# 2bitoperations/rtldavis

Measured on AMD Instinct MI355X. Metric: complex MSamples/s demodulated (uint8 IQ -> packed bits -> preamble matches -> packets), higher is better.
Workload: dtype f32 (FIR: f16 x f16 -> f32 on the matrix pipe, exact integer accumulation); 1 GPU; 4096 streams x 33 blocks x 8192 samples uint8 IQ per GPU (BASELINE configs[3]/[4]: 64 unique synthetic streams tiled, 2.21 GB resident in HBM), 14 samples/symbol, 19.2 kbit/s; streams_per_gpu=4096, parallelism=streams/1

## Files before the change

include/rtldavis_hip.h:

```cpp
#ifndef RTLDAVIS_HIP_H
#define RTLDAVIS_HIP_H

#include <stddef.h>
#include <stdint.h>

#ifdef __cplusplus
extern "C" {
#endif

#define RD_MAX_PREAMBLE 64
#define RD_MAX_PKT_BYTES 32

typedef enum rd_status {
    RD_OK = 0,
    RD_ERR_ARG = -1,
    RD_ERR_DEVICE = -2,
    RD_ERR_CAPACITY = -3,
    RD_ERR_STATE = -4
} rd_status;

typedef struct rd_config {
    int32_t bit_rate;
    int32_t symbol_length;
    int32_t preamble_symbols;
    int32_t packet_symbols;
    int32_t block_size;
    uint8_t preamble[RD_MAX_PREAMBLE];
} rd_config;

typedef struct rd_packet {
    int32_t stream;
    int32_t call;
    int32_t index;
    int32_t nbytes;
    uint8_t data[RD_MAX_PKT_BYTES];
    double rssi;
    double snr;
} rd_packet;

typedef struct rd_parsed {
    int32_t stream;
    int32_t call;
    int32_t index;
    int32_t freq_err;
    int32_t id;
    int32_t nbytes;
    uint8_t data[RD_MAX_PKT_BYTES];
    double rssi;
    double snr;
} rd_parsed;

typedef struct rd_timing {
    float demod_ms;
    float fixup_ms;
    float search_ms;
    float slice_ms;
    float total_ms;
    int32_t runs;
} rd_timing;

const char *rd_last_error(void);
int rd_device_count(void);
int rd_set_device(int device);
int rd_set_wait_timeout_ms(int ms);

typedef struct rd_demod rd_demod;

int rd_create(const rd_config *cfg, rd_demod **out);
void rd_destroy(rd_demod *h);
int rd_reset(rd_demod *h);
int rd_demod_block(rd_demod *h, const void *samples, size_t count, int is_complex, rd_packet *out, int cap, int *n);
int rd_create_multi(const rd_config *cfg, int n_streams, rd_demod **out);
int rd_demod_blocks(rd_demod *h, const uint8_t *iq, size_t nbytes, rd_packet *out, int cap, int *n);
int rd_demod_submit(rd_demod *h, const void *samples, size_t count, int is_complex);
int rd_set_input_push(int mode);
int rd_demod_input_mode(rd_demod *h);
int rd_demod_register_input(rd_demod *h, void *host, size_t nbytes);
int rd_demod_submit_from(rd_demod *h, size_t offset, size_t count, int is_complex);
int rd_demod_fetch(rd_demod *h, rd_packet *out, int cap, int *n);
int rd_demod_inflight(rd_demod *h);
int rd_demod_refetch(rd_demod *h, rd_packet *out, int cap, int *n);
int rd_demod_set_parse(rd_demod *h, int enabled);
int rd_demod_parsed(rd_demod *h, rd_parsed *out, int cap, int *n);
int rd_parse_packet(const uint8_t *data, int nbytes, uint8_t *msg, int *id);
int rd_copy_discriminated_stream(rd_demod *h, int stream, double *out, size_t n);
int rd_copy_discriminated(rd_demod *h, double *out, size_t n);
int rd_copy_filtered(rd_demod *h, double *out_interleaved, size_t n_complex);
int rd_copy_quantized(rd_demod *h, uint8_t *out, size_t n);

typedef struct rd_batch rd_batch;

int rd_batch_create(const rd_config *cfg, int n_streams, int n_blocks, rd_batch **out);
void rd_batch_destroy(rd_batch *b);
int rd_batch_input_ptr(rd_batch *b, void **dev_ptr, size_t *nbytes);
int rd_batch_upload(rd_batch *b, const uint8_t *iq_host, size_t nbytes);
int rd_batch_upload_async(rd_batch *b, const uint8_t *iq_host, size_t nbytes, void *hip_stream);
int rd_batch_run(rd_batch *b, void *hip_stream);
int rd_batch_results(rd_batch *b, rd_packet *out, int cap, int *n);
int rd_batch_copy_bits(rd_batch *b, int stream, uint8_t *out, size_t nbytes);
int rd_batch_copy_discriminated(rd_batch *b, int stream, size_t t0, double *out, size_t n);
int rd_batch_set_parse(rd_batch *b, int enabled);
int rd_batch_parsed(rd_batch *b, rd_parsed *out, int cap, int *n);
int rd_batch_set_timing(rd_batch *b, int enabled);
int rd_batch_get_timing(rd_batch *b, rd_timing *out);
int rd_batch_set_pipelined(rd_batch *b, int enabled);
#define RD_FORM_ORDERED_TAIL 1u
#define RD_FORM_SECOND_PASS 8u
#define RD_FORM_ONE_LAUNCH_TAIL 16u
int rd_batch_last_run_forms(rd_batch *b, uint32_t *forms);
int rd_batch_get_counters(rd_batch *b, uint64_t *fixup_runs, uint64_t *matches);
int rd_k1_schedule(rd_batch *b, uint32_t *tiles_per_chunk, uint32_t *waves);

int rd_lut_execute(const uint8_t *in_bytes, size_t n_bytes, double *out_cplx, size_t n_cplx);
int rd_rotate_fs4(const double *in_cplx, double *out_cplx, size_t n_cplx);
int rd_fir9(const double *in_cplx, size_t n_in, double *out_cplx, size_t n_out);
int rd_discriminate(const double *in_cplx, size_t n_in, double *out, size_t n_out);
int rd_quantize(const double *in, uint8_t *out, size_t n);
int rd_search(const rd_config *cfg, const uint8_t *quantized, size_t n, int32_t *indices, int cap, int *count);

typedef struct rd_chan_config {
    int32_t out_rate;
    int32_t decim;
    int32_t n_taps;
    int32_t n_channels;
    double gain;
} rd_chan_config;
typedef struct rd_chan rd_chan;

#define RD_IQ_U8 0
#define RD_IQ_S8 1
#define RD_IQ_S16 2
#define RD_IQ_CF32 4

int rd_chan_create(const rd_chan_config *cfg, const double *taps, const int64_t *shift_hz, rd_chan **out);
int rd_chan_create_fmt(const rd_chan_config *cfg, int sample_format, const double *taps, const int64_t *shift_hz,
                       rd_chan **out);
void rd_chan_destroy(rd_chan *h);
int rd_chan_upload(rd_chan *h, const void *wide_iq, size_t nbytes);
int rd_chan_input_ptr(rd_chan *h, size_t n_wide_samples, void **dev_ptr);
int rd_chan_run(rd_chan *h, size_t n_out, void *dst_dev, size_t dst_stream_stride, void *hip_stream);
int rd_chan_run_host(rd_chan *h, size_t n_out, uint8_t *out_host, size_t nbytes);
int rd_chan_spectrum(rd_chan *h, int n_bins, double *power_host, uint32_t *segments);
int rd_chan_spectrum_dev(rd_chan *h, int n_bins, void *dst_dev, void *hip_stream);
int rd_chan_set_gain(rd_chan *h, const double *gain, int n);

typedef struct rd_wideband rd_wideband;
int rd_wideband_create(const rd_config *cfg, const rd_chan_config *ccfg, const double *taps,
                       const int64_t *shift_hz, rd_wideband **out);
int rd_wb_create_fmt(const rd_config *cfg, const rd_chan_config *ccfg, int sample_format, const double *taps,
                     const int64_t *shift_hz, rd_wideband **out);
void rd_wideband_destroy(rd_wideband *w);
int rd_wideband_reset(rd_wideband *w);
int rd_wideband_submit(rd_wideband *w, const void *wide_iq, size_t nbytes);
int rd_wideband_fetch(rd_wideband *w, rd_packet *out, int cap, int *n);
int rd_wideband_refetch(rd_wideband *w, rd_packet *out, int cap, int *n);
int rd_wideband_inflight(rd_wideband *w);
int rd_wideband_copy_channelized(rd_wideband *w, uint8_t *out, size_t nbytes);
int rd_wideband_copy_discriminated(rd_wideband *w, int channel, double *out, size_t n);
int rd_wb_set_parse(rd_wideband *w, int enabled);
int rd_wb_parsed(rd_wideband *w, rd_parsed *out, int cap, int *n);
int rd_wb_retune(rd_wideband *w, const int64_t *shift_hz, int n);
int rd_wb_tuning(rd_wideband *w, int64_t *shift_hz, int64_t *phase, int n);
int rd_wb_set_gain(rd_wideband *w, const double *gain, int n);
int rd_wb_gains(rd_wideband *w, double *gain, int n);
typedef struct rd_chan_level {
    uint64_t power;
    uint32_t peak;
    uint32_t clipped;
    float gain;
    uint32_t chunk;
} rd_chan_level;
typedef struct rd_input_level {
    uint64_t power;
    uint64_t chunk;
    uint32_t peak;
    uint32_t clipped;
} rd_input_level;
int rd_wb_set_levels(rd_wideband *w, int enabled);
int rd_wb_levels(rd_wideband *w, rd_chan_level *out, int n, rd_input_level *in);
typedef struct rd_spectrum_info {
    uint64_t chunk;
    uint32_t segments;
    uint32_t n_bins;
} rd_spectrum_info;
int rd_wb_set_spectrum(rd_wideband *w, int n_bins);
int rd_wb_spectrum(rd_wideband *w, double *power, int n_bins, rd_spectrum_info *info);
typedef struct rd_burst {
    int32_t  channel;
    uint32_t first;
    uint32_t windows;
    uint32_t flags;
    uint64_t power;
    uint32_t peak;
    uint32_t pad;
    int64_t  corr_re, corr_im;
} rd_burst;
typedef struct rd_burst_floor {
    uint32_t threshold;
    uint32_t windows_off;
    uint32_t n_bursts;
    uint32_t chunk;
    uint64_t power_off;
    int64_t  corr_re_off, corr_im_off;
} rd_burst_floor;
int rd_wb_set_bursts(rd_wideband *w, int enabled);
int rd_wb_set_burst_threshold(rd_wideband *w, const uint32_t *thr, int n);
int rd_wb_burst_thresholds(rd_wideband *w, uint32_t *thr, int n);
int rd_wb_bursts(rd_wideband *w, rd_burst *out, int cap, int *n, rd_burst_floor *floor, int n_floor);
#define RD_BURST_MSG_BYTES 10
#define RD_BURST_MSG_REPAIRED 2u
#define RD_BD_REPAIR_L 8
#define RD_BURST_MSG_NARROW 4u
#define RD_BD_NB_GRID 64
#define RD_BD_NB_SHIFT 11
#define RD_BD_NB_MIN_SL 4
#define RD_BD_NB_MAX_SL 51
typedef struct rd_burst_msg {
    int32_t  channel;
    uint32_t first;
    int32_t  tau;
    uint32_t flags;
    uint64_t time;
    uint64_t margin;
    int64_t  f_re, f_im;
    uint8_t  data[RD_BURST_MSG_BYTES];
    uint8_t  ones;
    uint8_t  id;
    uint8_t  pad[4];
} rd_burst_msg;
int rd_wb_set_burst_decode(rd_wideband *w, int enabled);
int rd_wb_set_burst_repair(rd_wideband *w, int max_flips);
int rd_wb_burst_repair(rd_wideband *w, int *max_flips);
int rd_wb_set_burst_narrow(rd_wideband *w, int on);
int rd_wb_burst_narrow(rd_wideband *w, int *on);
int rd_bd_narrow_table(int sl, int16_t *taps, int16_t *centres);
int rd_wb_burst_messages(rd_wideband *w, rd_burst_msg *out, int cap, int *n, uint32_t *long_runs, int n_channels);
#define RD_BURST_MSG_EXPECTED 8u
#define RD_BX_MAX 64
#define RD_BX_MAX_SPAN 2048
#define RD_BX_ANY_ID 0xFFu
#define RD_BX_NO_ENTRY 0xFFFFFFFFu
typedef struct rd_expect {
    int32_t  channel;
    uint32_t id;
    uint64_t t_lo, t_hi;
    int32_t  corr_re, corr_im;
} rd_expect;
int rd_wb_set_burst_expect(rd_wideband *w, const rd_expect *e, int n);
int rd_wb_burst_expect(rd_wideband *w, rd_expect *out, int cap, int *n);
int rd_wb_expected_messages(rd_wideband *w, rd_burst_msg *out, int cap, int *n, uint32_t *candidates, int n_cand);
#define RD_BURST_MSG_SEARCHED 16u
#define RD_BS_MAX_CENTRES 8
#define RD_BS_PER 4
#define RD_BS_TILE 1024
typedef struct rd_bs_header {
    uint32_t n_msgs, sync_hits;
    uint32_t chunk;
    uint32_t dropped;
} rd_bs_header;
int rd_wb_set_burst_search(rd_wideband *w, const uint8_t *centres, int n);
int rd_wb_burst_search(rd_wideband *w, uint8_t *out, int cap, int *n);
int rd_wb_searched_messages(rd_wideband *w, rd_burst_msg *out, int cap, int *n, rd_bs_header *hdr, int n_hdr);
#define RD_BQ_MAX_GAP 1024
#define RD_BQ_INBAND 1u
#define RD_BQ_UNMEASURABLE 128u
typedef struct rd_burst_quality {
    uint64_t pkt, sig, noise;
    uint64_t pkt_nb, sig_nb, noise_nb;
    uint32_t n_noise, clipped;
    uint16_t peak; uint8_t g; uint8_t flags;
    uint32_t chunk;
} rd_burst_quality;
int rd_wb_set_burst_quality(rd_wideband *w, int on, int noise_gap);
int rd_wb_burst_quality(rd_wideband *w, int *on, int *noise_gap);
int rd_wb_burst_message_quality(rd_wideband *w, rd_burst_quality *out, int cap, int *n);
int rd_wb_expected_message_quality(rd_wideband *w, rd_burst_quality *out, int cap, int *n);
int rd_bq_window(int sl, int n_sym, int block_size, int have_prev, int64_t tau, int gap, int32_t *out);
#define RD_BC_RUNS 1u
#define RD_BC_MESSAGES 2u
#define RD_BC_MAX_ROLL 1024
#define RD_BC_MAX_QUOTA 65536
#define RD_BC_MAX_POOL (1u << 26)
#define RD_BC_PER 16
#define RD_BC_CUT_START 1
#define RD_BC_CUT_END 2
#define RD_BC_FROM_PREV 4
typedef struct rd_burst_clip {
    int32_t  channel;
    uint32_t source;
    uint32_t flags;
    int32_t  t0;
    uint32_t n;
    uint32_t offset;
    uint64_t time;
    uint64_t ref;
    uint32_t chunk;
    uint32_t pad;
} rd_burst_clip;
int rd_wb_set_burst_clips(rd_wideband *w, int sources, int pre, int post, int quota);
int rd_wb_burst_clips_config(rd_wideband *w, int *sources, int *pre, int *post, int *quota);
int rd_wb_burst_clips(rd_wideband *w, rd_burst_clip *out, int cap, int *n, uint8_t *bytes, size_t bytes_cap, size_t *n_bytes,
                      uint32_t *dropped, int n_channels);
int rd_bc_window(int block_size, int have_prev, int64_t a, int64_t e, int32_t *out);
#define RD_BURST_MSG_REPLAYED 32u
#define RD_CD_MAX_SPAN 2048
#define RD_CD_MAX_JOBS (1 << 20)
#define RD_CD_MAX_TAU (1 << 30)
typedef struct rd_clip_job {
    uint64_t offset;
    uint64_t clock;
    uint32_t n;
    uint32_t id;
    int32_t  tau_lo, tau_hi;
    int32_t  corr_re, corr_im;
    int32_t  channel;
    uint32_t pad;
} rd_clip_job;
typedef struct rd_cd_header { uint32_t n_msgs, candidates; int32_t ca, cb; } rd_cd_header;
typedef struct rd_clips rd_clips;
int rd_clips_create(const rd_config *cfg, rd_clips **out);
void rd_clips_destroy(rd_clips *h);
int rd_clips_upload(rd_clips *h, const uint8_t *pool, size_t nbytes);
int rd_clips_decode(rd_clips *h, const rd_clip_job *jobs, int n_jobs, int max_flips, int narrow, rd_burst_msg *msgs,
                    rd_cd_header *hdr, int64_t *soft);
int rd_clips_kernel_ms(rd_clips *h, float *ms);
int rd_cd_check_jobs(const rd_config *cfg, const rd_clip_job *jobs, int n_jobs, size_t pool_outputs, int *bad, const char **why);
#define RD_CS_MAX_SYM 192
#define RD_CS_MAX_PRE 4096
#define RD_CS_MAX_N (1 << 24)
#define RD_CS_MAX_SPECS (1 << 20)
#define RD_CS_MAX_AMP (1u << 16)
#define RD_CS_MAX_NOISE (1u << 20)
#define RD_CS_MAX_AT (1 << 30)
#define RD_CS_MAX_POOL (1ull << 40)
#define RD_CS_TABLE 4096
typedef struct rd_clip_spec {
    uint64_t offset;
    uint64_t seed;
    uint32_t n;
    int32_t  at;
    uint32_t phase0;
    int32_t  f_c;
    uint32_t f_d;
    uint32_t amp_q;
    uint32_t noise_q;
    uint32_t n_sym;
    uint16_t pre, post;
    uint32_t pad;
    uint8_t  bits[24];
} rd_clip_spec;
int rd_clips_synth(rd_clips *h, const rd_clip_spec *specs, int n_specs, uint64_t pool_outputs);
int rd_clips_download(rd_clips *h, uint8_t *out, size_t nbytes);
int rd_clips_synth_ms(rd_clips *h, float *ms);
int rd_cs_check_specs(const rd_clip_spec *specs, int n_specs, uint64_t pool_outputs, int *bad, const char **why);
void rd_cs_table(int16_t out[RD_CS_TABLE]);
int rd_wb_fetched_chunk(rd_wideband *w, uint64_t *chunk);
int rd_wideband_debug_advance_clock(rd_wideband *w, uint64_t n_out);

void rd_debug_mfma_taps(uint16_t *out);
void rd_debug_mfma_taps8(uint16_t *out);
void rd_debug_mfma_taps8s(uint16_t *vals, uint32_t *idx);
int rd_debug_demod_mfma(const uint8_t *iq_host, int n_streams, uint32_t n_samples, int hist_mode,
                        uint32_t hist_bytes, float *g_out, uint32_t *bits_out, uint32_t *fix_out,
                        uint32_t fix_cap, uint32_t *n_fix);
int rd_debug_bursts(const uint8_t *chan, size_t stride, int n_ch, size_t n_out, const uint32_t *thr, uint64_t seq,
                    rd_burst *recs_out, rd_burst_floor *floor_out);
int rd_debug_burst_decode(const rd_config *cfg, const uint8_t *cur, const uint8_t *prev, size_t stride, int n_ch,
                          uint64_t clock, uint64_t seq, const rd_burst *runs, const uint32_t *n_runs,
                          rd_burst_msg *msgs_out, uint32_t *n_msgs, uint32_t *long_runs, uint32_t *chunk);
int rd_debug_burst_decode_repair(const rd_config *cfg, const uint8_t *cur, const uint8_t *prev, size_t stride, int n_ch,
                                 uint64_t clock, uint64_t seq, const rd_burst *runs, const uint32_t *n_runs, int max_flips,
                                 rd_burst_msg *msgs_out, uint32_t *n_msgs, uint32_t *long_runs, uint32_t *chunk);
int rd_debug_burst_decode_narrow(const rd_config *cfg, const uint8_t *cur, const uint8_t *prev, size_t stride, int n_ch,
                                 uint64_t clock, uint64_t seq, const rd_burst *runs, const uint32_t *n_runs, int max_flips,
                                 int narrow, rd_burst_msg *msgs_out, uint32_t *n_msgs, uint32_t *long_runs, uint32_t *chunk);
int rd_debug_burst_expect(const rd_config *cfg, const uint8_t *cur, const uint8_t *prev, size_t stride, int n_ch,
                          uint64_t clock, uint64_t seq, const rd_expect *e, int n_e, int max_flips, int narrow,
                          rd_burst_msg *msgs_out, uint32_t *hdr_out);
int rd_debug_burst_search(const rd_config *cfg, const uint8_t *cur, const uint8_t *prev, size_t stride, int n_ch,
                          uint64_t clock, uint64_t seq, const uint8_t *centres, int n, rd_burst_msg *msgs_out,
                          rd_bs_header *hdr_out);
#define RD_BQ_DEBUG_CHUNK 0x51A7u
int rd_debug_burst_quality(const rd_config *cfg, const uint8_t *cur, const uint8_t *prev, size_t stride, int n_ch,
                           int noise_gap, const rd_burst_msg *msgs, const uint32_t *n_msgs_per_channel, rd_burst_quality *out);
size_t rd_bc_slot_size(int n_ch, int quota);
int rd_debug_burst_clips(const rd_config *cfg, const uint8_t *cur, const uint8_t *prev, size_t stride, int n_ch, uint64_t clock,
                         uint64_t seq, const rd_burst *runs, const uint32_t *n_runs, const rd_burst_msg *msgs,
                         const uint32_t *n_msgs, const rd_burst_msg *x_msgs, const uint32_t *x_hdr, int n_expect,
                         const rd_burst_msg *s_msgs, const rd_bs_header *s_hdr, int n_search, const uint32_t *owed_prev,
                         int sources, int pre, int post, int quota, uint8_t *out);

#ifdef __cplusplus
}
#endif
#endif
```

rtldavis_amd/batch.py:

```python
from __future__ import annotations

import ctypes as C
from typing import List, Optional

import numpy as np

from . import _lib
from .dsp import Packet, PacketConfig, _cfg_struct


RD_PACKET_DTYPE = np.dtype([("stream", "<i4"), ("call", "<i4"), ("index", "<i4"), ("nbytes", "<i4"),
                            ("data", "u1", (_lib.RD_MAX_PKT_BYTES,)), ("rssi", "<f8"), ("snr", "<f8")])
assert RD_PACKET_DTYPE.itemsize == C.sizeof(_lib.RdPacket)


RD_PARSED_DTYPE = np.dtype([("stream", "<i4"), ("call", "<i4"), ("index", "<i4"), ("freq_err", "<i4"),
                            ("id", "<i4"), ("nbytes", "<i4"), ("data", "u1", (_lib.RD_MAX_PKT_BYTES,)),
                            ("rssi", "<f8"), ("snr", "<f8")])
assert RD_PARSED_DTYPE.itemsize == C.sizeof(_lib.RdParsed)


class BatchDemodulator:
    def __init__(self, cfg: PacketConfig, n_streams: int, n_blocks: int, device: Optional[int] = None) -> None:
        self.cfg = cfg
        self.n_streams = int(n_streams)
        self.n_blocks = int(n_blocks)
        self.n_samples = self.n_blocks * cfg.block_size
        self._b = C.c_void_p()
        if device is not None:
            _lib.check(_lib.lib().rd_set_device(int(device)))
        _lib.check(_lib.lib().rd_batch_create(C.byref(_cfg_struct(cfg)), self.n_streams, self.n_blocks, C.byref(self._b)))
        self._cap = 0
        self._recs = None

    def close(self) -> None:
        if self._b:
            b, self._b = self._b, None
            _lib.lib().rd_batch_destroy(b)

    def __del__(self):
        try:
            self.close()
        except Exception:
            pass

    def input_ptr(self):
        p, n = C.c_void_p(), C.c_size_t()
        _lib.check(_lib.lib().rd_batch_input_ptr(self._b, C.byref(p), C.byref(n)))
        return p.value, n.value

    def upload(self, iq: np.ndarray) -> None:
        a = np.ascontiguousarray(iq, dtype=np.uint8)
        if a.size != self.n_streams * 2 * self.n_samples:
            raise ValueError("Incompatible array sizes")
        _lib.check(_lib.lib().rd_batch_upload(self._b, a.ctypes.data, a.size))

    def upload_async(self, iq: np.ndarray, hip_stream: int) -> None:
        if iq.dtype != np.uint8 or not iq.flags["C_CONTIGUOUS"] or iq.size != self.n_streams * 2 * self.n_samples:
            raise ValueError("Incompatible array sizes")
        _lib.check(_lib.lib().rd_batch_upload_async(self._b, iq.ctypes.data, iq.size, C.c_void_p(hip_stream or None)))

    def run(self, hip_stream: int = 0) -> None:
        _lib.check(_lib.lib().rd_batch_run(self._b, C.c_void_p(hip_stream or None)))

    def set_parse(self, enabled: bool) -> None:
        _lib.check(_lib.lib().rd_batch_set_parse(self._b, int(bool(enabled))))

    def parsed(self) -> np.ndarray:
        cap = max(1024, 4 * self.n_streams)
        while True:
            buf = (_lib.RdParsed * cap)()
            n = C.c_int(0)
            rc = _lib.lib().rd_batch_parsed(self._b, buf, cap, C.byref(n))
            if rc == _lib.RD_ERR_CAPACITY:
                cap = n.value + 1024
                continue
            _lib.check(rc)
            return np.frombuffer(buf, dtype=RD_PARSED_DTYPE, count=n.value).copy()

    def set_timing(self, level) -> None:
        _lib.check(_lib.lib().rd_batch_set_timing(self._b, int(level)))

    def set_pipelined(self, enabled=True) -> None:
        _lib.check(_lib.lib().rd_batch_set_pipelined(self._b, 1 if enabled else 0))

    def timing(self) -> dict:
        t = _lib.RdTiming()
        _lib.check(_lib.lib().rd_batch_get_timing(self._b, C.byref(t)))
        return {k: float(getattr(t, k)) for k, _ in t._fields_}

    def last_run_forms(self) -> dict:
        f = C.c_uint32()
        _lib.check(_lib.lib().rd_batch_last_run_forms(self._b, C.byref(f)))
        return {"ordered_tail": bool(f.value & 1), "second_pass": bool(f.value & 8), "one_launch_tail": bool(f.value & 16)}

    def counters(self) -> dict:
        f, m = C.c_uint64(), C.c_uint64()
        _lib.check(_lib.lib().rd_batch_get_counters(self._b, C.byref(f), C.byref(m)))
        ch, wv = C.c_uint32(), C.c_uint32()
        _lib.check(_lib.lib().rd_k1_schedule(self._b, C.byref(ch), C.byref(wv)))
        return {"fixup_runs": f.value, "matches": m.value, "k1_chunk": ch.value, "k1_waves": wv.value}

    def results(self) -> np.ndarray:
        L = _lib.lib()
        n = C.c_int(0)
        if self._recs is None:
            self._cap = max(1024, 16 * self.n_streams)
            self._recs = (_lib.RdPacket * self._cap)()
        rc = L.rd_batch_results(self._b, self._recs, self._cap, C.byref(n))
        if rc == _lib.RD_ERR_CAPACITY:
            self._cap = n.value + 1024
            self._recs = (_lib.RdPacket * self._cap)()
            rc = L.rd_batch_results(self._b, self._recs, self._cap, C.byref(n))
        _lib.check(rc)
        return np.frombuffer(self._recs, dtype=RD_PACKET_DTYPE, count=n.value)

    def records(self):
        out = []
        for r in self.results():
            data = np.frombuffer(r["data"][: int(r["nbytes"])].tobytes(), dtype=np.uint8)
            out.append((int(r["stream"]), int(r["call"]),
                        Packet(int(r["index"]), data, float(r["rssi"]), float(r["snr"]))))
        return out

    def packets(self) -> List[List[List[Packet]]]:
        res = [[[] for _ in range(self.n_blocks)] for _ in range(self.n_streams)]
        for s, c, p in self.records():
            res[s][c].append(p)
        return res

    def bits(self, stream: int) -> np.ndarray:
        out = np.empty((self.n_samples + 7) // 8, dtype=np.uint8)
        _lib.check(_lib.lib().rd_batch_copy_bits(self._b, int(stream), out.ctypes.data, out.size))
        return out

    def discriminated(self, stream: int, t0: int, n: int) -> np.ndarray:
        out = np.empty(int(n), dtype=np.float64)
        _lib.check(_lib.lib().rd_batch_copy_discriminated(self._b, int(stream), int(t0), out.ctypes.data, out.size))
        return out

    def demodulate(self, iq: np.ndarray) -> List[List[List[Packet]]]:
        self.upload(iq)
        self.run()
        return self.packets()
```

rtldavis_amd/csrc/rd_batch.hip:

```cpp
#include <algorithm>
#include <chrono>
#include <cstdio>
#include <cstdlib>
#include <cstring>
#include <map>
#include <mutex>
#include <vector>

#include "rd_internal.h"
#include "rd_math.h"

static_assert(RD_BATCH_RUN == RD_RUN, "rd_batch_plan.h sizes the bit arrays by the kernels' run length");

static bool dbg_host() {
    static int v = -1;
    if (v < 0) v = getenv("RD_DEBUG_HOST") ? 1 : 0;
    return v == 1;
}
static double now_ms() {
    return std::chrono::duration<double, std::milli>(std::chrono::steady_clock::now().time_since_epoch()).count();
}

struct rd_batch_bufs {
    int device = -1;
    uint8_t *d_iq = nullptr;
    uint32_t *d_bits = nullptr, *d_fix = nullptr;
    uint32_t *d_cnt = nullptr;
    uint32_t *fixb = nullptr, *gstate = nullptr;
    uint32_t match_cap = 0, rec_cap = 0;
    rd_match *d_matches = nullptr;
    rd_packet *d_recs = nullptr;
    void *d_tasks = nullptr;
    rd_parsed *d_parsed = nullptr;
    uint32_t *h_cnt_pin = nullptr;
    rd_packet *h_recs_pin = nullptr;
    hipStream_t copy_stream = nullptr;
    hipEvent_t done = nullptr;
    hipEvent_t kdone = nullptr;
    hipEvent_t kfirst = nullptr;
    hipEvent_t uploaded = nullptr;
};
struct rd_batch_run_state {
    bool ran = false;
    bool fetched = false;
    bool upload_pending = false;
    hipStream_t stream = nullptr;
    int cnt_set = 0;
    bool timing = false, detail = false;
    hipEvent_t *ev = nullptr;
    rd_run_plan plan;
    bool ft_run = false;
    bool dev_order = false;
    int dense = 0;
    bool second_pass = false;
    bool deferred = false;
    uint32_t ft_seq = 0;
    uint32_t last_launch[2] = {0, 0};
    uint32_t have = 0;
    uint32_t h_cnt[RD_CNT_SLOTS] = {};
};
struct rd_batch_timer {
    std::vector<hipEvent_t> evs;
    size_t ev_runs = 0;
    std::vector<uint8_t> ev_end;
};
struct rd_batch {
    rd_devcfg dc;
    int n_streams, n_blocks;
    rd_batch_sizes sz;
    bool dev_ready = false;
    bool timing = false, timing_detail = false, parse = false, pipelined = false;
    rd_batch_bufs m;
    rd_batch_run_state run;
    rd_batch_learned learned;
    rd_batch_timer timer;
    rd_order_scratch order;
};

static rd_layout batch_layout(const rd_batch *b) {
    rd_layout l;
    l.iq = b->m.d_iq;
    l.stream_stride = (size_t)b->sz.n_samples * 2;
    l.n_streams = b->n_streams;
    l.n_samples = (uint32_t)b->sz.n_samples;
    l.hist_mode = 0;
    l.valid_from = 0;
    l.bits = b->m.d_bits;
    l.bits_stride = b->sz.bits_stride;
    return l;
}

extern "C" int rd_batch_create(const rd_config *cfg, int n_streams, int n_blocks, rd_batch **out) {
    if (!out) return rd_fail_msg(RD_ERR_ARG, "null out");
    rd_devcfg dc;
    int rc = rd_devcfg_checked(cfg, &dc);
    if (rc) return rc;
    const char *why = "";
    if ((rc = rd_batch_check_size(n_streams, n_blocks, cfg->block_size, &why))) return rd_fail_msg(rc, "%s", why);
    rd_batch *b = new rd_batch();
    b->dc = dc;
    b->n_streams = n_streams;
    b->n_blocks = n_blocks;
    b->sz = rd_batch_sizes_of(n_streams, n_blocks, dc, rd_batch_hooks());
    *out = b;
    return RD_OK;
}

static uint32_t *batch_cnt(const rd_batch *b) { return b->m.d_cnt + (size_t)b->run.cnt_set * b->sz.cnt_stride; }

static int batch_alloc_lists(rd_batch *b, uint32_t match_cap) {
    rd_batch_bufs &m = b->m;
    const bool ran = b->run.ran;
    if (m.match_cap) {
        hipFree(m.d_matches); m.d_matches = nullptr;
        hipFree(m.d_recs); m.d_recs = nullptr;
        hipHostFree(m.h_recs_pin); m.h_recs_pin = nullptr;
        hipFree(m.d_tasks); m.d_tasks = nullptr;
        hipFree(m.d_parsed); m.d_parsed = nullptr;
    }
    m.match_cap = m.rec_cap = 0;
    b->run.ran = false;
    const uint32_t rec_cap = 2 * match_cap;
    HIPCHK(hipMalloc(&m.d_matches, (size_t)match_cap * sizeof(rd_match)));
    HIPCHK(hipMalloc(&m.d_recs, (size_t)rec_cap * sizeof(rd_packet)));
    HIPCHK(hipMalloc(&m.d_tasks, (size_t)rec_cap * RD_TASK_BYTES));
    HIPCHK(hipHostMalloc((void **)&m.h_recs_pin, (size_t)rec_cap * sizeof(rd_packet), hipHostMallocDefault));
    m.match_cap = match_cap;
    m.rec_cap = rec_cap;
    b->run.ran = ran;
    return RD_OK;
}

static int batch_alloc(rd_batch *b) {
    rd_batch_bufs &m = b->m;
    if (b->dev_ready) return rd_use_device(m.device);
    int rc = rd_ensure_device();
    if (rc) return rc;
    HIPCHK(hipGetDevice(&m.device));
    const rd_batch_sizes z = b->sz = rd_batch_sizes_of(b->n_streams, b->n_blocks, b->dc, rd_batch_hooks_env());
    b->learned.bcap = z.bcap;
    HIPCHK(hipMalloc(&m.d_iq, z.iq_bytes + RD_INPUT_PAD));
    HIPCHK(hipMemset(m.d_iq + z.iq_bytes, 127, RD_INPUT_PAD));
    HIPCHK(hipMalloc(&m.d_bits, (uint64_t)b->n_streams * z.bits_stride * sizeof(uint32_t)));
    HIPCHK(hipMalloc(&m.d_fix, (size_t)z.fix_cap * sizeof(uint32_t)));
    if (z.ft_ok) {
        HIPCHK(hipMalloc(&m.fixb, z.groups * z.fix_bcap * sizeof(uint32_t)));
        HIPCHK(hipMalloc(&m.gstate, 3 * z.groups * sizeof(uint32_t)));
        HIPCHK(hipMemset(m.gstate, 0, 3 * z.groups * sizeof(uint32_t)));
    }
    HIPCHK(hipMalloc(&m.d_cnt, 2 * z.cnt_stride * sizeof(uint32_t)));
    HIPCHK(hipMemset(m.d_cnt, 0, 2 * z.cnt_stride * sizeof(uint32_t)));
    if ((rc = batch_alloc_lists(b, z.match_cap))) return rc;
    HIPCHK(hipHostMalloc((void **)&m.h_cnt_pin, RD_CNT_SLOTS * sizeof(uint32_t), hipHostMallocDefault));
    HIPCHK(hipEventCreateWithFlags(&m.done, hipEventDisableTiming));
    HIPCHK(hipEventCreateWithFlags(&m.kdone, hipEventDisableTiming));
    HIPCHK(hipEventCreateWithFlags(&m.kfirst, hipEventDisableTiming));
    HIPCHK(hipEventCreateWithFlags(&m.uploaded, hipEventDisableTiming));
    HIPCHK(hipStreamCreateWithFlags(&m.copy_stream, hipStreamNonBlocking));
    b->dev_ready = true;
    return RD_OK;
}

static void batch_free(rd_batch_bufs &m) {
    hipFree(m.d_iq); hipFree(m.d_bits); hipFree(m.d_fix); hipFree(m.d_cnt);
    hipFree(m.d_matches); hipFree(m.d_recs); hipFree(m.d_tasks);
    hipFree(m.d_parsed);
    hipFree(m.fixb); hipFree(m.gstate);
    hipHostFree(m.h_cnt_pin); hipHostFree(m.h_recs_pin);
    if (m.done) hipEventDestroy(m.done);
    if (m.kdone) hipEventDestroy(m.kdone);
    if (m.kfirst) hipEventDestroy(m.kfirst);
    if (m.uploaded) hipEventDestroy(m.uploaded);
    if (m.copy_stream) hipStreamDestroy(m.copy_stream);
}

static int timer_reserve(rd_batch_timer &t, size_t n) {
    const size_t old = t.evs.size();
    if (old >= n) return RD_OK;
    t.evs.resize(n, nullptr);
    for (size_t i = old; i < n; i++) HIPCHK(hipEventCreate(&t.evs[i]));
    return RD_OK;
}

static int batch_readback(rd_batch *b, hipEvent_t after) {
    rd_batch_bufs &m = b->m;
    HIPCHK(hipStreamWaitEvent(m.copy_stream, after, 0));
    HIPCHK(hipMemcpyAsync(m.h_cnt_pin, batch_cnt(b), RD_CNT_SLOTS * sizeof(uint32_t), hipMemcpyDeviceToHost, m.copy_stream));
    b->run.have = rd_batch_spec_count(b->run.dev_order, m.match_cap, m.rec_cap, b->learned.spec_recs);
    if (b->run.have)
        HIPCHK(hipMemcpyAsync(m.h_recs_pin, m.d_recs, (size_t)b->run.have * sizeof(rd_packet), hipMemcpyDeviceToHost, m.copy_stream));
    HIPCHK(hipEventRecord(m.done, m.copy_stream));
    return RD_OK;
}

static std::mutex g_tail_mx;
typedef std::pair<int, hipStream_t> rd_tail_key;
static std::map<rd_tail_key, rd_batch *> g_tail;

static void tail_park(rd_batch *b) {
    g_tail[rd_tail_key(b->m.device, b->run.stream)] = b;
    b->run.deferred = true;
}
static rd_batch *tail_take(int device, hipStream_t st) {
    auto it = g_tail.find(rd_tail_key(device, st));
    if (it == g_tail.end()) return nullptr;
    rd_batch *p = it->second;
    g_tail.erase(it);
    p->run.deferred = false;
    return p;
}
static void tail_drop(rd_batch *p) {
    auto it = g_tail.find(rd_tail_key(p->m.device, p->run.stream));
    if (it != g_tail.end() && it->second == p) g_tail.erase(it);
    p->run.deferred = false;
}

static int batch_flush_locked(rd_batch *p) {
    if (!p->run.deferred) return RD_OK;
    tail_drop(p);
    int rc = rd_use_device(p->m.device);
    if (rc) return rc;
    HIPCHK(hipEventRecord(p->m.kdone, p->run.stream));
    return batch_readback(p, p->m.kdone);
}
static int batch_flush(rd_batch *b) {
    std::lock_guard<std::mutex> g(g_tail_mx);
    return batch_flush_locked(b);
}
static bool batch_stream_has_tail(int device, hipStream_t st) {
    std::lock_guard<std::mutex> g(g_tail_mx);
    return g_tail.find(rd_tail_key(device, st)) != g_tail.end();
}
static int batch_adopt(int device, hipStream_t st, hipEvent_t carrier) {
    std::lock_guard<std::mutex> g(g_tail_mx);
    rd_batch *p = tail_take(device, st);
    return p ? batch_readback(p, carrier) : RD_OK;
}

static int batch_settle(rd_batch *b, const hipStream_t *st, const char *what = nullptr) {
    if (!b->run.ran || b->run.fetched) return RD_OK;
    int rc = batch_flush(b);
    if (rc) return rc;
    if (!st) return rd_wait_event(b->m.done, what);
    HIPCHK(hipStreamWaitEvent(*st, b->m.done, 0));
    return RD_OK;
}

extern "C" void rd_batch_destroy(rd_batch *b) {
    if (!b) return;
    {
        std::lock_guard<std::mutex> g(g_tail_mx);
        tail_drop(b);
    }
    if (b->dev_ready && rd_owns_device_state()) {
        if (b->m.device >= 0) hipSetDevice(b->m.device);
        if (b->run.ran && !b->run.fetched) hipDeviceSynchronize();
        batch_free(b->m);
        for (auto &e : b->timer.evs) if (e) hipEventDestroy(e);
    }
    delete b;
}

extern "C" int rd_batch_input_ptr(rd_batch *b, void **dev_ptr, size_t *nbytes) {
    if (!b || !dev_ptr) return rd_fail_msg(RD_ERR_ARG, "null argument");
    int rc = batch_alloc(b);
    if (rc) return rc;
    *dev_ptr = b->m.d_iq;
    if (nbytes) *nbytes = b->sz.iq_bytes;
    return RD_OK;
}

extern "C" int rd_batch_upload(rd_batch *b, const uint8_t *iq_host, size_t nbytes) {
    if (!b || !iq_host) return rd_fail_msg(RD_ERR_ARG, "null argument");
    int rc = batch_alloc(b);
    if (rc) return rc;
    if (nbytes != b->sz.iq_bytes) {
        return rd_fail_msg(RD_ERR_ARG, "Incompatible array sizes: got %zu bytes, expected %zu", nbytes, b->sz.iq_bytes);
    }
    if ((rc = batch_settle(b, nullptr, "the previous run before an upload"))) return rc;
    HIPCHK(hipMemcpy(b->m.d_iq, iq_host, nbytes, hipMemcpyHostToDevice));
    if (!b->learned.ft_sticky) b->learned.tail_off = false;
    return RD_OK;
}

extern "C" int rd_batch_upload_async(rd_batch *b, const uint8_t *iq_host, size_t nbytes, void *hip_stream) {
    if (!b || !iq_host) return rd_fail_msg(RD_ERR_ARG, "null argument");
    int rc = batch_alloc(b);
    if (rc) return rc;
    if (nbytes != b->sz.iq_bytes) return rd_fail_msg(RD_ERR_ARG, "Incompatible array sizes: got %zu bytes, expected %zu", nbytes, b->sz.iq_bytes);
    hipStream_t cs = (hipStream_t)hip_stream;
    if ((rc = batch_settle(b, &cs))) return rc;
    HIPCHK(hipMemcpyAsync(b->m.d_iq, iq_host, nbytes, hipMemcpyHostToDevice, cs));
    HIPCHK(hipEventRecord(b->m.uploaded, cs));
    b->run.upload_pending = true;
    if (!b->learned.ft_sticky) b->learned.tail_off = false;
    return RD_OK;
}

static hipEvent_t batch_event(const rd_batch *b, rd_run_event which) {
    switch (which) {
    case RD_RUN_EV0: return b->run.ev[0];
    case RD_RUN_EV1: return b->run.ev[1];
    case RD_RUN_EV4: return b->run.ev[4];
    case RD_RUN_KFIRST: return b->m.kfirst;
    case RD_RUN_KDONE: return b->m.kdone;
    default: return nullptr;
    }
}

static int batch_tail(rd_batch *b, bool first, uint32_t *zero_next = nullptr) {
    rd_batch_bufs &m = b->m;
    rd_batch_run_state &r = b->run;
    hipStream_t st = r.stream;
    const rd_layout lay = batch_layout(b);
    const long B = b->dc.B, L = b->dc.L, p_lo = B - L, p_hi = (long)(b->n_blocks + 1) * B - L;
    const bool last_on_slice = !b->parse, defer = first && r.plan.defer;
    hipEvent_t last = batch_event(b, first ? r.plan.end : r.plan.end_again);
    if (r.timing && first) b->timer.ev_end.push_back(defer ? 0 : 1);
    r.dev_order = false;
    if (r.ft_run && first) {
        rd_ft_bufs fb;
        fb.fixb = m.fixb; fb.gstate = m.gstate; fb.fix_bcap = b->sz.fix_bcap; fb.bcap = b->learned.bcap;
        fb.fixcnt = batch_cnt(b) + b->sz.ft_cnt_off;
        r.ft_seq = r.ft_seq % 4095u + 1u;
        const int ok = rd_launch_tail_fused(lay, b->dc, b->n_blocks, p_lo, p_hi, fb, b->sz.ft_limit ? b->sz.ft_limit : fb.bcap, r.ft_seq, 0,
                                            m.d_recs, m.rec_cap, batch_cnt(b), st, last_on_slice ? last : nullptr, zero_next,
                                            (uint32_t)b->sz.cnt_stride);
        if (!ok) return rd_fail_msg(RD_ERR_STATE, "the one-launch tail refused a shape its buffers were allocated for");
        r.dev_order = true;
        r.dense = 1;
    } else {
        rd_launch_search(m.d_bits, b->sz.bits_stride, b->n_streams, b->sz.n_samples, p_lo, p_hi, b->dc, m.d_matches, m.match_cap,
                         batch_cnt(b), st);
        if (r.timing && r.detail) HIPCHK(hipEventRecord(r.ev[3], st));
        r.dense = rd_launch_slice(lay, m.d_bits, b->sz.bits_stride, b->sz.n_samples, b->dc, m.d_matches, m.match_cap, 1, b->n_blocks, 0,
                                  m.d_recs, nullptr, batch_cnt(b), st, last_on_slice ? last : nullptr, m.d_tasks);
    }
    if (b->parse) {
        if (!m.d_parsed) HIPCHK(hipMalloc(&m.d_parsed, (size_t)m.rec_cap * sizeof(rd_parsed)));
        rd_launch_parse(lay, b->dc, m.d_recs, m.match_cap, m.d_parsed, batch_cnt(b), st, r.dense);
    }
    if (defer) {
        std::lock_guard<std::mutex> g(g_tail_mx);
        auto it = g_tail.find(rd_tail_key(m.device, st));
        if (it != g_tail.end() && it->second != b) {
            int rc = batch_flush_locked(it->second);
            if (rc) return rc;
        }
        tail_park(b);
        HIPCHK(hipGetLastError());
        return RD_OK;
    }
    if (!last_on_slice) HIPCHK(hipEventRecord(last, st));
    int rc = batch_readback(b, last);
    if (rc) return rc;
    HIPCHK(hipGetLastError());
    return RD_OK;
}

static int batch_refused(rd_batch *b, bool had_upload) {
    b->run.cnt_set ^= 1;
    b->run.upload_pending = had_upload;
    if (b->timing) b->timer.ev_runs--;
    b->run.ran = false;
    b->run.fetched = true;
    return rd_fail_msg(RD_ERR_STATE, "the demod kernel's grid has fewer waves than work queues and more chunks than waves: not launched");
}

static int batch_begin_run(rd_batch *b, hipStream_t st, bool *had_upload) {
    rd_batch_run_state &r = b->run;
    int rc = batch_settle(b, &st);
    if (rc) return rc;
    r.stream = st;
    *had_upload = r.upload_pending;
    if (r.upload_pending) {
        HIPCHK(hipStreamWaitEvent(st, b->m.uploaded, 0));
        r.upload_pending = false;
    }
    r.fetched = false;
    r.cnt_set ^= 1;
    r.timing = b->timing;
    r.detail = b->timing_detail;
    if (r.timing) {
        if ((rc = timer_reserve(b->timer, 5 * (b->timer.ev_runs + 1)))) return rc;
        r.ev = &b->timer.evs[5 * b->timer.ev_runs++];
    }
    return RD_OK;
}

extern "C" int rd_batch_run(rd_batch *b, void *hip_stream) {
    if (!b) return rd_fail_msg(RD_ERR_ARG, "null batch");
    int rc = batch_alloc(b);
    if (rc) return rc;
    rd_batch_run_state &r = b->run;
    hipStream_t st = (hipStream_t)hip_stream;
    bool had_upload = false;
    if ((rc = batch_begin_run(b, st, &had_upload))) return rc;
    uint32_t *cnt = batch_cnt(b), *cnt_next = b->m.d_cnt + (size_t)(r.cnt_set ^ 1) * b->sz.cnt_stride;
    const rd_run_plan p = r.plan = rd_batch_plan_run({b->sz.fast_ok, b->sz.ft_ok, b->learned.tail_off, r.timing, r.detail, b->pipelined,
                                                      b->parse, batch_stream_has_tail(b->m.device, st)});
    uint32_t *fixl = p.buckets ? b->m.fixb : b->m.d_fix, *bcnt = p.buckets ? cnt + b->sz.ft_cnt_off : nullptr;
    const uint32_t fixc = p.buckets ? b->sz.fix_bcap : b->sz.fix_cap;
    const rd_layout lay = batch_layout(b);
    uint32_t honoured = 0;
    if (p.record_around) HIPCHK(hipEventRecord(r.ev[0], st));
    if (p.demod) {
        honoured = rd_launch_demod(lay, fixl, fixc, cnt, st, batch_event(b, p.ride_start), batch_event(b, p.ride_stop),
                                   p.buckets ? RD_DEMOD_FIX_BUCKETS : 0u, r.last_launch, bcnt);
        if (honoured & RD_DEMOD_REFUSED) return batch_refused(b, had_upload);
    }
    if (p.record_around) HIPCHK(hipEventRecord(r.ev[1], st));
    if (p.record_carrier) HIPCHK(hipEventRecord(batch_event(b, p.carrier), st));
    if (p.carrier && (rc = batch_adopt(b->m.device, st, batch_event(b, p.carrier)))) return rc;
    r.second_pass = false;
    r.ft_run = p.demod && (honoured & RD_DEMOD_FIX_BUCKETS);
    if (!r.ft_run)
        rd_launch_fixup(lay, fixl, fixc, cnt, p.demod ? 0 : 1, cnt_next, st, (uint32_t)b->sz.cnt_stride, b->learned.last_fix);
    if (r.timing && r.detail) HIPCHK(hipEventRecord(r.ev[2], st));
    if ((rc = batch_tail(b, true, r.ft_run ? cnt_next : nullptr))) return rc;
    r.ran = true;
    return RD_OK;
}

static int batch_second_pass(rd_batch *b) {
    const uint32_t zero[5] = {0, 0, 0, 0, 0};
    HIPCHK(hipMemcpyAsync(batch_cnt(b) + RD_CNT_MATCH, zero, sizeof zero, hipMemcpyHostToDevice, b->run.stream));
    b->run.second_pass = true;
    return batch_tail(b, false);
}

struct batch_ladder {
    rd_batch *b;
    int read(rd_ladder_in &in) {
        rd_batch_run_state &r = b->run;
        const double ta = now_ms();
        int rc = rd_wait_event(b->m.done, "the batch run's results");
        if (rc) return rc;
        memcpy(r.h_cnt, b->m.h_cnt_pin, sizeof r.h_cnt);
        if (dbg_host()) fprintf(stderr, "[rd] finish: wait %.3f ms\n", now_ms() - ta);
        in = {r.h_cnt[RD_CNT_FIX], r.h_cnt[RD_CNT_MATCH], r.h_cnt[RD_CNT_OVF], r.ft_run, r.second_pass, r.dev_order, b->sz.fast_ok, 0,
              b->sz.fix_cap, b->m.match_cap, b->sz.ft_limit, (uint64_t)b->n_streams * b->sz.bits_stride};
        return RD_OK;
    }
    int carry_out(const rd_ladder_action &a) {
        rd_batch_run_state &r = b->run;
        int rc = RD_OK;
        r.dev_order = a.dev_order;
        if (a.exact_fixup) rd_launch_fixup(batch_layout(b), b->m.d_fix, b->sz.fix_cap, batch_cnt(b), 1, nullptr, r.stream);
        const uint32_t cap = b->sz.fix_cap;
        if (a.stamp_fix) HIPCHK(hipMemcpyAsync(batch_cnt(b) + RD_CNT_FIX, &cap, sizeof cap, hipMemcpyHostToDevice, r.stream));
        if (a.tail_overflow && dbg_host())
            fprintf(stderr, "[rd] one-launch tail overflow: flags %u (1 a stream's match list, 2 records), matches %u\n",
                    r.h_cnt[RD_CNT_OVF], r.h_cnt[RD_CNT_MATCH]);
        if (a.grow_to && (rc = batch_alloc_lists(b, a.grow_to))) return rc;
        if (a.second_pass && (rc = batch_second_pass(b))) return rc;
        if (a.done) r.fetched = true;
        return RD_OK;
    }
    int gave_up() { return rd_fail_msg(RD_ERR_DEVICE, "result lists kept overflowing"); }
};

static int batch_finish(rd_batch *b) {
    if (!b->run.ran) return rd_fail_msg(RD_ERR_STATE, "rd_batch_run has not been called");
    int rc = batch_flush(b);
    if (rc) return rc;
    batch_ladder hands = {b};
    return rd_batch_ladder_run(hands, b->learned);
}

extern "C" int rd_batch_results(rd_batch *b, rd_packet *out, int cap, int *n) {
    if (!b || !n) return rd_fail_msg(RD_ERR_ARG, "null argument");
    const double t0 = now_ms();
    int rc = batch_finish(b);
    if (rc) return rc;
    const double t1 = now_ms();
    rd_batch_bufs &m = b->m;
    rd_batch_run_state &r = b->run;
    const rd_result_counts c = rd_batch_result_counts(r.h_cnt, r.dense != 0, m.match_cap, m.rec_cap);
    if (c.nprim > r.have) {
        rc = rd_copy_d2h(m.h_recs_pin + r.have, m.d_recs + r.have, (size_t)(c.nprim - r.have) * sizeof(rd_packet), m.copy_stream);
        if (rc) return rc;
    }
    if (c.nextra) {
        rc = rd_copy_d2h(m.h_recs_pin + c.nprim, m.d_recs + m.match_cap, (size_t)c.nextra * sizeof(rd_packet), m.copy_stream);
        if (rc) return rc;
    }
    const uint32_t nrec = c.nprim + c.nextra;
    b->learned.spec_recs = std::max<uint32_t>(1024, c.nprim + c.nprim / 4);
    r.have = rd_batch_spec_count(r.dev_order, m.match_cap, m.rec_cap, b->learned.spec_recs);
    const double t2 = now_ms();
    if (!r.dev_order) rd_order_and_dedupe(m.h_recs_pin, nrec, b->dc.S, b->order);
    const size_t count = r.dev_order ? nrec : b->order.kept.size();
    *n = (int)count;
    if ((int)count > cap) return rd_fail_msg(RD_ERR_CAPACITY, "need room for %zu packets", count);
    if (count && !out) return rd_fail_msg(RD_ERR_ARG, "null out");
    if (r.dev_order && count) memcpy(out, m.h_recs_pin, count * sizeof(rd_packet));
    if (!r.dev_order)
        for (size_t i = 0; i < count; i++) out[i] = m.h_recs_pin[b->order.kept[i]];
    if (dbg_host())
        fprintf(stderr, "[rd] results%s: finish %.3f ms, D2H %u recs %.3f ms, %s %.3f ms\n", r.dev_order ? " (k_tail)" : "", t1 - t0,
                nrec, t2 - t1, r.dev_order ? "copy" : "order+dedupe+copy", now_ms() - t2);
    return RD_OK;
}

extern "C" int rd_batch_copy_bits(rd_batch *b, int stream, uint8_t *out, size_t nbytes) {
    if (!b || !out) return rd_fail_msg(RD_ERR_ARG, "null argument");
    if (stream < 0 || stream >= b->n_streams) return rd_fail_msg(RD_ERR_ARG, "stream out of range");
    const size_t need = (size_t)((b->sz.n_samples + 7) / 8);
    if (nbytes < need) return rd_fail_msg(RD_ERR_ARG, "bit buffer too small: %zu < %zu", nbytes, need);
    int rc = batch_finish(b);
    if (rc) return rc;
    return rd_copy_d2h(out, (const uint8_t *)(b->m.d_bits + (size_t)stream * b->sz.bits_stride), need, b->run.stream);
}

extern "C" int rd_batch_copy_discriminated(rd_batch *b, int stream, size_t t0, double *out, size_t n) {
    if (!b || !out) return rd_fail_msg(RD_ERR_ARG, "null argument");
    if (stream < 0 || stream >= b->n_streams || t0 + n > (size_t)b->sz.n_samples)
        return rd_fail_msg(RD_ERR_ARG, "range out of bounds");
    int rc = batch_alloc(b);
    if (rc) return rc;
    if (n == 0) return RD_OK;
    double *d = nullptr;
    HIPCHK(hipMalloc(&d, n * sizeof(double)));
    rd_launch_disc(batch_layout(b), stream, (long)t0, (long)n, d, b->run.stream);
    rc = rd_copy_d2h(out, d, n * sizeof(double), b->run.stream);
    hipFree(d);
    return rc;
}

extern "C" int rd_batch_set_parse(rd_batch *b, int enabled) {
    if (!b) return rd_fail_msg(RD_ERR_ARG, "null batch");
    b->parse = enabled != 0;
    return RD_OK;
}

extern "C" int rd_batch_parsed(rd_batch *b, rd_parsed *out, int cap, int *n) {
    if (!b || !n) return rd_fail_msg(RD_ERR_ARG, "null argument");
    if (!b->parse) return rd_fail_msg(RD_ERR_STATE, "rd_batch_set_parse(b, 1) must precede rd_batch_run");
    int rc = batch_finish(b);
    if (rc) return rc;
    const uint32_t np = std::min(b->run.h_cnt[RD_CNT_PARSED], b->m.rec_cap);
    std::vector<rd_parsed> recs(np);
    if (np) {
        rc = rd_copy_d2h(recs.data(), b->m.d_parsed, (size_t)np * sizeof(rd_parsed), b->run.stream);
        if (rc) return rc;
    }
    const size_t kept = rd_order_parsed(recs.data(), recs.size(), b->dc.S);
    *n = (int)kept;
    if ((int)kept > cap) return rd_fail_msg(RD_ERR_CAPACITY, "need room for %zu messages", kept);
    if (kept) {
        if (!out) return rd_fail_msg(RD_ERR_ARG, "null out");
        memcpy(out, recs.data(), kept * sizeof(rd_parsed));
    }
    return RD_OK;
}

extern "C" int rd_batch_set_pipelined(rd_batch *b, int enabled) {
    if (!b) return rd_fail_msg(RD_ERR_ARG, "null batch");
    b->pipelined = enabled != 0;
    return RD_OK;
}

extern "C" int rd_batch_set_timing(rd_batch *b, int enabled) {
    if (!b) return rd_fail_msg(RD_ERR_ARG, "null batch");
    b->timing = enabled != 0;
    b->timing_detail = enabled >= 2;
    b->timer.ev_runs = 0;
    b->timer.ev_end.clear();
    if (b->timing && b->dev_ready && rd_use_device(b->m.device) == RD_OK) return timer_reserve(b->timer, 5 * 64);
    return RD_OK;
}

extern "C" int rd_batch_get_timing(rd_batch *b, rd_timing *out) {
    if (!b || !out) return rd_fail_msg(RD_ERR_ARG, "null argument");
    if (!b->timing) return rd_fail_msg(RD_ERR_STATE, "timing not enabled");
    int rc = batch_finish(b);
    if (rc) return rc;
    rd_timing t = {};
    size_t n_end = 0;
    for (size_t r = 0; r < b->timer.ev_runs; r++) {
        hipEvent_t *e = &b->timer.evs[5 * r];
        float v[5] = {0, 0, 0, 0, 0};
        HIPCHK(hipEventElapsedTime(&v[0], e[0], e[1]));
        if (b->timing_detail) {
            HIPCHK(hipEventElapsedTime(&v[1], e[1], e[2]));
            HIPCHK(hipEventElapsedTime(&v[2], e[2], e[3]));
            HIPCHK(hipEventElapsedTime(&v[3], e[3], e[4]));
        }
        const bool has_end = r >= b->timer.ev_end.size() || b->timer.ev_end[r];
        if (has_end) { HIPCHK(hipEventElapsedTime(&v[4], e[0], e[4])); n_end++; }
        t.demod_ms += v[0]; t.fixup_ms += v[1]; t.search_ms += v[2]; t.slice_ms += v[3]; t.total_ms += v[4];
    }
    if (b->timer.ev_runs) {
        const float k = 1.0f / (float)b->timer.ev_runs;
        t.demod_ms *= k; t.fixup_ms *= k; t.search_ms *= k; t.slice_ms *= k;
        t.total_ms = n_end ? t.total_ms / (float)n_end : 0.0f;
    }
    t.runs = (int32_t)b->timer.ev_runs;
    b->timer.ev_runs = 0;
    b->timer.ev_end.clear();
    *out = t;
    return RD_OK;
}

extern "C" int rd_batch_last_run_forms(rd_batch *b, uint32_t *forms) {
    if (!b || !forms) return rd_fail_msg(RD_ERR_ARG, "null argument");
    int rc = batch_finish(b);
    if (rc) return rc;
    *forms = (b->run.dev_order ? RD_FORM_ORDERED_TAIL | RD_FORM_ONE_LAUNCH_TAIL : 0u) | (b->run.second_pass ? RD_FORM_SECOND_PASS : 0u);
    return RD_OK;
}

extern "C" int rd_k1_schedule(rd_batch *b, uint32_t *tiles_per_chunk, uint32_t *waves) {
    uint32_t v[2] = {0, 0};
    if (b) {
        if (!b->run.ran) return rd_fail_msg(RD_ERR_STATE, "rd_batch_run has not been called");
        v[0] = b->run.last_launch[0]; v[1] = b->run.last_launch[1];
    } else {
        rd_debug_last_launch(v);
    }
    if (tiles_per_chunk) *tiles_per_chunk = v[0];
    if (waves) *waves = v[1];
    return RD_OK;
}

extern "C" int rd_batch_get_counters(rd_batch *b, uint64_t *fixup_runs, uint64_t *matches) {
    if (!b) return rd_fail_msg(RD_ERR_ARG, "null batch");
    int rc = batch_finish(b);
    if (rc) return rc;
    if (fixup_runs) *fixup_runs = b->learned.last_fix;
    if (matches) *matches = b->learned.last_match;
    return RD_OK;
}
```

rtldavis_amd/csrc/rd_batch_plan.cpp:

```cpp
#include "rd_batch_plan.h"

#include <stdlib.h>

#include <algorithm>

int rd_batch_check_size(int n_streams, int n_blocks, int block_size, const char **why) {
    if (n_streams < 1 || n_blocks < 1) { *why = "n_streams and n_blocks must be >= 1"; return RD_ERR_ARG; }
    const long n = (long)n_blocks * block_size;
    const uint64_t runs = (uint64_t)n_streams * ((n + RD_BATCH_RUN - 1) / RD_BATCH_RUN);
    if (n > 0x7FFFFFF0L || runs > 0x0FFFFFFFull) {
        *why = "batch too large: at most 2^28 32-sample runs (8.6e9 samples) per batch";
        return RD_ERR_ARG;
    }
    *why = "";
    return RD_OK;
}

rd_batch_hooks rd_batch_hooks_env(void) {
    rd_batch_hooks h;
    const char *ti = getenv("RD_TAIL_IMPL");
    h.legacy_tail = ti && ti[0] == 'l';
    if (const char *e = getenv("RD_TEST_MATCH_CAP")) h.match_cap = atol(e);
    if (const char *e = getenv("RD_TEST_BUCKET_CAP")) h.bucket_cap = atol(e);
    if (const char *e = getenv("RD_TEST_FIX_BCAP")) h.fix_bcap = atol(e);
    return h;
}

rd_batch_sizes rd_batch_sizes_of(int n_streams, int n_blocks, const rd_devcfg &dc, const rd_batch_hooks &hooks) {
    rd_batch_sizes z;
    const long n = (long)n_blocks * dc.B;
    z.n_samples = n;
    z.bits_stride = (size_t)((n + 31) / 32);
    z.fast_ok = ((size_t)n * 2) % 16 == 0;
    const uint64_t runs = (uint64_t)n_streams * z.bits_stride;
    z.iq_bytes = (size_t)n_streams * n * 2;
    z.fix_cap = (uint32_t)std::min<uint64_t>(runs, std::max<uint64_t>(4096, runs / 8));
    z.match_cap = (uint32_t)std::min<uint64_t>((uint64_t)n_streams * (8 + 1ull * n_blocks) + 1024, 1u << 26);
    if (hooks.match_cap >= 1 && hooks.match_cap < (long)z.match_cap) z.match_cap = (uint32_t)hooks.match_cap;
    z.ft_ok = !hooks.legacy_tail && z.fast_ok && rd_davis_shape(dc) &&
              n < (1l << 30) && dc.B < (1 << 24) && z.bits_stride % 4 == 0 && dc.L >= dc.B &&
              (long)(n_blocks + 1) * dc.B - dc.L >= 0 &&
              ((long)(n_blocks + 1) * dc.B - dc.L) / 32 + 16 <= (long)z.bits_stride;
    if (hooks.bucket_cap >= 1 && hooks.bucket_cap < RD_BUCKET_MIN) z.ft_limit = (uint32_t)hooks.bucket_cap;
    if (!z.ft_ok) return z;
    z.groups = ((size_t)n_streams + RD_FT_STREAMS - 1) / RD_FT_STREAMS;
    z.ft_cnt_off = z.cnt_stride;
    z.cnt_stride += (z.groups + 3) & ~(size_t)3;
    const uint64_t tps = ((uint64_t)n + RD_TILE_SAMPLES - 1) / RD_TILE_SAMPLES;
    z.fix_bcap = (uint32_t)std::min<uint64_t>((2 * RD_FT_STREAMS * (tps / 4 + 8) + 63) & ~63ull, 1u << 20);
    if (hooks.fix_bcap >= 1 && hooks.fix_bcap < (long)z.fix_bcap) z.fix_bcap = (uint32_t)hooks.fix_bcap;
    z.bcap = rd_ord_bucket_cap(n);
    return z;
}

rd_run_plan rd_batch_plan_run(const rd_run_mode &m) {
    rd_run_plan p;
    p.demod = m.fast_ok;
    p.buckets = m.ft_ok && m.fast_ok && !m.tail_off && !(m.timing && m.timing_detail);
    if (m.timing && m.fast_ok) {
        p.ride_start = RD_RUN_EV0;
        p.ride_stop = RD_RUN_EV1;
    } else if (m.fast_ok && m.parked) {
        p.ride_stop = RD_RUN_KFIRST;
    }
    p.record_around = m.timing && !m.fast_ok;
    if (m.parked) {
        p.carrier = m.timing ? RD_RUN_EV1 : RD_RUN_KFIRST;
        p.record_carrier = !m.timing && !m.fast_ok;
    }
    p.defer = m.pipelined && !m.parse && !(m.timing && m.timing_detail);
    p.end_again = m.timing ? RD_RUN_EV4 : RD_RUN_KDONE;
    p.end = p.defer ? RD_RUN_EV_NONE : p.end_again;
    return p;
}

rd_ladder_action rd_batch_ladder_step(const rd_ladder_in &in, rd_batch_learned &lr) {
    rd_ladder_action a;
    a.dev_order = in.dev_order;
    const bool first_ft = in.ft_run && !in.second_pass;
    bool redo = false;
    if (first_ft && (in.ovf & (8u | 16u))) {
        a.exact_fixup = redo = true;
        lr.last_fix = in.all_runs;
        lr.tail_off = true;
        a.dev_order = false;
    } else {
        if (first_ft && (in.ovf & 1u)) {
            if (!in.ft_limit && lr.bcap < RD_BUCKET_MAX) lr.bcap = std::min<uint32_t>(2 * lr.bcap, RD_BUCKET_MAX);
            else if (!in.ft_limit) lr.ft_sticky = true;
        }
        if (in.fast_ok && !in.ft_run && in.fix > in.fix_cap) {
            a.exact_fixup = a.stamp_fix = redo = true;
            lr.last_fix = in.all_runs;
            if (lr.tail_off) a.dev_order = false;
        } else if (in.attempt == 0) {
            lr.last_fix = in.fix;
        }
        if (a.dev_order && in.ovf) {
            lr.tail_off = true;
            a.tail_overflow = a.second_pass = true;
            return a;
        }
    }
    if (!a.dev_order && in.match > in.match_cap) {
        a.grow_to = in.match + in.match / 4 + 1024;
        redo = true;
    }
    a.second_pass = redo;
    a.done = !redo;
    if (a.done) lr.last_match = in.match;
    return a;
}

uint32_t rd_batch_spec_count(bool dev_order, uint32_t match_cap, uint32_t rec_cap, uint32_t spec_recs) {
    return std::min(dev_order ? rec_cap : match_cap, spec_recs);
}

rd_result_counts rd_batch_result_counts(const uint32_t *h_cnt, bool dense, uint32_t match_cap, uint32_t rec_cap) {
    rd_result_counts c;
    c.nprim = dense ? std::min(h_cnt[RD_CNT_TASKS], rec_cap) : std::min(h_cnt[RD_CNT_MATCH], match_cap);
    c.nextra = dense ? 0u : std::min(h_cnt[RD_CNT_REC], match_cap);
    return c;
}
```

rtldavis_amd/csrc/rd_batch_plan.h:

```cpp
#pragma once
#include <stddef.h>
#include <stdint.h>

#include "rd_host.h"

enum { RD_CNT_FIX = 0, RD_CNT_MATCH = 1, RD_CNT_REC = 2, RD_CNT_TASKS = 3, RD_CNT_PARSED = 4, RD_CNT_OVF = 5, RD_CNT_SLOTS = 8 };
#define RD_FT_GSH 2
#define RD_FT_STREAMS (1 << RD_FT_GSH)
#define RD_NQUEUE 32
#define RD_QUEUE_STRIDE 64
#define RD_CNT_QUEUE0 RD_QUEUE_STRIDE
#define RD_CNT_TOTAL (RD_CNT_QUEUE0 + RD_NQUEUE * RD_QUEUE_STRIDE)
#define RD_TILE_SAMPLES 2048
#define RD_BATCH_RUN 32
#define RD_BATCH_ATTEMPTS 8

int rd_batch_check_size(int n_streams, int n_blocks, int block_size, const char **why);

struct rd_batch_hooks {
    bool legacy_tail = false;
    long match_cap = 0;
    long bucket_cap = 0;
    long fix_bcap = 0;
};
rd_batch_hooks rd_batch_hooks_env(void);

struct rd_batch_sizes {
    long n_samples = 0;
    size_t bits_stride = 0;
    bool fast_ok = false;
    size_t iq_bytes = 0;
    uint32_t fix_cap = 0;
    uint32_t match_cap = 0;
    bool ft_ok = false;
    size_t groups = 0;
    size_t cnt_stride = RD_CNT_TOTAL;
    size_t ft_cnt_off = 0;
    uint32_t fix_bcap = 0;
    uint32_t bcap = 0;
    uint32_t ft_limit = 0;
};
rd_batch_sizes rd_batch_sizes_of(int n_streams, int n_blocks, const rd_devcfg &dc, const rd_batch_hooks &hooks);

enum rd_run_event : uint8_t { RD_RUN_EV_NONE = 0, RD_RUN_EV0, RD_RUN_EV1, RD_RUN_EV4, RD_RUN_KFIRST, RD_RUN_KDONE };
struct rd_run_plan {
    bool demod = false;
    bool buckets = false;
    rd_run_event ride_start = RD_RUN_EV_NONE, ride_stop = RD_RUN_EV_NONE;
    bool record_around = false;
    rd_run_event carrier = RD_RUN_EV_NONE;
    bool record_carrier = false;
    bool defer = false;
    rd_run_event end = RD_RUN_EV_NONE;
    rd_run_event end_again = RD_RUN_EV_NONE;
};
struct rd_run_mode {
    bool fast_ok, ft_ok, tail_off, timing, timing_detail, pipelined, parse;
    bool parked;
};
rd_run_plan rd_batch_plan_run(const rd_run_mode &m);

struct rd_batch_learned {
    bool tail_off = false;
    bool ft_sticky = false;
    uint32_t bcap = 0;
    uint32_t spec_recs = 1024;
    uint64_t last_fix = 0, last_match = 0;
};
struct rd_ladder_in {
    uint32_t fix, match, ovf;
    bool ft_run, second_pass, dev_order, fast_ok;
    int attempt;
    uint32_t fix_cap, match_cap, ft_limit;
    uint64_t all_runs;
};
struct rd_ladder_action {
    bool exact_fixup = false;
    bool stamp_fix = false;
    uint32_t grow_to = 0;
    bool second_pass = false;
    bool done = false;
    bool dev_order = false;
    bool tail_overflow = false;
};
rd_ladder_action rd_batch_ladder_step(const rd_ladder_in &in, rd_batch_learned &lr);
template <class Dev>
int rd_batch_ladder_run(Dev &dev, rd_batch_learned &lr) {
    for (int attempt = 0; attempt < RD_BATCH_ATTEMPTS; attempt++) {
        rd_ladder_in in = {};
        int rc = dev.read(in);
        if (rc) return rc;
        in.attempt = attempt;
        const rd_ladder_action a = rd_batch_ladder_step(in, lr);
        if ((rc = dev.carry_out(a))) return rc;
        if (a.done) return RD_OK;
    }
    return dev.gave_up();
}

uint32_t rd_batch_spec_count(bool dev_order, uint32_t match_cap, uint32_t rec_cap, uint32_t spec_recs);
struct rd_result_counts { uint32_t nprim, nextra; };
rd_result_counts rd_batch_result_counts(const uint32_t *h_cnt, bool dense, uint32_t match_cap, uint32_t rec_cap);
```

rtldavis_amd/csrc/rd_demod_mfma.hip:

```cpp
#include <cstdio>
#include <cstdlib>
#include <cstring>

#include <hip/hip_ext.h>

#include "rd_internal.h"
#include "rd_math.h"
#include "rd_mfma.h"

#define RD_MF_WG 256
#define RD_MF_WAVES (RD_MF_WG / 64)
#ifndef RD_MF_MINWAVES
#define RD_MF_MINWAVES 4
#endif
#define RD_MF_GROUP_BYTES 1152
#define RD_MF_IMG_BYTES (16 + 4 * RD_MF_GROUP_BYTES)
#define RD_MF_IMG_PAD 4624
#define RD_MF_XB_BYTES (3 * 1024 + 32 + 32)
#define RD_MF_PEND 64
#ifndef RD_MF_STAGE_TILES
#define RD_MF_STAGE_TILES 4
#endif

typedef _Float16 rd_h8 __attribute__((ext_vector_type(8)));
typedef _Float16 rd_h16 __attribute__((ext_vector_type(16)));
typedef _Float16 rd_h2 __attribute__((ext_vector_type(2)));
typedef float rd_f16v __attribute__((ext_vector_type(16)));
typedef uint32_t rd_u4v __attribute__((ext_vector_type(4)));
typedef float rd_f4v __attribute__((ext_vector_type(4)));
typedef uint32_t rd_u2v __attribute__((ext_vector_type(2)));

static const rd_mf_taps h_mf_taps = rd_mf_make_taps();
__device__ const rd_mf_taps8 g_mf_taps8 = rd_mf_make_taps8();
static const rd_mf_taps8 h_mf_taps8 = rd_mf_make_taps8();
extern "C" void rd_debug_mfma_taps8(uint16_t *out) { memcpy(out, &h_mf_taps8, sizeof h_mf_taps8); }
#ifndef RD_MF_SPARSE
#define RD_MF_SPARSE 1
#endif
constexpr bool rd_mf_taps8s_ok() { bool ok = true; (void)rd_mf_make_taps8s(&ok); return ok; }
static_assert(rd_mf_taps8s_ok(), "a row of the tap matrix has more than two non-zero elements in a group of four");
constexpr rd_mf_taps8s rd_mf_taps8s_value() { bool ok = true; return rd_mf_make_taps8s(&ok); }
__device__ const rd_mf_taps8s g_mf_taps8s = rd_mf_taps8s_value();
static const rd_mf_taps8s h_mf_taps8s = rd_mf_taps8s_value();
extern "C" void rd_debug_mfma_taps8s(uint16_t *vals, uint32_t *idx) {
    memcpy(vals, h_mf_taps8s.v, sizeof h_mf_taps8s.v);
    memcpy(idx, h_mf_taps8s.idx, sizeof h_mf_taps8s.idx);
}

extern "C" void rd_debug_mfma_taps(uint16_t *out) { memcpy(out, &h_mf_taps, sizeof h_mf_taps); }

__device__ __forceinline__ rd_h8 rd_mf_frag(rd_u2v d) {
    rd_u4v v;
    v.x = d.x & 0x00FF00FFu;
    v.y = __builtin_amdgcn_perm(0u, d.x, 0x0c030c01u);
    v.z = d.y & 0x00FF00FFu;
    v.w = __builtin_amdgcn_perm(0u, d.y, 0x0c030c01u);
    return __builtin_bit_cast(rd_h8, v);
}

__device__ __forceinline__ float rd_mf_num(float ar, float ai, float cr, float ci, float &t1) {
    t1 = ai * ci;
    return __builtin_fmaf(-ar, cr, -t1);
}
__device__ __forceinline__ float rd_mf_guard(float nmin, float tmax) { return __builtin_fmaf(-4.76837158e-7f, tmax, nmin); }


template <int OFF>
__device__ __forceinline__ void rd_lds_write16(uint32_t addr, rd_f4v v) {
    asm volatile("ds_write_b128 %0, %1 offset:%2" : : "v"(addr), "v"(v), "i"(OFF) : "memory");
}
template <int OFF>
__device__ __forceinline__ rd_f4v rd_lds_read16(uint32_t addr) {
    rd_f4v r;
    asm volatile("ds_read_b128 %0, %1 offset:%2" : "=v"(r) : "v"(addr), "i"(OFF) : "memory");
    return r;
}
__device__ __forceinline__ void rd_lds_wait(rd_f4v &r) { asm volatile("s_waitcnt lgkmcnt(0)" : "+v"(r) : : "memory"); }
__device__ __forceinline__ void rd_lds_write4(uint32_t addr, uint32_t v) {
    asm volatile("ds_write_b32 %0, %1" : : "v"(addr), "v"(v) : "memory");
}
__device__ __forceinline__ rd_u4v rd_lds_read16u(uint32_t addr) {
    rd_u4v r;
    asm volatile("ds_read_b128 %0, %1\n\ts_waitcnt lgkmcnt(0)" : "=&v"(r) : "v"(addr) : "memory");
    return r;
}
__device__ __forceinline__ uint32_t rd_lds_read4(uint32_t addr) {
    uint32_t r;
    asm volatile("ds_read_b32 %0, %1\n\ts_waitcnt lgkmcnt(0)" : "=&v"(r) : "v"(addr) : "memory");
    return r;
}
__device__ __forceinline__ uint32_t rd_lds_addr(const void *p) {
    return (uint32_t)(uintptr_t)(const __attribute__((address_space(3))) void *)p;
}

__device__ __forceinline__ bool rd_mf_any(bool c) { return __ballot(c) != 0; }


struct rd_mf8_addr {
    uint32_t xw;
    uint32_t xw7;
    uint32_t rd1, rdE, rdO;
    uint32_t rd0;
};
struct rd_mf8_kept {
    float n2, n3;
    float g0r, g0i;
    float g1r, g1i, g2r, g2i;
    float nmin, tmax;
};

template <int B>
__device__ __forceinline__ constexpr int rd_mf8_woff() { return B == 0 ? 0 : (B & 1) ? 1024 : 2048; }

template <int B, int DBG>
__device__ __forceinline__ void rd_mf8_finish(const rd_mf8_kept &k, rd_f4v &p, uint32_t &W, uint32_t &fb, bool &slow) {
    rd_lds_wait(p);
    float t0, t1;
    const float n0 = rd_mf_num(p.x, p.y, p.z, p.w, t0);
    const float n1 = rd_mf_num(p.z, p.w, k.g0r, k.g0i, t1);
    if (DBG == 0 || DBG == 3) {
        const float nm = rd_mf_guard(rd_min3abs(k.nmin, n0, n1), rd_max3abs(k.tmax, t0, t1));
        if (rd_mf_any(!(nm > RD_MF_C0_MAX))) {
            slow = true;
            float F = rd_max3abs(0.0f, p.x, p.y);
            F = rd_max3abs(F, p.z, p.w);
            F = rd_max3abs(F, k.g0r, k.g0i);
            F = rd_max3abs(F, k.g1r, k.g1i);
            F = rd_max3abs(F, k.g2r, k.g2i);
            if (!(nm > rd_mf_c0(F))) fb |= 1u << (8 * (B & 3));
        }
    }
    uint32_t w = rd_shift_in_sign(W, n0);
    w = rd_shift_in_sign(w, n1);
    w = rd_shift_in_sign(w, k.n2);
    W = __builtin_amdgcn_alignbit(w, __builtin_bit_cast(uint32_t, k.n3), 27);
}

template <int B, int DBG>
__device__ __forceinline__ void rd_mf8_block(const rd_h8 (&A)[2], const rd_f16v &dcC, const int sidx, const int sidx2, const rd_u2v (&D)[9],
                                             rd_h8 &bfA, rd_h16 &bb, const rd_mf8_addr &ad, rd_mf8_kept &k0, rd_mf8_kept &kp, rd_f4v &p, uint32_t &Wlo,
                                             uint32_t &Whi, uint32_t &fblo, uint32_t &fbhi, bool &slow, float *dg, int dleft) {
    const rd_h8 bfB = rd_mf_frag(D[B + 1]);
    if (RD_MF_SPARSE && DBG != 8 && DBG != 9) {
        const rd_h16 wB = __builtin_shufflevector(bfB, bfB, 0, 1, 2, 3, 4, 5, 6, 7, 0, 1, 2, 3, 4, 5, 6, 7);
        if (B & 1) bb = __builtin_shufflevector(wB, bb, 0, 1, 2, 3, 4, 5, 6, 7, 24, 25, 26, 27, 28, 29, 30, 31);
        else bb = __builtin_shufflevector(bb, wB, 0, 1, 2, 3, 4, 5, 6, 7, 16, 17, 18, 19, 20, 21, 22, 23);
    }
    __builtin_amdgcn_sched_barrier(0);
    rd_f16v acc;
    if (DBG == 8 || DBG == 9) {
        rd_f16v c0 = dcC;
        if (DBG == 9) asm volatile("" : "+v"(c0));
        acc = __builtin_amdgcn_mfma_f32_32x32x16_f16(A[0], bfA, c0, 0, 0, 0);
        asm volatile("" : : "v"(bfB));
    } else if (RD_MF_SPARSE) {
        const uint32_t dbits = __builtin_bit_cast(uint32_t, -(float)RD_MF_DHI / 16777216.0f);
        uint64_t dh2 = ((uint64_t)dbits << 32) | dbits;
        asm volatile("" : "+s"(dh2));
        struct { uint64_t q[8]; } ci;
#pragma unroll
        for (int i = 0; i < 4; i++) asm volatile("v_mov_b64 %0, %1" : "=v"(ci.q[i]) : "s"(dh2));
#pragma unroll
        for (int i = 4; i < 8; i++) asm volatile("v_mov_b64 %0, 0" : "=v"(ci.q[i]));
        asm volatile("s_nop 1" ::: "memory");
        const rd_f16v c0 = __builtin_bit_cast(rd_f16v, ci);
        acc = (B & 1) ? __builtin_amdgcn_smfmac_f32_32x32x32_f16(A[1], bb, c0, sidx2, 0, 0)
                      : __builtin_amdgcn_smfmac_f32_32x32x32_f16(A[0], bb, c0, sidx, 0, 0);
    } else {
        acc = __builtin_amdgcn_mfma_f32_32x32x16_f16(A[0], bfA, dcC, 0, 0, 0);
        acc = __builtin_amdgcn_mfma_f32_32x32x16_f16(A[1], bfB, acc, 0, 0, 0);
    }
    if (B >= 2) rd_mf8_finish<B - 1, DBG>(kp, p, B - 1 <= 3 ? Wlo : Whi, B - 1 <= 3 ? fblo : fbhi, slow);
    __builtin_amdgcn_sched_barrier(0);
    float g[8];
#pragma unroll
    for (int i = 0; i < 8; i++) g[i] = __builtin_fmaf(acc[i], 2048.0f, acc[8 + i]);
    if (DBG == 3) {
#pragma unroll
        for (int r = 0; r < 4; r++)
            if (8 * B + r < dleft) { dg[2 * (8 * B + r)] = g[2 * r]; dg[2 * (8 * B + r) + 1] = g[2 * r + 1]; }
    }
    if (DBG != 10 && DBG != 11) {
        const rd_f4v x = {g[4], g[5], g[6], g[7]};
        if (B == 7) rd_lds_write16<0>(ad.xw7, x);
        else rd_lds_write16<rd_mf8_woff<B>()>(ad.xw, x);
    } else {
        asm volatile("" : : "v"(g[4]), "v"(g[5]), "v"(g[6]), "v"(g[7]));
    }
    if (B >= 1 && DBG != 10 && DBG != 11) p = rd_lds_read16<0>(B == 1 ? ad.rd1 : (B & 1) ? ad.rdO : ad.rdE);
    if (DBG == 11) asm volatile("" : "+v"(p));
    rd_mf8_kept &k = B == 0 ? k0 : kp;
    float t2, t3;
    k.n2 = rd_mf_num(g[0], g[1], g[2], g[3], t2);
    k.n3 = rd_mf_num(g[2], g[3], g[4], g[5], t3);
    k.nmin = rd_min3abs(3.0e38f, k.n2, k.n3);
    k.tmax = rd_max3abs(0.0f, t2, t3);
    k.g0r = g[0]; k.g0i = g[1];
    k.g1r = g[2]; k.g1i = g[3]; k.g2r = g[4]; k.g2i = g[5];
    bfA = bfB;
}

template <int DBG>
__device__ __forceinline__ void rd_mf8_tile(const rd_h8 (&A)[2], const rd_f16v &dcC, const int sidx, const int sidx2, const rd_u2v (&D)[9],
                                            const rd_mf8_addr &ad,
                                            uint32_t &word, uint32_t &fbw, bool &slow, float *dg, int dleft) {
    rd_h8 bfA = rd_mf_frag(D[0]);
    rd_h16 bb = __builtin_shufflevector(bfA, bfA, 0, 1, 2, 3, 4, 5, 6, 7, 8, 9, 10, 11, 12, 13, 14, 15);
    rd_mf8_kept k0, kp;
    rd_f4v p = {0.0f, 0.0f, 0.0f, 0.0f};
    uint32_t Wlo = 0, Whi = 0, fblo = 0, fbhi = 0;
    slow = false;
    rd_mf8_block<0, DBG>(A, dcC, sidx, sidx2, D, bfA, bb, ad, k0, kp, p, Wlo, Whi, fblo, fbhi, slow, dg, dleft);
    rd_mf8_block<1, DBG>(A, dcC, sidx, sidx2, D, bfA, bb, ad, k0, kp, p, Wlo, Whi, fblo, fbhi, slow, dg, dleft);
    rd_mf8_block<2, DBG>(A, dcC, sidx, sidx2, D, bfA, bb, ad, k0, kp, p, Wlo, Whi, fblo, fbhi, slow, dg, dleft);
    rd_mf8_block<3, DBG>(A, dcC, sidx, sidx2, D, bfA, bb, ad, k0, kp, p, Wlo, Whi, fblo, fbhi, slow, dg, dleft);
    rd_mf8_block<4, DBG>(A, dcC, sidx, sidx2, D, bfA, bb, ad, k0, kp, p, Wlo, Whi, fblo, fbhi, slow, dg, dleft);
    rd_mf8_block<5, DBG>(A, dcC, sidx, sidx2, D, bfA, bb, ad, k0, kp, p, Wlo, Whi, fblo, fbhi, slow, dg, dleft);
    rd_mf8_block<6, DBG>(A, dcC, sidx, sidx2, D, bfA, bb, ad, k0, kp, p, Wlo, Whi, fblo, fbhi, slow, dg, dleft);
    rd_mf8_block<7, DBG>(A, dcC, sidx, sidx2, D, bfA, bb, ad, k0, kp, p, Wlo, Whi, fblo, fbhi, slow, dg, dleft);
    rd_f4v p0 = rd_lds_read16<0>(ad.rd0);
    rd_mf8_finish<7, DBG>(kp, p, Whi, fbhi, slow);
    {
        rd_lds_wait(p0);
        float t0, t1;
        const float n0 = rd_mf_num(p0.x, p0.y, p0.z, p0.w, t0);
        const float n1 = rd_mf_num(p0.z, p0.w, k0.g0r, k0.g0i, t1);
        if (DBG == 0 || DBG == 3) {
            const float nm = rd_mf_guard(rd_min3abs(k0.nmin, n0, n1), rd_max3abs(k0.tmax, t0, t1));
            if (rd_mf_any(!(nm > RD_MF_C0_MAX))) {
                slow = true;
                float F = rd_max3abs(0.0f, p0.x, p0.y);
                F = rd_max3abs(F, p0.z, p0.w);
                F = rd_max3abs(F, k0.g0r, k0.g0i);
                F = rd_max3abs(F, k0.g1r, k0.g1i);
                F = rd_max3abs(F, k0.g2r, k0.g2i);
                if (!(nm > rd_mf_c0(F))) fblo |= 1u;
            }
        }
        uint32_t b0 = rd_shift_in_sign(0u, n0);
        b0 = rd_shift_in_sign(b0, n1);
        b0 = rd_shift_in_sign(b0, k0.n2);
        b0 = __builtin_amdgcn_alignbit(b0, __builtin_bit_cast(uint32_t, k0.n3), 27);
        Wlo = (b0 << 24) | Wlo;
    }
    const uint32_t Vlo = __builtin_bitreverse32(Wlo & 0xF0F0F0F0u), Vhi = __builtin_bitreverse32(Whi & 0xF0F0F0F0u);
    const auto r = __builtin_amdgcn_permlane32_swap(Vlo, Vhi, false, false);
    word = (r[1] << 4) | r[0];
    fbw = 0;
    if (slow && rd_mf_any((fblo | fbhi) != 0)) {
        const auto f = __builtin_amdgcn_permlane32_swap(fblo, fbhi, false, false);
        fbw = f[0] | f[1];
    }
}

#ifndef RD_MF_LOAD_AUX
#define RD_MF_LOAD_AUX 2
#endif

__device__ __forceinline__ void rd_mf_issue(const rd_layout &lay, uint32_t s, uint32_t ti, uint8_t *img, int lane,
                                            bool halo_dma = true) {
    const uint8_t *src = lay.iq + (size_t)s * lay.stream_stride + (size_t)ti * RD_TILE_BYTES;
    const int perm = 8 * (lane & 7) + (lane >> 3);
    const __attribute__((address_space(1))) void *g0 = (const __attribute__((address_space(1))) void *)(src + perm * 16);
    __builtin_amdgcn_global_load_lds(g0, (__attribute__((address_space(3))) void *)(img + 16), 16, 0, RD_MF_LOAD_AUX);
    __builtin_amdgcn_global_load_lds(g0, (__attribute__((address_space(3))) void *)(img + 16 + 128), 16, 1024, RD_MF_LOAD_AUX);
    __builtin_amdgcn_global_load_lds(g0, (__attribute__((address_space(3))) void *)(img + 16 + 256), 16, 2048, RD_MF_LOAD_AUX);
    __builtin_amdgcn_global_load_lds(g0, (__attribute__((address_space(3))) void *)(img + 16 + 384), 16, 3072, RD_MF_LOAD_AUX);
    const bool has_halo = (ti > 0) || lay.hist_mode;
    if (lane == 0 && halo_dma)
        __builtin_amdgcn_global_load_lds((const __attribute__((address_space(1))) void *)(src + (has_halo ? -16 : 0)),
                                         (__attribute__((address_space(3))) void *)(img), 16, 0, 0);
}

__device__ __forceinline__ int rd_lane_now() {
    return (int)__builtin_amdgcn_mbcnt_hi(~0u, __builtin_amdgcn_mbcnt_lo(~0u, 0u));
}

__device__ __forceinline__ void rd_mf_flush(const uint32_t *pend, uint32_t count, uint32_t *fix_list, uint32_t fix_cap,
                                            uint32_t *counters, uint32_t bits_stride, uint32_t *bucket_cnt) {
    const int lane = rd_lane_now();
    asm volatile("s_waitcnt lgkmcnt(0)" ::: "memory");
    if (bucket_cnt) {
        for (uint32_t i = lane; i < count; i += 64) {
            const uint32_t e = pend[i];
            const uint32_t grp = ((e >> 4) / bits_stride) >> RD_FT_GSH;
            const uint32_t slot = atomicAdd(&bucket_cnt[grp], 1u);
            if (slot < fix_cap) fix_list[(size_t)grp * fix_cap + slot] = e;
        }
        return;
    }
    uint32_t base = 0;
    if (lane == 0) base = atomicAdd(&counters[RD_CNT_FIX], count);
    base = __builtin_amdgcn_readfirstlane(base);
    for (uint32_t i = lane; i < count; i += 64)
        if (base + i < fix_cap) fix_list[base + i] = pend[i];
}


__device__ __forceinline__ void rd_mf_store_staged(uint32_t stage_addr, uint32_t nst, uint32_t *base, uint32_t stflags) {
    const int lane = rd_lane_now();
    if (nst == RD_MF_STAGE_TILES) {
#pragma unroll
        for (int j = 0; j < RD_MF_STAGE_TILES / 4; j++) {
            const rd_u4v v = rd_lds_read16u(stage_addr + 16 * (lane + 64 * j));
            if (!(stflags & 1)) __builtin_nontemporal_store(v, (rd_u4v *)(base + 4 * (lane + 64 * j)));
            else *(rd_u4v *)(base + 4 * (lane + 64 * j)) = v;
        }
    } else {
        for (uint32_t q = 0; q < nst; q++) base[64 * q + lane] = rd_lds_read4(stage_addr + 256 * q + 4 * lane);
    }
}

struct rd_mf_pos {
    uint32_t tile, s, ti, inchunk;
};
struct rd_mf_nextchunk {
    uint32_t tile, s, ti;
};
__device__ __forceinline__ rd_mf_nextchunk rd_mf_chunk_at(uint64_t chunk_id, uint32_t chunk, uint32_t tps, uint32_t total) {
    rd_mf_nextchunk c;
    const uint32_t n_chunks = (total + chunk - 1) / chunk;
    const bool have = chunk_id < n_chunks;
    const uint32_t nt = have ? (uint32_t)chunk_id * chunk : 0u;
    c.tile = have ? nt : 0xFFFFFFFFu;
    c.s = 0; c.ti = 0;
    if (have) {
        c.s = __builtin_amdgcn_readfirstlane(c.tile / tps);
        c.ti = c.tile - c.s * tps;
    }
    return c;
}
__device__ __forceinline__ rd_mf_pos rd_mf_next(rd_mf_pos p, uint32_t chunk, uint32_t tps, const rd_mf_nextchunk &nc) {
    rd_mf_pos q;
    if (p.inchunk + 1 < chunk) {
        q.tile = p.tile + 1; q.inchunk = p.inchunk + 1;
        q.s = p.s; q.ti = p.ti + 1;
        if (q.ti >= tps) { q.ti = 0; q.s++; }
    } else {
        q.tile = nc.tile; q.inchunk = 0;
        q.s = nc.s; q.ti = nc.ti;
    }
    return q;
}

__device__ __forceinline__ void rd_mf_read_window(uint32_t a_prv, uint32_t a_own, rd_u2v (&D)[9]) {
    asm volatile("ds_read_b64 %0, %9\n\t"
                 "ds_read_b64 %1, %10\n\t"
                 "ds_read_b64 %2, %10 offset:128\n\t"
                 "ds_read_b64 %3, %10 offset:256\n\t"
                 "ds_read_b64 %4, %10 offset:384\n\t"
                 "ds_read_b64 %5, %10 offset:512\n\t"
                 "ds_read_b64 %6, %10 offset:640\n\t"
                 "ds_read_b64 %7, %10 offset:768\n\t"
                 "ds_read_b64 %8, %10 offset:896\n\t"
                 "s_waitcnt lgkmcnt(0)"
                 : "=&v"(D[0]), "=&v"(D[1]), "=&v"(D[2]), "=&v"(D[3]), "=&v"(D[4]), "=&v"(D[5]), "=&v"(D[6]),
                   "=&v"(D[7]), "=&v"(D[8])
                 : "v"(a_prv), "v"(a_own)
                 : "memory");
}

__device__ __forceinline__ uint64_t rd_stamp() {
    uint64_t t;
    __builtin_amdgcn_sched_barrier(0);
    asm volatile("s_memtime %0\n\ts_waitcnt lgkmcnt(0)" : "=s"(t) : : "memory");
    __builtin_amdgcn_sched_barrier(0);
    return t;
}
__device__ __forceinline__ uint64_t rd_stamp_real() {
    uint64_t t;
    __builtin_amdgcn_sched_barrier(0);
    asm volatile("s_memrealtime %0\n\ts_waitcnt lgkmcnt(0)" : "=s"(t) : : "memory");
    __builtin_amdgcn_sched_barrier(0);
    return t;
}


#define RD_STAMP_WORDS 12
#define RD_STF_BUCKETS 8192u
template <int DBG, bool STAMP>
__global__ __launch_bounds__(RD_MF_WG, RD_MF_MINWAVES) void k_demod_mfma(rd_layout lay, uint32_t tiles_per_stream, uint32_t total_tiles,
                                                         uint32_t chunk, uint32_t *fix_list, uint32_t fix_cap,
                                                         uint32_t *counters, float *dbg_g, uint32_t stflags) {
    __shared__ __attribute__((aligned(16))) uint8_t s_img[RD_MF_WAVES][RD_MF_IMG_PAD];
    __shared__ __attribute__((aligned(32))) uint8_t s_xb[RD_MF_WAVES][RD_MF_XB_BYTES];
    __shared__ uint32_t s_pend[RD_MF_WAVES][RD_MF_PEND];
    __shared__ __attribute__((aligned(16))) uint32_t s_stage[RD_MF_WAVES][RD_MF_STAGE_TILES][64];
    constexpr bool LOADS = DBG != 1;
    const int lane = threadIdx.x & 63;
    const int wave = __builtin_amdgcn_readfirstlane(threadIdx.x >> 6);
    uint8_t *img0 = s_img[wave];
    uint8_t *xb = s_xb[wave];
    uint32_t *mypend = s_pend[wave];
    uint32_t npend = 0;
    constexpr bool CAN_BUCKET = DBG == 0 && !STAMP;
    uint32_t *bucket_cnt = (CAN_BUCKET && (stflags & RD_STF_BUCKETS)) ? (uint32_t *)dbg_g : nullptr;

    const int n = lane & 31, h = lane >> 5;
    rd_h8 A8[2];
    rd_f16v dcC;
    int sidx = 0, sidx2 = 0;
    if (RD_MF_SPARSE && DBG != 8 && DBG != 9) {
        A8[0] = *(const rd_h8 *)g_mf_taps8s.v[lane];
        A8[1] = *(const rd_h8 *)g_mf_taps8s.v[lane ^ 32];
        sidx = (int)g_mf_taps8s.idx[lane];
        sidx2 = (int)g_mf_taps8s.idx[lane ^ 32];
    } else {
        A8[0] = *(const rd_h8 *)g_mf_taps8.v[0][lane];
        A8[1] = *(const rd_h8 *)g_mf_taps8.v[1][lane];
    }
    const float dchi = -(float)RD_MF_DHI / 16777216.0f;
#pragma unroll
    for (int i = 0; i < 16; i++) dcC[i] = i < 8 ? dchi : 0.0f;
    if (RD_MF_SPARSE && DBG != 8 && DBG != 9) asm volatile("" : "+v"(A8[0]), "+v"(A8[1]), "+v"(sidx), "+v"(sidx2));
    else asm volatile("" : "+v"(A8[0]), "+v"(A8[1]), "+v"(dcC));
    const uint32_t img_addr = rd_lds_addr(img0);
    const uint32_t own = 16 + RD_MF_GROUP_BYTES * (n >> 3) + 16 * (n & 7) + 8 * h;
    const uint32_t prv = n == 0 ? 8 * h
                       : (n & 7) ? own + 16 * 55
                                 : 16 + RD_MF_GROUP_BYTES * ((n >> 3) - 1) + 16 * 63 + 8 * h;
    const uint32_t xb_addr = rd_lds_addr(xb), pend_addr = rd_lds_addr(mypend);
    const uint32_t stage_addr = rd_lds_addr(s_stage[wave]);
    const uint32_t rtoggle = lane == 0 ? 16u : 0u, wtoggle = lane == 63 ? 16u : 0u;
    rd_mf8_addr ad8;
    ad8.xw = xb_addr + 16 * lane;
    ad8.xw7 = xb_addr + (lane == 63 ? 3072 : 1024 + 16 * lane);
    ad8.rd1 = xb_addr + (h ? 1024 + 16 * (lane - 32) : 16 * (lane + 32));
    ad8.rdE = xb_addr + (h ? 2048 + 16 * (lane - 32) : 1024 + 16 * (lane + 32));
    ad8.rdO = xb_addr + (h ? 1024 + 16 * (lane - 32) : 2048 + 16 * (lane + 32));
    ad8.rd0 = xb_addr + (h ? 16 * (lane - 32) : lane ? 1024 + 16 * (lane + 31) : 3072 + 16);
    if (lane < 8) ((uint32_t *)(xb + 3072))[lane] = 0;

    const uint32_t nwaves = gridDim.x * RD_MF_WAVES;
    const uint32_t wave_id = blockIdx.x * RD_MF_WAVES + wave;
    const bool dynamic = !(stflags & 4096) && chunk >= 4;
    uint32_t cur_chunk = wave_id;
    rd_mf_nextchunk nextc = {0xFFFFFFFFu, 0, 0};
    if (!dynamic) nextc = rd_mf_chunk_at((uint64_t)cur_chunk + nwaves, chunk, tiles_per_stream, total_tiles);
    uint32_t grab = 0;
    bool grab_pending = false;
    const uint32_t my_queue = wave_id % RD_NQUEUE;
    uint32_t *queue = &counters[RD_CNT_QUEUE0 + RD_QUEUE_STRIDE * my_queue];
    rd_mf_pos cur;
    cur.tile = wave_id * chunk;
    cur.s = cur.tile / tiles_per_stream;
    cur.ti = cur.tile % tiles_per_stream;
    cur.inchunk = 0;
    rd_mf_pos nx1 = rd_mf_next(cur, chunk, tiles_per_stream, nextc);

    uint32_t nst = 0;
    uint32_t *st_base = nullptr;
    bool st_flush = false;
    uint64_t sm_wait = 0, sm_gap = 0, sm_comp = 0, sm_wait_st = 0, sm_t0 = 0, sm_r0 = 0, sm_mark = 0, sm_wmax = 0;
    uint32_t sm_iters = 0, sm_iters_st = 0;
    bool sm_stored = false;
    if (STAMP) { sm_t0 = rd_stamp(); sm_r0 = rd_stamp_real(); }
    if (LOADS && cur.tile < total_tiles) rd_mf_issue(lay, cur.s, cur.ti, img0, lane);
    if (STAMP) sm_mark = rd_stamp();
    while (cur.tile < total_tiles) {
        const uint32_t tile = cur.tile, s = cur.s, ti = cur.ti, inchunk = cur.inchunk;
        uint64_t sm_a = 0;
        if (STAMP) { sm_a = rd_stamp(); sm_comp += sm_a - sm_mark; }
        asm volatile("s_waitcnt vmcnt(0)" : "+v"(grab) : : "memory");
        uint64_t sm_b = 0;
        if (STAMP) {
            sm_b = rd_stamp();
            const uint64_t w = sm_b - sm_a;
            sm_wait += w;
            if (w > sm_wmax) sm_wmax = w;
            if (sm_stored) { sm_wait_st += w; sm_iters_st++; }
            sm_iters++;
            sm_stored = false;
        }
        if (dynamic) {
            if (grab_pending) {
                nextc = rd_mf_chunk_at((uint64_t)nwaves + my_queue + (uint64_t)RD_NQUEUE * __builtin_amdgcn_readfirstlane(grab),
                                       chunk, tiles_per_stream, total_tiles);
                grab_pending = false;
            }
            if (inchunk == 0) {
                const uint32_t one = 1, zoff = 0;
                uint64_t saved_exec;
                asm volatile("s_mov_b64 %1, exec\n\ts_mov_b64 exec, 1\n\tglobal_atomic_add %0, %2, %3, %4 sc0\n\ts_mov_b64 exec, %1"
                             : "+v"(grab), "=&s"(saved_exec) : "v"(zoff), "v"(one), "s"(queue) : "memory");
                grab_pending = true;
            }
        } else if (inchunk == 0 && tile != wave_id * chunk) {
            cur_chunk += nwaves;
            nextc = rd_mf_chunk_at((uint64_t)cur_chunk + nwaves, chunk, tiles_per_stream, total_tiles);
        }
        if (!(stflags & 4)) __builtin_amdgcn_s_setprio(3);
        rd_u2v D[9];
        rd_mf_read_window(img_addr + prv, img_addr + own, D);
        if (nst == RD_MF_STAGE_TILES || (nst && st_flush)) {
            rd_mf_store_staged(stage_addr, nst, st_base, stflags);
            nst = 0;
            if (STAMP) sm_stored = true;
        }
        const rd_mf_pos nx2 = rd_mf_next(nx1, chunk, tiles_per_stream, nextc);
        bool halo_dma = true;
        {
            const bool follows = nx1.tile < total_tiles && nx1.s == s && nx1.ti == ti + 1;
            if (follows) {
                halo_dma = false;
                if (n == 31) asm volatile("ds_write_b64 %0, %1" : : "v"(img_addr + 8 * h), "v"(D[8]) : "memory");
            }
        }
        if (LOADS && nx1.tile < total_tiles) rd_mf_issue(lay, nx1.s, nx1.ti, img0, lane, halo_dma);
        if (!(stflags & 4)) __builtin_amdgcn_s_setprio(0);
        if (STAMP) { sm_mark = rd_stamp(); sm_gap += sm_mark - sm_b; }

        uint32_t word = 0;
        bool slow_taken = false;
        uint32_t fbw8 = 0;
        if (DBG == 2 || DBG == 6) {
#pragma unroll
            for (int j = 0; j < 9; j++) word ^= D[j].x ^ D[j].y;
        } else {
            float *dg = DBG == 3 ? dbg_g + ((size_t)tile * RD_TILE_SAMPLES + 64 * n + 4 * h + 1) * 2 : nullptr;
            const int dleft = RD_TILE_SAMPLES - (64 * n + 4 * h + 1);
            rd_mf8_tile<DBG>(A8, dcC, sidx, sidx2, D, ad8, word, fbw8, slow_taken, dg, dleft);
            ad8.rd0 ^= rtoggle;
            ad8.xw7 ^= wtoggle;
        }
        uint32_t gmask = 0;
        const bool carry = inchunk > 0 && ti > 0;
        const uint32_t run = ti * 64 + 2 * n + h;
        const uint32_t t0 = run * RD_RUN;
        const bool any_flag = slow_taken && rd_mf_any(fbw8 != 0);
        if (any_flag) gmask = ((fbw8 * 0x00204081u) >> 21) & 0xFu;
        if (!carry && lane == 0) {
            if (ti == 0 && !lay.hist_mode) gmask = 0xFu;
            else gmask |= 1u;
        }
        const bool ragged = (ti + 1 == tiles_per_stream) && (lay.n_samples % RD_TILE_SAMPLES) != 0;
        if (DBG == 6) {
            if (word == 0x12345678u) lay.bits[0] = word;
        } else if (!ragged) {
            if (nst == 0) {
                st_base = &lay.bits[(size_t)s * lay.bits_stride + ti * 64];
                if (stflags & 2) st_base = &lay.bits[(((size_t)s * lay.bits_stride + ti * 64) & 0x3FFFFu) & ~255u];
            }
            rd_lds_write4(stage_addr + 256 * nst + 4 * (2 * n + h), word);
            nst++;
            const bool next_ragged = (nx1.ti + 1 == tiles_per_stream) && (lay.n_samples % RD_TILE_SAMPLES) != 0;
            st_flush = !(nx1.tile < total_tiles && nx1.s == s && nx1.ti == ti + 1 && !next_ragged);
        } else if (t0 < lay.n_samples) {
            const uint32_t left = lay.n_samples - t0;
            if (left < RD_RUN) {
                word &= (1u << left) - 1u;
                gmask &= (1u << ((left + RD_GROUP - 1) / RD_GROUP)) - 1u;
            }
            lay.bits[(size_t)s * lay.bits_stride + run] = word;
        } else {
            gmask = 0;
        }
        if (DBG == 1 || DBG == 2 || DBG == 6) gmask = 0;
        const uint64_t fm = (any_flag || !carry) ? __ballot(gmask != 0) : 0;
        if (fm) {
            static_assert(RD_MF_PEND >= 64, "a tile can list one word per lane");
            const uint32_t nf = (uint32_t)__popcll(fm);
            if (npend + nf > RD_MF_PEND) {
                rd_mf_flush(mypend, npend, fix_list, fix_cap, counters, (uint32_t)lay.bits_stride, bucket_cnt);
                npend = 0;
            }
            if (gmask)
                rd_lds_write4(pend_addr + 4 * (npend + __builtin_amdgcn_mbcnt_hi((uint32_t)(fm >> 32),
                                                                                  __builtin_amdgcn_mbcnt_lo((uint32_t)fm, 0))),
                              ((uint32_t)((size_t)s * lay.bits_stride + run) << 4) | gmask);
            npend += nf;
        }
        cur = nx1;
        nx1 = nx2;
    }
    if (nst) rd_mf_store_staged(stage_addr, nst, st_base, stflags);
    if (npend) rd_mf_flush(mypend, npend, fix_list, fix_cap, counters, (uint32_t)lay.bits_stride, bucket_cnt);
    if (STAMP && dbg_g) {
        const uint64_t t1 = rd_stamp(), r1 = rd_stamp_real();
        sm_comp += t1 - sm_mark;
        if (lane == 0) {
            uint64_t *o = (uint64_t *)dbg_g + (size_t)wave_id * RD_STAMP_WORDS;
            o[0] = sm_wait; o[1] = sm_gap; o[2] = sm_comp; o[3] = sm_wait_st;
            o[4] = sm_iters; o[5] = sm_iters_st; o[6] = t1 - sm_t0; o[7] = r1 - sm_r0;
            o[8] = sm_wmax; o[9] = sm_r0; o[10] = r1;
            uint32_t xcc;
            asm volatile("s_getreg_b32 %0, hwreg(HW_REG_XCC_ID)" : "=s"(xcc));
            o[11] = xcc;
        }
    }
}

static int rd_mf_env(const char *name, int dflt) {
    const char *e = getenv(name);
    return e ? atoi(e) : dflt;
}

struct rd_mf_params {
    int dbg = 0, stamp = 0, chunk_env = 0, per_cu_env = 0, n_cu = 256, test_wgs = 0;
    uint32_t stflags = 0;
    rd_mf_params() {
        chunk_env = rd_mf_env("RD_K1_CHUNK", 0);
        per_cu_env = rd_mf_env("RD_K1_WGS_PER_CU", 0);
        test_wgs = rd_mf_env("RD_TEST_K1_WGS", 0);
        if (test_wgs > 0 && test_wgs < RD_NQUEUE / RD_MF_WAVES) test_wgs = RD_NQUEUE / RD_MF_WAVES;
#ifdef RD_DIAG
        dbg = rd_mf_env("RD_K1_DEBUG", 0);
        stamp = rd_mf_env("RD_K1_STAMPS", 0) ? 1 : 0;
        stflags = (uint32_t)rd_mf_env("RD_K1_STFLAGS", 0) & (1u | 2u | 4u | 4096u);
#endif
        int dev = 0;
        hipDeviceProp_t prop;
        if (hipGetDevice(&dev) == hipSuccess && hipGetDeviceProperties(&prop, dev) == hipSuccess && prop.multiProcessorCount > 0)
            n_cu = prop.multiProcessorCount;
    }
};
static const rd_mf_params &rd_mf_get_params() {
    static const rd_mf_params p;
    return p;
}

#ifdef RD_DIAG
static uint64_t *g_stamp_buf = nullptr;
static uint32_t g_stamp_waves = 0;
extern "C" int rd_diag_read_stamps(uint64_t *out, uint32_t cap_waves, uint32_t *n_waves) {
    if (!g_stamp_buf || !n_waves) return RD_ERR_STATE;
    if (hipDeviceSynchronize() != hipSuccess) return RD_ERR_DEVICE;
    *n_waves = g_stamp_waves;
    const uint32_t n = g_stamp_waves < cap_waves ? g_stamp_waves : cap_waves;
    if (n && hipMemcpy(out, g_stamp_buf, (size_t)n * RD_STAMP_WORDS * 8, hipMemcpyDeviceToHost) != hipSuccess) return RD_ERR_DEVICE;
    return RD_OK;
}
extern "C" int rd_diag_variant(int *dbg, int *stamp, uint32_t *stflags) {
    const rd_mf_params &P = rd_mf_get_params();
    if (dbg) *dbg = P.dbg;
    if (stamp) *stamp = P.stamp;
    if (stflags) *stflags = P.stflags;
    return RD_OK;
}
#endif

struct rd_mf_launch_args {
    rd_layout lay;
    uint32_t tps, total;
    uint64_t total64;
    uint32_t *fix_list, fix_cap, *counters;
    hipStream_t st;
    hipEvent_t ev_start, ev_stop;
    uint32_t *bucket_cnt = nullptr;
    uint32_t *chunk_out = nullptr;
    float *dbg_g;
};

template <int D, bool STAMP>
static bool rd_mf_launch_variant(const rd_mf_launch_args &a) {
    const rd_mf_params &P = rd_mf_get_params();
    static const int per_cu_occ = [] {
        int occ = 0;
        const hipError_t e = hipOccupancyMaxActiveBlocksPerMultiprocessor(&occ, k_demod_mfma<D, STAMP>, RD_MF_WG, 0);
        return (e == hipSuccess && occ >= 1) ? (occ > 8 ? 8 : occ) : 2;
    }();
    const int per_cu = (P.per_cu_env >= 1 && P.per_cu_env <= 8) ? P.per_cu_env : per_cu_occ;
    uint32_t chunk = P.chunk_env > 0 ? (uint32_t)(P.chunk_env < 2 ? 2 : P.chunk_env) : ((P.stflags & 4096) ? 28 : 8);
    if (P.chunk_env <= 0) {
        const uint64_t waves = (uint64_t)P.n_cu * per_cu * RD_MF_WAVES;
        while (chunk > RD_MF_STAGE_TILES && a.total64 / chunk < waves) chunk -= RD_MF_STAGE_TILES;
    }
    if (chunk > a.total) chunk = a.total;
    const uint64_t chunks = (a.total64 + chunk - 1) / chunk;
    uint64_t wgs = (chunks + RD_MF_WAVES - 1) / RD_MF_WAVES;
    uint64_t max_wgs = (uint64_t)P.n_cu * per_cu;
    if (P.test_wgs > 0 && (uint64_t)P.test_wgs < max_wgs) max_wgs = (uint64_t)P.test_wgs;
    if (wgs > max_wgs) wgs = max_wgs;
    {
        const uint64_t nwaves = wgs * RD_MF_WAVES;
        const bool queues = !(P.stflags & 4096) && chunk >= 4;
        if (queues && !(nwaves >= RD_NQUEUE || chunks <= nwaves)) return false;
    }
    float *dbg = a.dbg_g;
    uint32_t stf = P.stflags;
    if (a.bucket_cnt && D == 0 && !STAMP) { dbg = (float *)a.bucket_cnt; stf |= RD_STF_BUCKETS; }
    if (a.chunk_out) { a.chunk_out[0] = chunk; a.chunk_out[1] = (uint32_t)wgs * RD_MF_WAVES; }
#ifdef RD_DIAG
    if (STAMP) {
        const uint32_t nw = (uint32_t)wgs * RD_MF_WAVES;
        if (nw > g_stamp_waves || !g_stamp_buf) {
            if (g_stamp_buf) hipFree(g_stamp_buf);
            g_stamp_buf = nullptr;
            if (hipMalloc(&g_stamp_buf, (size_t)nw * RD_STAMP_WORDS * 8) != hipSuccess) g_stamp_buf = nullptr;
        }
        g_stamp_waves = g_stamp_buf ? nw : 0;
        dbg = (float *)g_stamp_buf;
    }
#endif
    if (a.ev_start || a.ev_stop)
        hipExtLaunchKernelGGL((k_demod_mfma<D, STAMP>), dim3((unsigned)wgs), dim3(RD_MF_WG), 0, a.st, a.ev_start,
                              a.ev_stop, 0, a.lay, a.tps, a.total, chunk, a.fix_list, a.fix_cap, a.counters, dbg, stf);
    else
        hipLaunchKernelGGL((k_demod_mfma<D, STAMP>), dim3((unsigned)wgs), dim3(RD_MF_WG), 0, a.st, a.lay, a.tps, a.total,
                           chunk, a.fix_list, a.fix_cap, a.counters, dbg, stf);
    return true;
}

int rd_launch_demod_mfma(const rd_layout &lay, uint32_t *fix_list, uint32_t fix_cap, uint32_t *counters, hipStream_t st,
                          hipEvent_t ev_start, hipEvent_t ev_stop, float *dbg_g, uint32_t flags, uint32_t *chunk_out,
                          uint32_t *bucket_cnt) {
    rd_mf_launch_args a;
    a.chunk_out = chunk_out;
    a.bucket_cnt = (flags & RD_DEMOD_FIX_BUCKETS) && !dbg_g ? bucket_cnt : nullptr;
    a.lay = lay;
    a.tps = (lay.n_samples + RD_TILE_SAMPLES - 1) / RD_TILE_SAMPLES;
    a.total64 = (uint64_t)lay.n_streams * a.tps;
    if (a.total64 == 0) return a.bucket_cnt != nullptr ? 1 : 0;
    a.total = (uint32_t)a.total64;
    a.fix_list = fix_list; a.fix_cap = fix_cap; a.counters = counters;
    a.st = st; a.ev_start = ev_start; a.ev_stop = ev_stop; a.dbg_g = dbg_g;
    if (dbg_g) {
        return rd_mf_launch_variant<3, false>(a) ? 0 : -1;
    }
#ifdef RD_DIAG
    const rd_mf_params &P = rd_mf_get_params();
    if (P.stamp || P.dbg) {
        a.bucket_cnt = nullptr;
        if (P.stamp && P.dbg == 0) return rd_mf_launch_variant<0, true>(a) ? 0 : -1;
        switch (P.dbg) {
            case 1: return rd_mf_launch_variant<1, false>(a) ? 0 : -1;
            case 2: return rd_mf_launch_variant<2, false>(a) ? 0 : -1;
            case 6: return rd_mf_launch_variant<6, false>(a) ? 0 : -1;
            case 7: return rd_mf_launch_variant<7, false>(a) ? 0 : -1;
            case 8: return rd_mf_launch_variant<8, false>(a) ? 0 : -1;
            case 9: return rd_mf_launch_variant<9, false>(a) ? 0 : -1;
            case 10: return rd_mf_launch_variant<10, false>(a) ? 0 : -1;
            case 11: return rd_mf_launch_variant<11, false>(a) ? 0 : -1;
            default:
                fprintf(stderr, "[rd diag] no kernel variant RD_K1_DEBUG=%d RD_K1_STAMPS=%d is compiled in\n", P.dbg, P.stamp);
                abort();
        }
    }
#endif
    if (!rd_mf_launch_variant<0, false>(a)) return -1;
    return a.bucket_cnt != nullptr ? 1 : 0;
}

static uint32_t g_dbg_launch[2] = {0, 0};
void rd_debug_last_launch(uint32_t out[2]) { out[0] = g_dbg_launch[0]; out[1] = g_dbg_launch[1]; }

extern "C" int rd_debug_demod_mfma(const uint8_t *iq_host, int n_streams, uint32_t n_samples, int hist_mode,
                                   uint32_t hist_bytes, float *g_out, uint32_t *bits_out, uint32_t *fix_out,
                                   uint32_t fix_cap, uint32_t *n_fix) {
    int rc = rd_ensure_device();
    if (rc) return rc;
    const size_t stride = (size_t)n_samples * 2 + (hist_mode ? hist_bytes : 0);
    if (stride % 16 || (hist_mode && hist_bytes % 16)) return RD_ERR_ARG;
    const uint32_t tps = (n_samples + RD_TILE_SAMPLES - 1) / RD_TILE_SAMPLES;
    const size_t words = (n_samples + 31) / 32;
    const size_t iq_bytes = stride * n_streams;
    uint8_t *d_iq = nullptr;
    uint32_t *d_bits = nullptr, *d_fix = nullptr, *d_cnt = nullptr;
    float *d_g = nullptr;
    const size_t g_floats = (size_t)n_streams * tps * RD_TILE_SAMPLES * 2;
#define RD_DBG_CHK(x) do { if ((x) != hipSuccess) { rc = RD_ERR_DEVICE; goto out; } } while (0)
    RD_DBG_CHK(hipMalloc(&d_iq, iq_bytes + RD_INPUT_PAD));
    RD_DBG_CHK(hipMemset(d_iq + iq_bytes, 127, RD_INPUT_PAD));
    RD_DBG_CHK(hipMemcpy(d_iq, iq_host, iq_bytes, hipMemcpyHostToDevice));
    RD_DBG_CHK(hipMalloc(&d_bits, words * n_streams * 4));
    RD_DBG_CHK(hipMemset(d_bits, 0, words * n_streams * 4));
    RD_DBG_CHK(hipMalloc(&d_fix, (size_t)fix_cap * 4 + 4));
    RD_DBG_CHK(hipMalloc(&d_cnt, RD_CNT_TOTAL * 4));
    RD_DBG_CHK(hipMemset(d_cnt, 0, RD_CNT_TOTAL * 4));
    if (g_out) {
        RD_DBG_CHK(hipMalloc(&d_g, g_floats * 4));
        RD_DBG_CHK(hipMemset(d_g, 0, g_floats * 4));
    }
    {
        rd_layout lay;
        lay.iq = d_iq + (hist_mode ? hist_bytes : 0);
        lay.stream_stride = stride;
        lay.n_streams = n_streams;
        lay.n_samples = n_samples;
        lay.hist_mode = hist_mode;
        lay.valid_from = hist_mode ? -(long)(hist_bytes / 2) : 0;
        lay.bits = d_bits;
        lay.bits_stride = words;
        g_dbg_launch[0] = g_dbg_launch[1] = 0;
        if (rd_launch_demod_mfma(lay, d_fix, fix_cap, d_cnt, nullptr, nullptr, nullptr, d_g, 0, g_dbg_launch) < 0) {
            rc = RD_ERR_STATE;
            goto out;
        }
    }
    RD_DBG_CHK(hipDeviceSynchronize());
    if (g_out) RD_DBG_CHK(hipMemcpy(g_out, d_g, g_floats * 4, hipMemcpyDeviceToHost));
    RD_DBG_CHK(hipMemcpy(bits_out, d_bits, words * n_streams * 4, hipMemcpyDeviceToHost));
    {
        uint32_t cnt[RD_CNT_SLOTS];
        RD_DBG_CHK(hipMemcpy(cnt, d_cnt, sizeof cnt, hipMemcpyDeviceToHost));
        *n_fix = cnt[RD_CNT_FIX];
        const uint32_t have = cnt[RD_CNT_FIX] < fix_cap ? cnt[RD_CNT_FIX] : fix_cap;
        if (have) RD_DBG_CHK(hipMemcpy(fix_out, d_fix, (size_t)have * 4, hipMemcpyDeviceToHost));
    }
out:
#undef RD_DBG_CHK
    hipFree(d_iq); hipFree(d_bits); hipFree(d_fix); hipFree(d_cnt); hipFree(d_g);
    return rc;
}
```

rtldavis_amd/csrc/rd_internal.h:

```cpp
#pragma once
#include <hip/hip_runtime.h>
#include <stdint.h>

#include "../../include/rtldavis_hip.h"
#include "rd_hiphost.h"
#include "rd_host.h"
#include "rd_batch_plan.h"

#define RD_DEMOD_FIX_BUCKETS 4u
struct rd_ft_bufs {
    uint32_t *fixb = nullptr;
    uint32_t *fixcnt = nullptr;
    uint32_t fix_bcap = 0;
    uint32_t bcap = 0;
    uint32_t *gstate = nullptr;
};
#define RD_TILE_BYTES 4096
#define RD_INPUT_PAD 8192

struct rd_layout {
    const uint8_t *iq;
    size_t stream_stride;
    int n_streams;
    uint32_t n_samples;
    int hist_mode;
    long valid_from;
    uint32_t *bits;
    size_t bits_stride;
};


struct rd_match {
    int32_t stream;
    int32_t pos;
};

static inline int rd_devcfg_checked(const rd_config *c, rd_devcfg *d) {
    const char *why = "";
    const int rc = rd_make_devcfg(c, d, &why);
    return rc ? rd_fail_msg(rc, "%s", why) : RD_OK;
}

#define RD_DEMOD_REFUSED 0x80000000u
uint32_t rd_launch_demod(const rd_layout &lay, uint32_t *fix_list, uint32_t fix_cap, uint32_t *counters, hipStream_t st,
                         hipEvent_t ev_start = nullptr, hipEvent_t ev_stop = nullptr, uint32_t flags = 0,
                         uint32_t *chunk_out = nullptr, uint32_t *bucket_cnt = nullptr);
int rd_launch_demod_mfma(const rd_layout &lay, uint32_t *fix_list, uint32_t fix_cap, uint32_t *counters, hipStream_t st,
                          hipEvent_t ev_start = nullptr, hipEvent_t ev_stop = nullptr, float *dbg_g = nullptr,
                          uint32_t flags = 0, uint32_t *chunk_out = nullptr, uint32_t *bucket_cnt = nullptr);
void rd_debug_last_launch(uint32_t out[2]);
void rd_launch_fixup(const rd_layout &lay, const uint32_t *fix_list, uint32_t fix_cap, uint32_t *counters, int all,
                     uint32_t *zero_next, hipStream_t st, uint32_t zero_words = RD_CNT_TOTAL, uint64_t expect = 0);
void rd_launch_search(const uint32_t *bits, size_t bits_stride, int n_streams, long n_bits, long p_lo, long p_hi,
                      const rd_devcfg &cfg, rd_match *matches, uint32_t match_cap, uint32_t *counters,
                      hipStream_t st);
int rd_launch_tail_fused(const rd_layout &lay, const rd_devcfg &cfg, int n_calls, long p_lo, long p_hi, const rd_ft_bufs &fb,
                         uint32_t bucket_limit, uint32_t seq, int skip_fix, rd_packet *recs, uint32_t rec_cap, uint32_t *counters,
                         hipStream_t st, hipEvent_t ev_stop = nullptr, uint32_t *zero_next = nullptr, uint32_t zero_words = 0);
int rd_launch_slice(const rd_layout &lay, const uint32_t *bits, size_t bits_stride, long n_bits, const rd_devcfg &cfg,
                     const rd_match *matches, uint32_t match_cap, int batch_mode, int n_calls, int call,
                     rd_packet *recs, rd_packet *recs_host, uint32_t *counters, hipStream_t st,
                     hipEvent_t ev_stop = nullptr, void *tasks = nullptr);
#define RD_TASK_BYTES 16
void rd_launch_parse(const rd_layout &lay, const rd_devcfg &cfg, const rd_packet *recs, uint32_t match_cap,
                     rd_parsed *parsed, uint32_t *counters, hipStream_t st, int dense = 0);
void rd_launch_stream_parse(const rd_layout &lay, const rd_devcfg &cfg, const rd_packet *recs, uint32_t match_cap,
                            int32_t *fe, const uint32_t *counters, hipStream_t st);
struct rd_cplx_layout;
void rd_launch_cplx_stream_parse(const rd_cplx_layout &lay, const rd_devcfg &cfg, const rd_packet *recs, uint32_t match_cap,
                                 int32_t *fe, const uint32_t *counters, hipStream_t st);
void rd_launch_disc(const rd_layout &lay, int stream, long t0, long n, double *out, hipStream_t st);
void rd_launch_filtered(const rd_layout &lay, int stream, long t0, long n, double *out, hipStream_t st);
void rd_launch_window_update(uint32_t *win_out, const uint32_t *win_in, long n_win_bits, const uint32_t *block,
                             long n_block_bits, int n_streams, size_t win_stride, size_t block_stride,
                             hipStream_t st);

#define RD_SB_THREADS 1024
#ifndef RD_SBC_THREADS
#define RD_SBC_THREADS 256
#endif
struct rd_sb_args {
    rd_devcfg cfg;
    uint8_t *ring;
    size_t ring_stride;
    const uint8_t *in;
    const uint32_t *win_in;
    uint32_t *win_out;
    rd_packet *recs_host;
    uint32_t *cnt_host;
    uint32_t *flag_host;
    uint32_t seq;
    long seen_before;
    uint64_t *stamps;
    int parse;
    int32_t *fe_host;
};
int rd_launch_stream_block(const rd_sb_args &a, int n_streams, hipStream_t st);

struct rd_sbc_args {
    rd_devcfg cfg;
    double *ring;
    const void *in;
    int in_is_u8;
    const uint32_t *win_in;
    uint32_t *win_out;
    rd_packet *recs_host;
    uint32_t *cnt_host, *flag_host;
    uint32_t seq;
    long seen_before;
    uint32_t *sync;
    uint64_t *stamps;
    int parse;
    int32_t *fe_host;
};
int rd_launch_stream_block_cplx(const rd_sbc_args &a, hipStream_t st);

struct rd_cplx_layout {
    const double *x;
    long valid_from;
    long n;
};
void rd_launch_cplx_bits(const rd_cplx_layout &lay, uint32_t *bits, hipStream_t st);
void rd_launch_cplx_disc(const rd_cplx_layout &lay, long t0, long n, double *out, hipStream_t st);
void rd_launch_cplx_filtered(const rd_cplx_layout &lay, long t0, long n, double *out, hipStream_t st);
void rd_launch_cplx_slice(const rd_cplx_layout &lay, const uint32_t *bits, long n_bits, const rd_devcfg &cfg,
                          const rd_match *matches, uint32_t match_cap, int call, rd_packet *recs, rd_packet *recs_host,
                          uint32_t *counters, hipStream_t st);
void rd_launch_lut(const uint8_t *in, double *out, size_t n_cplx, hipStream_t st);

void rd_launch_rotate(const double *in, double *out, size_t n, hipStream_t st);
void rd_launch_fir9(const double *in, double *out, size_t n_out, hipStream_t st);
void rd_launch_discriminate(const double *in, double *out, size_t n_out, hipStream_t st);
void rd_launch_quantize(const double *in, uint8_t *out, size_t n, hipStream_t st);
void rd_launch_pack_bytes(const uint8_t *in01, uint32_t *words, size_t n, hipStream_t st);

int rd_chan_stream_prepare(rd_chan *h);
int rd_chan_stream_launch(rd_chan *h, const uint8_t *wide, const uint8_t *prev, size_t n_out, uint64_t t_base, void *dst,
                          size_t dst_stride, hipStream_t st);
int rd_chan_retune(rd_chan *h, const int64_t *rec, int n, int slot, hipStream_t st);
void rd_chan_tuning(const rd_chan *h, const int64_t **shift_hz, const int64_t **phase);
int rd_chan_check_gains(const rd_chan *h, const double *gain, int n);
const float *rd_chan_gains(const rd_chan *h);
int rd_chan_stream_gains(rd_chan *h, const float *gain, int slot, hipStream_t st);
#define RD_LV_ACC_WORDS 8
int rd_chan_stream_levels(rd_chan *h, const uint8_t *wide, size_t n_out, const uint8_t *chan_out, size_t out_stride,
                          uint64_t seq, rd_chan_level *out, rd_input_level *in, uint32_t *acc, hipStream_t st);
#define RD_CF32_CLAMP 8.0f
__device__ __forceinline__ float rd_chan_adm(uint32_t bits) {
    const float v = __builtin_bit_cast(float, bits);
    return v != v ? 0.0f : fminf(fmaxf(v, -RD_CF32_CLAMP), RD_CF32_CLAMP);
}
#define RD_SP_MAX_GROUPS 64
struct rd_spec;
int rd_spec_check(int n_bins, size_t n_samples);
int rd_spec_prepare(rd_spec **sp, int n_bins, size_t n_samples, hipStream_t st);
int rd_spec_launch(rd_spec *sp, const uint8_t *wide, int fmt, size_t n_samples, uint64_t seq, void *out, hipStream_t st);
void rd_spec_destroy(rd_spec *sp);
int rd_bursts_check(size_t n_out);
int rd_bursts_launch(const uint8_t *chan_out, size_t out_stride, int n_ch, size_t n_out, uint64_t seq, void *slot, hipStream_t st);
#define RD_BD_MAX_W 32
#define RD_BD_MAX_LOOK_W 16
#define RD_BD_DATA_BYTES RD_BURST_MSG_BYTES
#define RD_BD_MAX_FLIPS 2
int rd_bd_look_windows(const rd_config *cfg);
int rd_burst_decode_check(const rd_config *cfg);
int rd_burst_decode_launch(const rd_config *cfg, const uint8_t *chan_out, const uint8_t *chan_prev, size_t out_stride, int n_ch,
                           size_t n_out, uint64_t clock, uint64_t seq, int max_flips, const uint32_t *narrow_tab,
                           const void *burst_slot, void *slot, hipStream_t st);
int rd_bd_narrow_upload(int sl, uint32_t **d_tab);
int rd_burst_expect_stage(const rd_config *cfg, int have_prev, uint64_t clock, const rd_expect *e, int n, void *slot_host,
                          uint32_t *cand);
int rd_burst_expect_launch(const rd_config *cfg, const uint8_t *chan_out, const uint8_t *chan_prev, size_t out_stride, int n_ch,
                           size_t n_out, uint64_t clock, uint64_t seq, int n, int max_flips, const uint32_t *narrow_tab,
                           void *slot_dev, hipStream_t st);
int rd_burst_search_launch(const rd_config *cfg, const uint8_t *chan_out, const uint8_t *chan_prev, size_t out_stride, int n_ch,
                           size_t n_out, uint64_t clock, uint64_t seq, const uint8_t *centres, int n, const uint32_t *narrow_tab,
                           void *slot_dev, hipStream_t st);
int rd_burst_quality_launch(const rd_config *cfg, const uint8_t *chan_out, const uint8_t *chan_prev, size_t out_stride, int n_ch,
                            size_t n_out, int noise_gap, const uint32_t *narrow_tab, const rd_burst_msg *recs, size_t cap,
                            const rd_bq_header *hdr, int n_groups, rd_burst_quality *qual, hipStream_t st);
int rd_burst_clips_check(int n_ch, int sources, int pre, int post, int quota);
int rd_burst_clips_launch(const rd_config *cfg, const uint8_t *chan_out, const uint8_t *chan_prev, size_t out_stride, int n_ch,
                          size_t n_out, uint64_t clock, uint64_t seq, int sources, int pre, int post, int quota,
                          const void *burst_slot, const void *decode_slot, const void *expect_slot, int n_expect,
                          const void *search_slot, int n_search, const rd_bc_header *prev_hdr, void *slot, hipStream_t st);
int rd_chan_format(const rd_chan *h);
int rd_chan_n_channels(const rd_chan *h);
int rd_chan_decim(const rd_chan *h);
const float *rd_chan_device_gains(const rd_chan *h);
int64_t rd_chan_out_rate(const rd_chan *h);
int64_t rd_chan_wide_rate(const rd_chan *h);
int rd_chan_bytes_per_sample(const rd_chan *h);
int rd_demod_prepare(rd_demod *h, hipStream_t *st, hipStream_t *st_copy);
int rd_demod_check_room(rd_demod *h);
int rd_demod_submit_device(rd_demod *h, const uint8_t *dev_block);
int rd_demod_pending(const rd_demod *h);
```

rtldavis_amd/csrc/rd_tail.hip:

```cpp
#include "rd_device.h"

#define RD_FT_WG 256
#ifndef RD_FT_DEPTH
#define RD_FT_DEPTH 5
#endif
struct rd_ft_args {
    rd_layout lay;
    rd_devcfg cfg;
    int n_calls;
    int p_hi;
    int skip_fix;
    const uint32_t *fixb;
    const uint32_t *fixcnt;
    uint32_t fix_bcap;
    uint32_t bcap;
    uint32_t bucket_limit;
    uint32_t *gstate;
    uint32_t seq;
    rd_packet *recs;
    uint32_t rec_cap;
    uint32_t *counters;
    uint32_t *zero_next;
    uint32_t zero_words;
    uint64_t *stamps;
    int abl;
};
#define RD_FT_STAMP(k) RD_STAMP(a.stamps && (tid & 63) == 0, a.stamps[(size_t)grp * 8 + (k)])

template <int S_, int T>
__device__ __forceinline__ uint32_t rd_tap(const uint32_t *r, int o) {
    constexpr int wj = (T * S_) >> 5, sh = (T * S_) & 31;
    return sh ? __builtin_amdgcn_alignbit(r[o + wj + 1], r[o + wj], sh) : r[o + wj];
}
constexpr int rd_tt3(bool pa, bool pb, bool pc) { return (pa ? 0xF0 : 0x0F) & (pb ? 0xCC : 0x33) & (pc ? 0xAA : 0x55); }
template <int S_, int P_, uint64_t PRE_, int T>
__device__ __forceinline__ uint32_t rd_match_from(uint32_t m, const uint32_t *r, int o) {
    if constexpr (T >= P_) {
        return m;
    } else if constexpr (T + 1 == P_) {
        const uint32_t v = rd_tap<S_, T>(r, o);
        return __builtin_amdgcn_bitop3_b32(m, v, v, rd_tt3(true, (PRE_ >> T) & 1, (PRE_ >> T) & 1));
    } else {
        const uint32_t n = __builtin_amdgcn_bitop3_b32(m, rd_tap<S_, T>(r, o), rd_tap<S_, T + 1>(r, o),
                                                       rd_tt3(true, (PRE_ >> T) & 1, (PRE_ >> (T + 1)) & 1));
        return rd_match_from<S_, P_, PRE_, T + 2>(n, r, o);
    }
}
template <int S_, int P_, uint64_t PRE_>
__device__ __forceinline__ uint32_t rd_match_word(const uint32_t *r, int o) {
    static_assert(P_ >= 3, "three taps in the first instruction");
    const uint32_t m = __builtin_amdgcn_bitop3_b32(rd_tap<S_, 0>(r, o), rd_tap<S_, 1>(r, o), rd_tap<S_, 2>(r, o),
                                                   rd_tt3(PRE_ & 1, (PRE_ >> 1) & 1, (PRE_ >> 2) & 1));
    return rd_match_from<S_, P_, PRE_, 3>(m, r, o);
}

template <int S_, int P_, uint64_t PRE_, int K_>
__global__ __launch_bounds__(RD_FT_WG, 4) void k_tail(rd_ft_args a) {
    constexpr int G = RD_FT_STREAMS;
    static_assert(PRE_ & 1, "positions below 0 are skipped because the preamble starts with a one");
    static_assert(RD_FT_WG == 64 * G, "one wave per stream in the classify strips");
    extern __shared__ __attribute__((aligned(16))) uint32_t s_dyn[];
    uint32_t *s_t = s_dyn;
    int32_t *s_pos = (int32_t *)(s_dyn + (size_t)G * a.bcap * 8);
    uint32_t *s_ord = s_dyn + (size_t)G * a.bcap * 9;
    __shared__ uint32_t s_cnt[G], s_kept[G];
    __shared__ uint32_t s_ready;
    const int tid = threadIdx.x, lane = tid & 63, wave = __builtin_amdgcn_readfirstlane(tid >> 6);
    const int grp = blockIdx.x, n_groups = gridDim.x;
    const int stream0 = grp * G;
    const int n_here = a.lay.n_streams - stream0 < G ? a.lay.n_streams - stream0 : G;
    const int nwords = (int)((a.lay.n_samples + 31) / 32);
    if (grp == 0 && a.zero_next)
        for (uint32_t i = tid; i < a.zero_words; i += RD_FT_WG) a.zero_next[i] = 0;
    if (tid < G) { s_cnt[tid] = 0; s_kept[tid] = 0; }
    if (tid == 0) s_ready = 0;
    const int prio_q = (int)(((unsigned)grp * 4u) / (unsigned)n_groups);
    if (wave == 0) RD_FT_STAMP(0);

    uint32_t n_fix_raw = 0;
    if (!a.skip_fix) {
        const uint32_t *bk = a.fixb + (size_t)grp * a.fix_bcap;
        const uint32_t e_first = (uint32_t)tid < a.fix_bcap ? bk[tid] : 0u;
        n_fix_raw = a.fixcnt[grp];
        const uint32_t n_fix = n_fix_raw < a.fix_bcap ? n_fix_raw : a.fix_bcap;
        uint32_t *s_items = s_t;
        __shared__ uint32_t s_nitems;
        static_assert(RD_GROUPS == 4, "an entry lists up to four groups");
        for (uint32_t i0 = 0; i0 < n_fix; i0 += RD_FT_WG) {
            if (tid == 0) s_nitems = 0;
            __syncthreads();
            const uint32_t i = i0 + (uint32_t)tid;
            const uint32_t e = i < n_fix ? (i0 == 0 ? e_first : bk[i]) : 0u;
            const uint32_t k = (uint32_t)__popc(e & 0xFu);
            if (k) {
                uint32_t at = atomicAdd(&s_nitems, k);
                for (int g = 0; g < RD_GROUPS; g++)
                    if ((e >> g) & 1) s_items[at++] = ((uint32_t)tid << 2) | (uint32_t)g;
                s_items[4 * RD_FT_WG + tid] = e;
            }
            __syncthreads();
            const uint32_t n_items = s_nitems;
            for (uint32_t it = (uint32_t)tid; it < n_items; it += RD_FT_WG) {
                const uint32_t item = s_items[it];
                const uint32_t ee = s_items[4 * RD_FT_WG + (item >> 2)];
                const int g = (int)(item & 3u);
                const uint32_t widx = ee >> 4;
                const uint32_t s = widx / (uint32_t)a.lay.bits_stride;
                const uint32_t run = widx - s * (uint32_t)a.lay.bits_stride;
                const uint8_t *base = rd_view_of(a.lay, s).base;
                const long t0 = (long)run * RD_RUN + g * RD_GROUP;
                const long left = (long)a.lay.n_samples - t0;
                if (left <= 0) continue;
                const int count = left < RD_GROUP ? (int)left : RD_GROUP;
                const uint8_t *p = base + 2 * (t0 - 10);
                uint32_t dw[10];
                const long x = a.lay.valid_from - (t0 - 10), z = (long)a.lay.n_samples + 8 - (t0 - 10);
                const int d_lo = x <= 0 ? 0 : x >= 20 ? 10 : (int)(x / 2);
                const int d_hi = z <= 0 ? 0 : z >= 20 ? 10 : (int)((z + 1) / 2);
#pragma unroll
                for (int d = 0; d < 10; d++) dw[d] = (d >= d_lo && d < d_hi) ? *(const uint32_t *)(p + 4 * d) : 0u;
                ((uint8_t *)a.lay.bits)[(size_t)widx * 4 + g] = (uint8_t)rd_exact_group_dw(dw, t0, count, a.lay.valid_from);
            }
            if (i0 + RD_FT_WG < n_fix) __syncthreads();
        }
    }
    __syncthreads();
    if (wave == 0) RD_FT_STAMP(1);

    {
        constexpr int NW = ((RD_SEARCH_OUT + ((P_ - 1) * S_ + 31) / 32 + 1 + 3) / 4) * 4;
        const int gps = a.p_hi / (32 * RD_SEARCH_OUT) + 1;
        const int wgps = (gps + 63) / 64;
        const int units = n_here * wgps;
        auto fetch = [&](int g, int rem, uint32_t (&r)[NW]) {
            const int gi = rem * 64 + lane;
            const uint32_t *w = a.lay.bits + (size_t)(stream0 + g) * a.lay.bits_stride;
            int w0 = RD_SEARCH_OUT * gi;
            w0 = w0 + NW <= nwords ? w0 : nwords - NW;
#pragma unroll
            for (int j = 0; j < NW / 4; j++) {
                const uint4 v4 = *(const uint4 *)(w + w0 + 4 * j);
                r[4 * j] = v4.x; r[4 * j + 1] = v4.y; r[4 * j + 2] = v4.z; r[4 * j + 3] = v4.w;
            }
        };
        auto test = [&](int g, int rem, const uint32_t (&r)[NW]) {
            const int gi = rem * 64 + lane;
            uint32_t m[RD_SEARCH_OUT] = {};
            const int p0 = 32 * RD_SEARCH_OUT * gi;
            if (gi < gps) {
#pragma unroll
                for (int o = 0; o < RD_SEARCH_OUT; o++) m[o] = rd_match_word<S_, P_, PRE_>(r, o);
                if (p0 + 32 * RD_SEARCH_OUT - 1 > a.p_hi) {
#pragma unroll
                    for (int o = 0; o < RD_SEARCH_OUT; o++) {
                        const int q0 = p0 + 32 * o;
                        if (q0 + 31 > a.p_hi) m[o] &= (a.p_hi < q0) ? 0u : (0xFFFFFFFFu >> (31 - (a.p_hi - q0)));
                    }
                }
            }
            uint32_t anym = 0;
#pragma unroll
            for (int o = 0; o < RD_SEARCH_OUT; o++) anym |= m[o];
            if (__ballot(anym != 0)) {
                uint32_t mine = 0;
#pragma unroll
                for (int o = 0; o < RD_SEARCH_OUT; o++) mine += (uint32_t)__popc(m[o]);
                uint32_t incl = mine;
#pragma unroll
                for (int sh = 1; sh < 64; sh <<= 1) {
                    const uint32_t up = (uint32_t)__shfl_up((int)incl, sh, 64);
                    if (lane >= sh) incl += up;
                }
                const uint32_t tot = (uint32_t)__shfl((int)incl, 63, 64);
                uint32_t slot0 = 0;
                if (lane == 0) slot0 = atomicAdd(&s_cnt[g], tot);
                uint32_t slot = (uint32_t)__builtin_amdgcn_readfirstlane((int)slot0) + incl - mine;
#pragma unroll
                for (int o = 0; o < RD_SEARCH_OUT; o++) {
                    uint32_t mm = m[o];
                    while (mm) {
                        const int bpos = __builtin_ctz(mm);
                        mm &= mm - 1;
                        if (slot < a.bcap) s_pos[(size_t)g * a.bcap + slot] = p0 + 32 * o + bpos;
                        slot++;
                    }
                }
            }
        };
        constexpr int DEPTH = RD_FT_DEPTH;
        uint32_t rb[DEPTH][NW];
        const int dq = G / wgps, dr = G % wgps;
        int fg = wave / wgps, fr = wave % wgps, fu = wave;
        int tg = fg, tr = fr, prio_k = 0;
        auto step = [&](int &gg, int &rr) { gg += dq; rr += dr; if (rr >= wgps) { rr -= wgps; gg++; } };
        auto fetch_next = [&](uint32_t (&r)[NW]) {
#ifdef RD_DIAG
            if (a.abl & 2) return;
#endif
            fetch(fg, fr, r);
            if (fu + G < units) { fu += G; step(fg, fr); }
        };
        auto test_next = [&](const uint32_t (&r)[NW]) {
#ifdef RD_DIAG
            if (a.abl & 1) { if (r[0] == 0x12345678u) s_cnt[0] = 1; step(tg, tr); return; }
#endif
            switch ((prio_q + prio_k++) & 3) {
                case 0: __builtin_amdgcn_s_setprio(0); break;
                case 1: __builtin_amdgcn_s_setprio(1); break;
                case 2: __builtin_amdgcn_s_setprio(2); break;
                default: __builtin_amdgcn_s_setprio(3); break;
            }
            test(tg, tr, r);
            step(tg, tr);
        };
        if (wave < units) {
#pragma unroll
            for (int j = 0; j < DEPTH - 1; j++) fetch_next(rb[j]);
            for (int u = wave; u < units; u += DEPTH * G) {
#pragma unroll
                for (int j = 0; j < DEPTH; j++) {
                    if (u + j * G < units) {
                        fetch_next(rb[(j + DEPTH - 1) % DEPTH]);
                        test_next(rb[j]);
                    }
                }
            }
        }
    }
    __builtin_amdgcn_s_setprio(0);
    if (wave == 0) RD_FT_STAMP(6);
    rd_barrier_lds();
    if (wave == 0) RD_FT_STAMP(2);

    constexpr int NBITS = (K_ - 1) * S_ + 1;
    constexpr int NU = (NBITS + 31) / 32;
    constexpr int NWS = NU + 1;
    static_assert(K_ % 8 == 0 && (K_ + 7) / 8 <= 12 && NWS <= 36, "packet bytes fit a task entry");
    const int g = wave;
    const int stream = stream0 + g;
    const uint32_t nmatch = g < n_here ? s_cnt[g] : 0u;
    const bool ovf = nmatch > a.bucket_limit;
    const uint32_t count = ovf ? 0u : nmatch;
    uint32_t *tg = s_t + (size_t)g * a.bcap * 8;
    const int B = a.cfg.B, L = a.cfg.L;
    for (uint32_t j = lane; j < count; j += 64) {
        const int pos = s_pos[(size_t)g * a.bcap + j];
        const uint32_t *w = a.lay.bits + (size_t)stream * a.lay.bits_stride;
        const int wi0 = pos >> 5;
        const uint32_t sh = (uint32_t)(pos & 31);
        uint32_t W[NWS];
#pragma unroll
        for (int i = 0; i < NWS; i++) W[i] = (wi0 + i < nwords) ? w[wi0 + i] : 0u;
        const uint32_t pl = (uint32_t)(pos + L), bq = pl / (uint32_t)B, br = pl - bq * (uint32_t)B;
        const int b0 = (int)bq - 1;
        const int q0 = pos - ((b0 + 1) * B - L);
        const bool ok0 = b0 >= 0 && b0 < a.n_calls;
        const int b1 = b0 - 1, q1 = q0 + B;
        const bool ok1 = br == 0 && b1 >= 0 && b1 < a.n_calls;
        uint32_t uu[NU];
#pragma unroll
        for (int i = 0; i < NU; i++) uu[i] = __builtin_amdgcn_alignbit(W[i + 1], W[i], sh);
        uint32_t dw[3] = {0, 0, 0};
#pragma unroll
        for (int k = 0; k < K_; k++) {
            const int bit = k * S_, bi = k >> 3;
            const uint32_t b = (uu[bit >> 5] >> (bit & 31)) & 1u;
            dw[bi >> 2] |= b << (8 * (bi & 3) + 7 - (k & 7));
        }
        const uint32_t ph0 = (uint32_t)q0 % (uint32_t)S_, ph1 = (uint32_t)q1 % (uint32_t)S_;
        uint4 *e = (uint4 *)(tg + 8 * j);
        e[0] = uint4{(ok0 ? 1u : 0u) | (ok1 ? 2u : 0u), (uint32_t)b0, (ph0 << 24) | (uint32_t)q0, (ph1 << 24) | (uint32_t)q1};
        e[1] = uint4{dw[0], dw[1], dw[2], 0u};
    }
    if (wave == 0) RD_FT_STAMP(7);
    for (uint32_t j = lane; j < ((count + 63) & ~63u); j += 64) {
        const bool live = j < count;
        const uint4 me = live ? *(const uint4 *)(tg + 8 * j) : uint4{0, 0, 0, 0};
        const uint4 md = live ? *(const uint4 *)(tg + 8 * j + 4) : uint4{0, 0, 0, 0};
        const int b0 = (int)me.y, b1 = b0 - 1;
        const uint32_t k0 = me.z, k1 = me.w;
        bool dup0 = false, dup1 = false;
        for (uint32_t i0 = 0; i0 < count; i0 += 4) {
            uint4 xa[4], da[4];
#pragma unroll
            for (int u = 0; u < 4; u++) {
                const uint32_t i = (i0 + u) < a.bcap ? i0 + u : i0;
                xa[u] = *(const uint4 *)(tg + 8 * i);
                da[u] = *(const uint4 *)(tg + 8 * i + 4);
            }
#pragma unroll
            for (int u = 0; u < 4; u++) {
                const uint32_t i = i0 + u;
                const uint4 x = xa[u], d = da[u];
                const int ob0 = (int)x.y;
                const bool lower = i < j;
                if (i < count && d.x == md.x && d.y == md.y && d.z == md.z) {
                    if ((x.x & 1u) && ob0 == b0 && (x.z < k0 || (x.z == k0 && lower))) dup0 = true;
                    if ((x.x & 2u) && ob0 - 1 == b0 && (x.w < k0 || (x.w == k0 && lower))) dup0 = true;
                    if ((x.x & 1u) && ob0 == b1 && (x.z < k1 || (x.z == k1 && lower))) dup1 = true;
                    if ((x.x & 2u) && ob0 - 1 == b1 && (x.w < k1 || (x.w == k1 && lower))) dup1 = true;
                }
            }
        }
        if (live) tg[8 * j + 7] = (((me.x & 1u) && !dup0) ? 1u : 0u) | (((me.x & 2u) && !dup1) ? 2u : 0u);
    }
    uint32_t kept_here = 0;
    for (uint32_t j = lane; j < ((count + 63) & ~63u); j += 64) {
        const bool live = j < count;
        const uint4 me = live ? *(const uint4 *)(tg + 8 * j) : uint4{0, 0, 0, 0};
        const uint32_t mk = live ? tg[8 * j + 7] : 0u;
        const int b0 = (int)me.y, b1 = b0 - 1;
        const uint32_t k0 = me.z, k1 = me.w;
        uint32_t r0 = 0, r1 = 0;
        for (uint32_t i0 = 0; i0 < count; i0 += 4) {
            uint4 xa[4];
            uint32_t ka[4];
#pragma unroll
            for (int u = 0; u < 4; u++) {
                const uint32_t i = (i0 + u) < a.bcap ? i0 + u : i0;
                xa[u] = *(const uint4 *)(tg + 8 * i);
                ka[u] = tg[8 * i + 7];
            }
#pragma unroll
            for (int u = 0; u < 4; u++) {
                const uint4 x = xa[u];
                const uint32_t xk = (i0 + u) < count ? ka[u] & 3u : 0u;
                const int ob0 = (int)x.y;
                auto before = [](int ca, uint32_t ka_, int cb, uint32_t kb) { return ca < cb || (ca == cb && ka_ < kb); };
                if (xk & 1u) { r0 += before(ob0, x.z, b0, k0) ? 1u : 0u; r1 += before(ob0, x.z, b1, k1) ? 1u : 0u; }
                if (xk & 2u) { r0 += before(ob0 - 1, x.w, b0, k0) ? 1u : 0u; r1 += before(ob0 - 1, x.w, b1, k1) ? 1u : 0u; }
            }
        }
        kept_here += (uint32_t)__popcll(__ballot((mk & 1u) != 0)) + (uint32_t)__popcll(__ballot((mk & 2u) != 0));
        if (live) tg[8 * j + 7] = mk | (r0 << 2) | (r1 << 17);
    }
    if (lane == 0) s_kept[g] = kept_here;
    if (ovf && lane == 0) atomicOr(&a.counters[RD_CNT_OVF], 1u);
    rd_barrier_lds();
    uint32_t off = 0, total = 0, mtotal = 0;
#pragma unroll
    for (int i = 0; i < G; i++) {
        off += i < g ? s_kept[i] : 0u;
        total += s_kept[i];
        mtotal += i < n_here ? s_cnt[i] : 0u;
    }
    for (uint32_t j = lane; j < count; j += 64) {
        const uint32_t res = tg[8 * j + 7];
        if (res & 1u) s_ord[off + ((res >> 2) & 0x7FFFu)] = ((uint32_t)g << 16) | (j << 1);
        if (res & 2u) s_ord[off + (res >> 17)] = ((uint32_t)g << 16) | (j << 1) | 1u;
    }
    const uint32_t tag = (a.seq & 0xFFFu) << 20;
    if (tid == 0) {
        __hip_atomic_store(&a.gstate[n_groups + grp], tag | (mtotal < 0xFFFFFu ? mtotal : 0xFFFFFu), __ATOMIC_RELAXED, __HIP_MEMORY_SCOPE_AGENT);
        __hip_atomic_store(&a.gstate[2 * n_groups + grp], tag | (n_fix_raw < 0xFFFFFu ? n_fix_raw : 0xFFFFFu), __ATOMIC_RELAXED,
                           __HIP_MEMORY_SCOPE_AGENT);
        __hip_atomic_store(&a.gstate[grp], tag | total, __ATOMIC_RELAXED, __HIP_MEMORY_SCOPE_AGENT);
        if (n_fix_raw > a.fix_bcap) atomicOr(&a.counters[RD_CNT_OVF], 8u);
    }
    rd_barrier_lds();
    if (wave == 0) RD_FT_STAMP(3);

    if (wave == G - 1) {
        uint32_t polls = 0;
        bool gave_up = false;
        auto tagged = [&](const uint32_t *p) -> uint32_t {
            for (;;) {
                const uint32_t v = __hip_atomic_load(p, __ATOMIC_RELAXED, __HIP_MEMORY_SCOPE_AGENT);
                if ((v & 0xFFF00000u) == tag) return v & 0xFFFFFu;
                if (++polls > (1u << 22)) { gave_up = true; return 0u; }
                __builtin_amdgcn_s_sleep(8);
            }
        };
        uint32_t sum = 0;
        for (int j0 = 0; j0 < grp; j0 += 1024) {
            uint32_t v[16];
#pragma unroll
            for (int k = 0; k < 16; k++) {
                const int j = j0 + lane + 64 * k;
                v[k] = j < grp ? __hip_atomic_load(&a.gstate[j], __ATOMIC_RELAXED, __HIP_MEMORY_SCOPE_AGENT) : tag;
            }
#pragma unroll
            for (int k = 0; k < 16; k++) {
                if ((v[k] & 0xFFF00000u) != tag) v[k] = tag | tagged(&a.gstate[j0 + lane + 64 * k]);
                sum += v[k] & 0xFFFFFu;
            }
        }
#pragma unroll
        for (int o = 32; o > 0; o >>= 1) sum += (uint32_t)__shfl_xor((int)sum, o, 64);
        if (lane == 0) __hip_atomic_store(&s_ready, sum + 1u, __ATOMIC_RELAXED, __HIP_MEMORY_SCOPE_WORKGROUP);
        if (grp == n_groups - 1) {
            uint32_t mt = 0, ft = 0;
            for (int i0 = 0; i0 < n_groups; i0 += 512) {
                uint32_t vm[8], vf[8];
#pragma unroll
                for (int k = 0; k < 8; k++) {
                    const int i = i0 + lane + 64 * k;
                    vm[k] = i < n_groups ? __hip_atomic_load(&a.gstate[n_groups + i], __ATOMIC_RELAXED, __HIP_MEMORY_SCOPE_AGENT) : tag;
                    vf[k] = i < n_groups ? __hip_atomic_load(&a.gstate[2 * n_groups + i], __ATOMIC_RELAXED, __HIP_MEMORY_SCOPE_AGENT) : tag;
                }
#pragma unroll
                for (int k = 0; k < 8; k++) {
                    const int i = i0 + lane + 64 * k;
                    if ((vm[k] & 0xFFF00000u) != tag) vm[k] = tagged(&a.gstate[n_groups + i]);
                    if ((vf[k] & 0xFFF00000u) != tag) vf[k] = tagged(&a.gstate[2 * n_groups + i]);
                    mt += vm[k] & 0xFFFFFu;
                    ft += vf[k] & 0xFFFFFu;
                }
            }
#pragma unroll
            for (int o = 32; o > 0; o >>= 1) {
                mt += (uint32_t)__shfl_xor((int)mt, o, 64);
                ft += (uint32_t)__shfl_xor((int)ft, o, 64);
            }
            if (lane == 0) {
                a.counters[RD_CNT_TASKS] = sum + total;
                a.counters[RD_CNT_MATCH] = mt;
                a.counters[RD_CNT_FIX] = ft;
                if (sum + total > a.rec_cap) atomicOr(&a.counters[RD_CNT_OVF], 2u);
            }
        }
        if (__ballot(gave_up) && lane == 0) atomicOr(&a.counters[RD_CNT_OVF], 16u);
        RD_FT_STAMP(4);
    }
    float *s_res = (float *)(s_dyn + (size_t)G * a.bcap * 11);
    if ((uint32_t)wave < total) {
        rd_k_h8 Ahi[3], Alo[3];
#pragma unroll
        for (int d = 0; d < 3; d++) {
            Ahi[d] = *(const rd_k_h8 *)g_rssi_taps.v[0][d][lane];
            Alo[d] = *(const rd_k_h8 *)g_rssi_taps.v[1][d][lane];
        }
        struct task { int stream, call, q; };
        auto task_at = [&](uint32_t r) {
            const uint32_t o = s_ord[r];
            const uint32_t *e = s_t + ((size_t)(o >> 16) * a.bcap + ((o >> 1) & 0x7FFFu)) * 8;
            task t;
            t.stream = stream0 + (int)(o >> 16);
            t.call = (int)e[1] - (int)(o & 1u);
            t.q = (int)(e[2] & 0xFFFFFFu) + ((o & 1u) ? B : 0);
            return t;
        };
        auto view = [&](int s) { return rd_view_of(a.lay, s); };
        auto job_of = [&](const task &t) {
            return rd_rssi_prepare(view(__builtin_amdgcn_readfirstlane(t.stream)), __builtin_amdgcn_readfirstlane(t.call) * B, a.cfg,
                                   __builtin_amdgcn_readfirstlane(t.q), lane);
        };
        task t_cur = task_at((uint32_t)wave);
        rd_rssi_job j_cur = job_of(t_cur);
        rd_rssi_data d_cur = {};
        if (j_cur.ok) d_cur = rd_rssi_fetch(j_cur);
        for (uint32_t r = (uint32_t)wave; r < total; r += G) {
            const task t_now = t_cur;
            const rd_rssi_job j_now = j_cur;
            const rd_rssi_data d_now = d_cur;
            if (r + G < total) {
                t_cur = task_at(r + G);
                j_cur = job_of(t_cur);
                if (j_cur.ok) d_cur = rd_rssi_fetch(j_cur);
            }
            double rssi = 0.0, snr = 0.0;
            if (j_now.ok) {
                float noise, sig;
                rd_rssi_block(j_now, d_now, Ahi, Alo, lane, noise, sig);
                rd_rssi_finish(noise, sig, j_now.ns, j_now.pe, j_now.q, lane, rssi, snr);
            } else {
                rd_rssi_u8(view(__builtin_amdgcn_readfirstlane(t_now.stream)), (long)__builtin_amdgcn_readfirstlane(t_now.call) * B, a.cfg,
                           (long)__builtin_amdgcn_readfirstlane(t_now.q), lane, rssi, snr);
            }
            if (lane == 0) { s_res[2 * r] = (float)rssi; s_res[2 * r + 1] = (float)snr; }
        }
    }
    rd_barrier_lds();
    if ((uint32_t)tid < total) {
        uint32_t spins = 0, v = 0;
        while (!(v = __hip_atomic_load(&s_ready, __ATOMIC_RELAXED, __HIP_MEMORY_SCOPE_WORKGROUP)) && ++spins < (1u << 24))
            __builtin_amdgcn_s_sleep(2);
        const uint32_t first = v - 1u;
        for (uint32_t r = (uint32_t)tid; r < total; r += RD_FT_WG) {
            const uint32_t o = s_ord[r];
            const uint32_t *e = s_t + ((size_t)(o >> 16) * a.bcap + ((o >> 1) & 0x7FFFu)) * 8;
            const uint4 x = *(const uint4 *)e, d = *(const uint4 *)(e + 4);
            const uint32_t at = first + r;
            if (at < a.rec_cap) {
                const double rssi = (double)s_res[2 * r], snr = (double)s_res[2 * r + 1];
                uint4 *out = (uint4 *)&a.recs[at];
                out[0] = uint4{(uint32_t)(stream0 + (int)(o >> 16)), (uint32_t)((int)x.y - (int)(o & 1u)),
                               (uint32_t)((int)(x.z & 0xFFFFFFu) + ((o & 1u) ? B : 0)), (uint32_t)a.cfg.nbytes};
                out[1] = uint4{d.x, d.y, d.z, 0u};
                out[2] = uint4{0u, 0u, 0u, 0u};
                const uint2 rb = __builtin_bit_cast(uint2, rssi), sb = __builtin_bit_cast(uint2, snr);
                out[3] = uint4{rb.x, rb.y, sb.x, sb.y};
            }
        }
    }
    if (wave == 0) RD_FT_STAMP(5);
}

#ifdef RD_DIAG
static uint64_t *g_ft_stamps = nullptr;
static uint32_t g_ft_groups = 0;
extern "C" int rd_diag_read_tail_stamps(uint64_t *out, uint32_t cap_groups, uint32_t *n_groups) {
    if (!g_ft_stamps || !n_groups) return RD_ERR_STATE;
    if (hipDeviceSynchronize() != hipSuccess) return RD_ERR_DEVICE;
    *n_groups = g_ft_groups;
    const uint32_t n = g_ft_groups < cap_groups ? g_ft_groups : cap_groups;
    if (n && hipMemcpy(out, g_ft_stamps, (size_t)n * 64, hipMemcpyDeviceToHost) != hipSuccess) return RD_ERR_DEVICE;
    return RD_OK;
}
#endif

size_t rd_tail_fused_lds(uint32_t bcap) { return (size_t)RD_FT_STREAMS * bcap * (8 + 1 + 2 + 4) * sizeof(uint32_t); }

int rd_launch_tail_fused(const rd_layout &lay, const rd_devcfg &cfg, int n_calls, long p_lo, long p_hi, const rd_ft_bufs &fb,
                         uint32_t bucket_limit, uint32_t seq, int skip_fix, rd_packet *recs, uint32_t rec_cap, uint32_t *counters,
                         hipStream_t st, hipEvent_t ev_stop, uint32_t *zero_next, uint32_t zero_words) {
    const long n_bits = lay.n_samples;
    if (!rd_davis_shape(cfg) || n_bits >= (1l << 30) || cfg.B >= (1 << 24) ||
        lay.n_streams <= 0 || p_lo > 0 || p_hi < 0 || p_hi >= (1l << 30) || !fb.gstate || !fb.fixb || fb.bcap == 0 || fb.bcap % 32 ||
        fb.bcap > RD_BUCKET_MAX || lay.bits_stride % 4 || ((size_t)lay.bits % 16) || lay.hist_mode ||
        p_hi / 32 + 16 > (n_bits + 31) / 32)
        return 0;
    rd_ft_args a;
    a.lay = lay; a.cfg = cfg; a.n_calls = n_calls; a.p_hi = (int)p_hi; a.skip_fix = skip_fix;
    a.fixb = fb.fixb; a.fixcnt = fb.fixcnt; a.fix_bcap = fb.fix_bcap;
    a.bcap = fb.bcap; a.bucket_limit = bucket_limit < fb.bcap ? bucket_limit : fb.bcap;
    a.gstate = fb.gstate; a.seq = seq;
    a.recs = recs; a.rec_cap = rec_cap; a.counters = counters; a.zero_next = zero_next; a.zero_words = zero_words;
    a.stamps = nullptr;
    a.abl = 0;
    const uint32_t groups = (uint32_t)(lay.n_streams + RD_FT_STREAMS - 1) / RD_FT_STREAMS;
#ifdef RD_DIAG
    if (const char *e = getenv("RD_FT_ABL")) a.abl = atoi(e);
    if (getenv("RD_FT_STAMPS")) {
        if (groups > g_ft_groups) { if (g_ft_stamps) hipFree(g_ft_stamps); g_ft_stamps = nullptr; if (hipMalloc(&g_ft_stamps, (size_t)groups * 64) != hipSuccess) g_ft_stamps = nullptr; }
        g_ft_groups = g_ft_stamps ? groups : 0;
        a.stamps = g_ft_stamps;
    }
#endif
    const size_t lds = std::max<size_t>(rd_tail_fused_lds(fb.bcap), 33 * 1024);
    static bool attr_set = false;
    if (lds > 48 * 1024) rd_allow_lds((const void *)k_tail<14, 16, 0x91D3ull, 80>, 150 * 1024, attr_set);
    rd_launch_ev(k_tail<14, 16, 0x91D3ull, 80>, dim3(groups), dim3(RD_FT_WG), lds, st, ev_stop, a);
    return 1;
}
```

rtldavis_amd/csrc/rd_tail_kernels.hip:

```cpp
#include "rd_device.h"

uint32_t rd_launch_demod(const rd_layout &lay, uint32_t *fix_list, uint32_t fix_cap, uint32_t *counters, hipStream_t st,
                         hipEvent_t ev_start, hipEvent_t ev_stop, uint32_t flags, uint32_t *chunk_out, uint32_t *bucket_cnt) {
    if (!bucket_cnt) flags &= ~RD_DEMOD_FIX_BUCKETS;
    const int bucketed = rd_launch_demod_mfma(lay, fix_list, fix_cap, counters, st, ev_start, ev_stop, nullptr, flags, chunk_out, bucket_cnt);
    if (bucketed < 0) return RD_DEMOD_REFUSED;
    return bucketed ? RD_DEMOD_FIX_BUCKETS : 0u;
}

__global__ __launch_bounds__(256) void k_fixup(rd_layout lay, uint32_t runs_per_stream, const uint32_t *fix_list,
                                               uint32_t fix_cap, const uint32_t *counters, int all,
                                               uint32_t *zero_next, uint32_t zero_words) {
    if (zero_next && blockIdx.x == 0)
        for (uint32_t i = threadIdx.x; i < zero_words; i += blockDim.x) zero_next[i] = 0;
    uint64_t count;
    if (all) {
        count = (uint64_t)lay.n_streams * runs_per_stream;
    } else {
        count = counters[RD_CNT_FIX];
        if (count > fix_cap) count = fix_cap;
    }
    const uint64_t stride = (uint64_t)gridDim.x * blockDim.x;
    for (uint64_t i = (uint64_t)blockIdx.x * blockDim.x + threadIdx.x; i < count; i += stride) {
        if (all) {
            const uint32_t s = (uint32_t)(i / runs_per_stream);
            const uint32_t run = (uint32_t)(i - (uint64_t)s * runs_per_stream);
            const long t0 = (long)run * RD_RUN;
            const long left = (long)lay.n_samples - t0;
            lay.bits[(size_t)s * lay.bits_stride + run] = rd_exact_run(rd_view_of(lay, s), t0, left < RD_RUN ? (int)left : RD_RUN);
        } else {
            const uint32_t e = fix_list[i];
            const uint32_t widx = e >> 4;
            const uint32_t s = widx / (uint32_t)lay.bits_stride;
            const uint32_t run = widx - s * (uint32_t)lay.bits_stride;
            const rd_stream_view v = rd_view_of(lay, s);
            for (int g = 0; g < RD_GROUPS; g++) {
                if (!((e >> g) & 1)) continue;
                const long t0 = (long)run * RD_RUN + g * RD_GROUP;
                const long left = (long)lay.n_samples - t0;
                if (left <= 0) break;
                const int count = left < RD_GROUP ? (int)left : RD_GROUP;
                const uint8_t *p = v.base + 2 * (t0 - 10);
                uint32_t dw[10];
                const long x = v.valid_from - (t0 - 10), z = (long)lay.n_samples + 8 - (t0 - 10);
                const int d_lo = x <= 0 ? 0 : x >= 20 ? 10 : (int)(x / 2);
                const int d_hi = z <= 0 ? 0 : z >= 20 ? 10 : (int)((z + 1) / 2);
#pragma unroll
                for (int d = 0; d < 10; d++) dw[d] = (d >= d_lo && d < d_hi) ? *(const uint32_t *)(p + 4 * d) : 0u;
                ((uint8_t *)lay.bits)[(size_t)widx * 4 + g] = (uint8_t)rd_exact_group_dw(dw, t0, count, v.valid_from);
            }
        }
    }
}

void rd_launch_fixup(const rd_layout &lay, const uint32_t *fix_list, uint32_t fix_cap, uint32_t *counters, int all,
                     uint32_t *zero_next, hipStream_t st, uint32_t zero_words, uint64_t expect) {
    const uint32_t rps = (lay.n_samples + RD_RUN - 1) / RD_RUN;
    if (rps == 0 || lay.n_streams == 0) return;
    uint64_t want = all ? (uint64_t)lay.n_streams * rps : fix_cap;
    if (!all && expect > 0) want = std::min<uint64_t>(want, std::max<uint64_t>(expect + expect / 4, 256 * 256));
    uint64_t wgs = (want + 255) / 256;
    if (wgs > 256ull * 16) wgs = 256ull * 16;
    if (wgs == 0) wgs = 1;
    hipLaunchKernelGGL(k_fixup, dim3((unsigned)wgs), dim3(256), 0, st, lay, rps, fix_list, fix_cap, counters, all,
                       zero_next, zero_words);
}


#define RD_MATCH_PEND 128
#define RD_SEARCH_WAVES 4
#ifndef RD_SEARCH_UNROLL
#define RD_SEARCH_UNROLL 2
#endif

__device__ __forceinline__ void rd_flush_matches(const rd_match *pend, uint32_t count, rd_match *matches,
                                                 uint32_t match_cap, uint32_t *counters, int lane) {
    asm volatile("s_waitcnt lgkmcnt(0)" ::: "memory");
    uint32_t base = 0;
    if (lane == 0) base = atomicAdd(&counters[RD_CNT_MATCH], count);
    base = __builtin_amdgcn_readfirstlane(base);
    for (uint32_t i = lane; i < count; i += 64)
        if (base + i < match_cap) matches[base + i] = pend[i];
}

template <int S_, int P_, uint64_t PRE_>
__global__ __launch_bounds__(64 * RD_SEARCH_WAVES) void k_search(const uint32_t *bits, size_t bits_stride, int n_streams, long nwords,
                                                long base, long groups_per_stream, long p_lo, long p_hi,
                                                rd_devcfg cfg, rd_match *matches, uint32_t match_cap,
                                                uint32_t *counters) {
    __shared__ rd_match pend_all[RD_SEARCH_WAVES][RD_MATCH_PEND];
    const int lane = threadIdx.x & 63;
    rd_match *pend = pend_all[threadIdx.x >> 6];
    uint32_t npend = 0;
    const uint32_t wgps = (uint32_t)((groups_per_stream + 63) / 64);
    const uint32_t nwave_groups = (uint32_t)n_streams * wgps;
    const uint32_t nwaves = gridDim.x * RD_SEARCH_WAVES;
    const uint32_t wave0 = __builtin_amdgcn_readfirstlane(blockIdx.x * RD_SEARCH_WAVES + (threadIdx.x >> 6));
    constexpr int NW = S_ > 0 ? ((RD_SEARCH_OUT + ((P_ > 0 ? P_ - 1 : 0) * (S_ > 0 ? S_ : 1) + 31) / 32 + 1 + 3) / 4) * 4 : 4;
    const int nwords_i = (int)nwords, gps = (int)groups_per_stream, plo = (int)p_lo, phi = (int)p_hi;
    const int base_i = (int)base, base_w = (int)(base >> 5);
    const bool aligned16 = (bits_stride % 4 == 0) && (base_w % 4 == 0) && ((size_t)bits % 16 == 0);
    const uint32_t dq_n = nwaves / wgps, dr_n = nwaves % wgps;
    uint32_t s0 = wave0 / wgps, rem0 = wave0 % wgps;
    for (uint32_t wg0 = wave0; wg0 < nwave_groups; wg0 += nwaves * RD_SEARCH_UNROLL) {
        uint32_t r[RD_SEARCH_UNROLL][NW];
        uint32_t su[RD_SEARCH_UNROLL], remu[RD_SEARCH_UNROLL];
        {
            uint32_t sx = s0, rx = rem0;
#pragma unroll
            for (int u = 0; u < RD_SEARCH_UNROLL; u++) {
                su[u] = sx; remu[u] = rx;
                sx += dq_n; rx += dr_n;
                if (rx >= wgps) { rx -= wgps; sx++; }
            }
            s0 = sx; rem0 = rx;
        }
        if constexpr (S_ > 0) {
#pragma unroll
            for (int u = 0; u < RD_SEARCH_UNROLL; u++) {
                const uint32_t wg = wg0 + u * nwaves;
                if (wg >= nwave_groups) break;
                const int gi = (int)remu[u] * 64 + lane;
                const uint32_t *w = bits + (size_t)su[u] * bits_stride;
                const int w0 = base_w + RD_SEARCH_OUT * gi;
                if (aligned16 && gi < gps && w0 >= 0 && w0 + NW <= nwords_i) {
#pragma unroll
                    for (int j = 0; j < NW / 4; j++) {
                        const uint4 v4 = *(const uint4 *)(w + w0 + 4 * j);
                        r[u][4 * j] = v4.x; r[u][4 * j + 1] = v4.y; r[u][4 * j + 2] = v4.z; r[u][4 * j + 3] = v4.w;
                    }
                } else {
#pragma unroll
                    for (int j = 0; j < NW; j++) r[u][j] = gi < gps ? rd_word_at(w, nwords, (long)w0 + j) : 0u;
                }
            }
        }
#pragma unroll
        for (int u = 0; u < RD_SEARCH_UNROLL; u++) {
            const uint32_t wg = wg0 + u * nwaves;
            if (wg >= nwave_groups) break;
            const uint32_t s = su[u];
            const int gi = (int)remu[u] * 64 + lane;
            uint32_t m[RD_SEARCH_OUT] = {};
            int p0 = 0;
            if (gi < gps) {
                p0 = base_i + 32 * RD_SEARCH_OUT * gi;
                const uint32_t *w = bits + (size_t)s * bits_stride;
#pragma unroll
                for (int o = 0; o < RD_SEARCH_OUT; o++) m[o] = 0xFFFFFFFFu;
                if constexpr (S_ > 0) {
                    uint32_t any[RD_SEARCH_OUT] = {};
                    uint32_t held[RD_SEARCH_OUT];
                    bool have_held = false;
#pragma unroll
                    for (int k = 0; k < P_; k++) {
                        const int wj = (k * S_) >> 5, sh = (k * S_) & 31;
                        const bool one = (PRE_ >> k) & 1;
#pragma unroll
                        for (int o = 0; o < RD_SEARCH_OUT; o++) {
                            const uint32_t v = sh ? __builtin_amdgcn_alignbit(r[u][o + wj + 1], r[u][o + wj], sh) : r[u][o + wj];
                            if (one) m[o] &= v;
                            else if (have_held) any[o] = any[o] | held[o] | v;
                            else held[o] = v;
                        }
                        if (!one) have_held = !have_held;
                    }
#pragma unroll
                    for (int o = 0; o < RD_SEARCH_OUT; o++) {
                        if (have_held) any[o] |= held[o];
                        m[o] &= ~any[o];
                    }
                } else {
                    for (int k = 0; k < cfg.P; k++) {
                        const uint32_t x = ((cfg.pre_mask >> k) & 1) ? 0u : 0xFFFFFFFFu;
#pragma unroll
                        for (int o = 0; o < RD_SEARCH_OUT; o++)
                            m[o] &= rd_bits32_at(w, nwords, (long)p0 + 32 * o + (long)k * cfg.S) ^ x;
                    }
                }
                if (p0 < plo || p0 + 32 * RD_SEARCH_OUT - 1 > phi) {
#pragma unroll
                    for (int o = 0; o < RD_SEARCH_OUT; o++) {
                        const int q0 = p0 + 32 * o;
                        if (q0 < plo) m[o] &= (plo - q0 >= 32) ? 0u : (0xFFFFFFFFu << (plo - q0));
                        if (q0 + 31 > phi) m[o] &= (phi < q0) ? 0u : (0xFFFFFFFFu >> (31 - (phi - q0)));
                    }
                }
            }
#pragma unroll
            for (int o = 0; o < RD_SEARCH_OUT; o++) {
                uint32_t mm = m[o];
                uint64_t any = __ballot(mm != 0);
                while (any) {
                    const uint32_t nf = (uint32_t)__popcll(any);
                    if (npend + nf > RD_MATCH_PEND) {
                        rd_flush_matches(pend, npend, matches, match_cap, counters, lane);
                        npend = 0;
                    }
                    if (mm) {
                        const int bpos = __builtin_ctz(mm);
                        mm &= mm - 1;
                        rd_match e;
                        e.stream = (int32_t)s;
                        e.pos = (int32_t)(p0 + 32 * o + bpos);
                        pend[npend + __builtin_amdgcn_mbcnt_hi((uint32_t)(any >> 32),
                                                               __builtin_amdgcn_mbcnt_lo((uint32_t)any, 0))] = e;
                    }
                    npend += nf;
                    any = __ballot(mm != 0);
                }
            }
        }
    }
    __shared__ uint32_t left[RD_SEARCH_WAVES + 1];
    if (lane == 0) left[threadIdx.x >> 6] = npend;
    __syncthreads();
    if ((threadIdx.x >> 6) == 0) {
        const uint32_t mine = lane < RD_SEARCH_WAVES ? left[lane] : 0u;
        uint32_t incl = mine;
#pragma unroll
        for (int o = 1; o < RD_SEARCH_WAVES; o <<= 1) {
            const uint32_t up = __shfl_up(incl, o, 64);
            if (lane >= o) incl += up;
        }
        const uint32_t tot = __shfl(incl, RD_SEARCH_WAVES - 1, 64);
        if (tot) {
            uint32_t base_slot = 0;
            if (lane == 0) base_slot = atomicAdd(&counters[RD_CNT_MATCH], tot);
            base_slot = __builtin_amdgcn_readfirstlane(base_slot);
#pragma unroll 1
            for (int wv = 0; wv < RD_SEARCH_WAVES; wv++) {
                const uint32_t n = __shfl(mine, wv, 64), off = __shfl(incl - mine, wv, 64);
                for (uint32_t i = lane; i < n; i += 64)
                    if (base_slot + off + i < match_cap) matches[base_slot + off + i] = pend_all[wv][i];
            }
        }
    }
}

static int rd_search_wgs_per_cu() {
    static const int cap = [] {
        const char *e = getenv("RD_K2_WGS_PER_CU");
        const int v = e ? atoi(e) : 32 / 4;
        return (v < 1 || v > 64) ? 32 / 4 : v;
    }();
    return cap;
}

void rd_launch_search(const uint32_t *bits, size_t bits_stride, int n_streams, long n_bits, long p_lo, long p_hi,
                      const rd_devcfg &cfg, rd_match *matches, uint32_t match_cap, uint32_t *counters,
                      hipStream_t st) {
    if (p_hi < p_lo || n_streams == 0) return;
    const long base = (p_lo >> 5) << 5;
    const long nwords = (n_bits + 31) / 32;
    const long groups = (p_hi - base) / (32 * RD_SEARCH_OUT) + 1;
    const uint64_t total = (uint64_t)n_streams * groups;
    uint64_t wgs = (total + 64 * RD_SEARCH_WAVES - 1) / (64 * RD_SEARCH_WAVES);
    const int cap = rd_search_wgs_per_cu();
    if (wgs > 256ull * cap) wgs = 256ull * cap;
    if (rd_davis_search(cfg))
        hipLaunchKernelGGL((k_search<14, 16, 0x91D3ull>), dim3((unsigned)wgs), dim3(64 * RD_SEARCH_WAVES), 0, st, bits, bits_stride,
                           n_streams, nwords, base, groups, p_lo, p_hi, cfg, matches, match_cap, counters);
    else
        hipLaunchKernelGGL((k_search<0, 0, 0>), dim3((unsigned)wgs), dim3(64 * RD_SEARCH_WAVES), 0, st, bits, bits_stride, n_streams,
                           nwords, base, groups, p_lo, p_hi, cfg, matches, match_cap, counters);
}

struct rd_task {
    uint32_t rec;
    int32_t stream;
    int32_t call;
    int32_t q;
};

template <int S_, int K_>
__global__ __launch_bounds__(256) void k_classify(const uint32_t *bits, size_t bits_stride, int nwords, rd_devcfg cfg,
                                                  const rd_match *matches, uint32_t match_cap, int n_calls,
                                                  rd_packet *recs, rd_task *tasks, uint32_t *counters) {
    constexpr int NBITS = (K_ - 1) * S_ + 3;
    constexpr int NU = (NBITS + 31) / 32;
    constexpr int NW = NU + 1;
    constexpr int NBYTES = (K_ + 7) / 8;
    static_assert(K_ % 8 == 0 && NBYTES <= RD_MAX_PKT_BYTES, "whole bytes only");
    __shared__ uint32_t s_tot[4], s_base;
    const int lane = threadIdx.x & 63;
    uint32_t count = counters[RD_CNT_MATCH];
    if (count > match_cap) count = match_cap;
    const uint32_t nthreads = gridDim.x * blockDim.x;
    for (uint32_t g0 = blockIdx.x * blockDim.x; g0 < count; g0 += nthreads) {
        const uint32_t i = g0 + threadIdx.x;
        const bool live = i < count;
        int stream = 0, pos = 0;
        if (live) { stream = matches[i].stream; pos = matches[i].pos; }
        const uint32_t pl = (uint32_t)(pos + cfg.L), bq = pl / (uint32_t)cfg.B, br = pl - bq * (uint32_t)cfg.B;
        const int b0 = (int)bq - 1;
        const int q0 = pos - ((b0 + 1) * cfg.B - cfg.L);
        const bool ok0 = live && b0 >= 0 && b0 < n_calls;
        const int b1 = b0 - 1, q1 = q0 + cfg.B;
        const bool ok1 = live && br == 0 && b1 >= 0 && b1 < n_calls;
        const uint32_t *w = bits + (size_t)stream * bits_stride;
        const int o = pos - 1, wi0 = o >> 5;
        const uint32_t sh = (uint32_t)(o & 31);
        uint32_t W[NW];
#pragma unroll
        for (int j = 0; j < NW; j++) {
            const int wi = wi0 + j;
            W[j] = (live && wi >= 0 && wi < nwords) ? w[wi] : 0u;
        }
        uint32_t u[NU];
#pragma unroll
        for (int j = 0; j < NU; j++) u[j] = __builtin_amdgcn_alignbit(W[j + 1], W[j], sh);
        uint32_t dprev = 0, dnext = 0;
#pragma unroll
        for (int j = 0; j < NU; j++) {
            const uint32_t nxt = j + 1 < NU ? u[j + 1] : 0u;
            const uint32_t y = u[j] ^ __builtin_amdgcn_alignbit(nxt, u[j], 1);
            uint32_t mp = 0, mn = 0;
#pragma unroll
            for (int k = 0; k < K_; k++) {
                if (((k * S_) >> 5) == j) mp |= 1u << ((k * S_) & 31);
                if (((k * S_ + 1) >> 5) == j) mn |= 1u << ((k * S_ + 1) & 31);
            }
            dprev |= y & mp;
            dnext |= y & mn;
        }
        const bool same_prev = dprev == 0, same_next = dnext == 0;
        uint32_t dw[(NBYTES + 3) / 4];
#pragma unroll
        for (int m = 0; m < (NBYTES + 3) / 4; m++) dw[m] = 0;
#pragma unroll
        for (int k = 0; k < K_; k++) {
            const int bit = k * S_ + 1, bi = k >> 3;
            const uint32_t b = (u[bit >> 5] >> (bit & 31)) & 1u;
            dw[bi >> 2] |= b << (8 * (bi & 3) + 7 - (k & 7));
        }
        auto superseded = [&](int q) { return RD_SUPERSEDED(S_, q, cfg.B, same_prev, same_next); };
        const bool use0 = ok0 && !superseded(q0), use1 = ok1 && !superseded(q1);
        const int ntask = (use0 ? 1 : 0) + (use1 ? 1 : 0);
        const uint32_t incl = rd_wave_incl_scan_u32((uint32_t)ntask, lane);
        const uint32_t tot = __shfl(incl, 63, 64);
        const int wv = threadIdx.x >> 6;
        __syncthreads();
        if (lane == 0) s_tot[wv] = tot;
        __syncthreads();
        if (threadIdx.x == 0) {
            uint32_t sum = 0;
#pragma unroll
            for (int k = 0; k < 4; k++) sum += s_tot[k];
            s_base = sum ? atomicAdd(&counters[RD_CNT_TASKS], sum) : 0u;
        }
        __syncthreads();
        uint32_t base = s_base;
#pragma unroll
        for (int k = 0; k < 4; k++) base += k < wv ? s_tot[k] : 0u;
        base = __builtin_amdgcn_readfirstlane(base);
        if (ntask) {
            uint32_t t = base + incl - (uint32_t)ntask;
            const int pb = use0 ? b0 : b1, pq = use0 ? q0 : q1;
            auto put = [&](uint32_t ri, int call, int q) {
                uint32_t *r = (uint32_t *)&recs[ri];
                const uint4 hdr = {(uint32_t)stream, (uint32_t)call, (uint32_t)q, (uint32_t)NBYTES};
                *(uint4 *)r = hdr;
                uint32_t d8[RD_MAX_PKT_BYTES / 4];
#pragma unroll
                for (int m = 0; m < RD_MAX_PKT_BYTES / 4; m++) d8[m] = m < (NBYTES + 3) / 4 ? dw[m] : 0u;
#pragma unroll
                for (int m = 0; m < RD_MAX_PKT_BYTES / 16; m++)
                    *(uint4 *)(r + 4 + 4 * m) = uint4{d8[4 * m], d8[4 * m + 1], d8[4 * m + 2], d8[4 * m + 3]};
                const rd_task tk = {ri, stream, call, q};
                tasks[t++] = tk;
            };
            put(t, pb, pq);
            if (use0 && use1) put(t, b1, q1);
        }
    }
}

__global__ __launch_bounds__(256) void k_rssi_u8(rd_layout lay, rd_devcfg cfg, const rd_task *tasks, uint32_t task_cap,
                                                 rd_packet *recs, const uint32_t *counters) {
    const int lane = threadIdx.x & 63;
    const uint32_t nw = gridDim.x * (blockDim.x >> 6);
    const uint32_t i0 = blockIdx.x * (blockDim.x >> 6) + (threadIdx.x >> 6);
    rd_k_h8 Ahi[3], Alo[3];
#pragma unroll
    for (int d = 0; d < 3; d++) {
        Ahi[d] = *(const rd_k_h8 *)g_rssi_taps.v[0][d][lane];
        Alo[d] = *(const rd_k_h8 *)g_rssi_taps.v[1][d][lane];
    }
    rd_task t_cur = {0, 0, 0, 0}, t_nxt = {0, 0, 0, 0};
    if (i0 < task_cap) t_cur = tasks[i0];
    if (i0 + nw < task_cap) t_nxt = tasks[i0 + nw];
    uint32_t count = counters[RD_CNT_TASKS];
    if (count > task_cap) count = task_cap;
    auto view = [&](int stream) { return rd_view_of(lay, stream); };
    auto job_of = [&](const rd_task &t) {
        const int stream = __builtin_amdgcn_readfirstlane(t.stream), call = __builtin_amdgcn_readfirstlane(t.call),
                  q = __builtin_amdgcn_readfirstlane(t.q);
        return rd_rssi_prepare(view(stream), call * cfg.B, cfg, q, lane);
    };
    rd_rssi_job j_cur = {};
    rd_rssi_data d_cur = {};
    if (i0 < count) {
        j_cur = job_of(t_cur);
        if (j_cur.ok) d_cur = rd_rssi_fetch(j_cur);
    }
    for (uint32_t i = i0; i < count; i += nw) {
        const rd_task t_now = t_cur;
        const rd_rssi_job j_now = j_cur;
        const rd_rssi_data d_now = d_cur;
        if (i + nw < count) {
            j_cur = job_of(t_nxt);
            if (j_cur.ok) d_cur = rd_rssi_fetch(j_cur);
        }
        t_cur = t_nxt;
        if (i + 2 * nw < task_cap) t_nxt = tasks[i + 2 * nw];
        const uint32_t rec = __builtin_amdgcn_readfirstlane(t_now.rec);
        double rssi = 0.0, snr = 0.0;
        if (j_now.ok) {
            float noise, sig;
            rd_rssi_block(j_now, d_now, Ahi, Alo, lane, noise, sig);
            rd_rssi_finish(noise, sig, j_now.ns, j_now.pe, j_now.q, lane, rssi, snr);
        } else {
            const int stream = __builtin_amdgcn_readfirstlane(t_now.stream);
            rd_rssi_u8(view(stream), (long)__builtin_amdgcn_readfirstlane(t_now.call) * cfg.B, cfg,
                       (long)__builtin_amdgcn_readfirstlane(t_now.q), lane, rssi, snr);
        }
        if (lane == 0) { recs[rec].rssi = rssi; recs[rec].snr = snr; }
    }
}

int rd_launch_slice(const rd_layout &lay, const uint32_t *bits, size_t bits_stride, long n_bits, const rd_devcfg &cfg,
                    const rd_match *matches, uint32_t match_cap, int batch_mode, int n_calls, int call,
                    rd_packet *recs, rd_packet *recs_host, uint32_t *counters, hipStream_t st, hipEvent_t ev_stop,
                    void *tasks) {
    rd_u8_src src;
    src.lay = lay;
    if (tasks && batch_mode && recs && !recs_host && rd_davis_slice(cfg) && n_bits < (1l << 30)) {
        const uint32_t cg = std::min<uint32_t>((match_cap + 255) / 256, 1024);
        hipLaunchKernelGGL((k_classify<14, 80>), dim3(cg ? cg : 1), dim3(256), 0, st, bits, bits_stride,
                           (int)((n_bits + 31) / 32), cfg, matches, match_cap, n_calls, recs, (rd_task *)tasks, counters);
        const uint32_t rg = std::min<uint32_t>(rd_slice_grid(match_cap), 1024);
        rd_launch_ev(k_rssi_u8, dim3(rg), dim3(256), 0, st, ev_stop, lay, cfg, (const rd_task *)tasks, 2 * match_cap, recs, counters);
        return 1;
    }
    rd_launch_ev(k_slice_rssi<rd_u8_src>, dim3(rd_slice_grid(match_cap)), dim3(256), 0, st, ev_stop, src, bits, bits_stride,
                 (n_bits + 31) / 32, cfg, matches, match_cap, batch_mode, n_calls, call, recs, recs_host, counters);
    return 0;
}

template <int S_, int P_, uint64_t PRE_, int K_>
__global__ __launch_bounds__(RD_SB_THREADS) void k_stream_block(rd_sb_args a) {
    extern __shared__ __attribute__((aligned(16))) uint8_t sb_lds[];
    const int B = a.cfg.B, nwin = (2 * B) / 32, nbw = B / 32;
    uint8_t *s_iq = sb_lds;
    uint32_t *s_win = (uint32_t *)(sb_lds + 32 + 2 * (size_t)B);
    int32_t *s_match = (int32_t *)(s_win + nwin);
    __shared__ uint32_t s_nm;
    const int tid = threadIdx.x, lane = tid & 63, wave = tid >> 6;
    const int stream = blockIdx.x;
    uint8_t *ring = a.ring + (size_t)stream * a.ring_stride;
    const uint8_t *in = a.in + (size_t)stream * 2 * (size_t)B;
    const bool have_hist = a.seen_before > 0;
    RD_SB_STAMP(0);
    if (tid == 0) s_nm = 0;
    const int pieces = (2 * B) / 16;
    uint4 nw[2], oc[2], ph = {0, 0, 0, 0};
#pragma unroll
    for (int k = 0; k < 2; k++) {
        const int i = tid + RD_SB_THREADS * k;
        nw[k] = uint4{0, 0, 0, 0}; oc[k] = uint4{0, 0, 0, 0};
        if (i < pieces) {
            nw[k] = *(const uint4 *)(in + 16 * (size_t)i);
            if (have_hist) oc[k] = *(const uint4 *)(ring + 32 + 2 * (size_t)B + 16 * (size_t)i);
        }
    }
    if (have_hist && tid < 2) ph = *(const uint4 *)(ring + 2 * (size_t)B + 16 * (size_t)tid);
    const uint32_t *win_in = a.win_in + (size_t)stream * nwin;
    uint32_t *win_out = a.win_out + (size_t)stream * nwin;
    uint32_t oldw = 0;
    if (tid < nbw) oldw = win_in[nbw + tid];
    __syncthreads();
    RD_SB_STAMP(1);
#pragma unroll
    for (int k = 0; k < 2; k++) {
        const int i = tid + RD_SB_THREADS * k;
        if (i < pieces) {
            *(uint4 *)(ring + 32 + 2 * (size_t)B + 16 * (size_t)i) = nw[k];
            *(uint4 *)(s_iq + 32 + 16 * (size_t)i) = nw[k];
            if (have_hist) {
                *(uint4 *)(ring + 32 + 16 * (size_t)i) = oc[k];
                if (i >= pieces - 2) *(uint4 *)(s_iq + 16 * (i - (pieces - 2))) = oc[k];
            }
        }
    }
    if (have_hist && tid < 2) *(uint4 *)(ring + 16 * (size_t)tid) = ph;
    if (!have_hist && tid < 2) *(uint4 *)(s_iq + 16 * tid) = uint4{0, 0, 0, 0};
    if (tid < nbw) s_win[tid] = oldw;
    rd_barrier_lds();
    RD_SB_STAMP(2);
    const long vfrom = have_hist ? -16 : 0;
    for (int g = tid; g < B / 8; g += RD_SB_THREADS) {
        const int t0 = 8 * g;
        uint32_t dw[10];
#pragma unroll
        for (int d = 0; d < 10; d++) {
            const int smp = t0 - 10 + 2 * d;
            dw[d] = (smp + 1 >= -16 && smp + 1 < B) ? *(const uint32_t *)(s_iq + 32 + 2 * smp) : 0u;
        }
        ((uint8_t *)(s_win + nbw))[g] = (uint8_t)rd_exact_group_dw(dw, (long)t0, 8, vfrom);
    }
    __syncthreads();
    RD_SB_STAMP(3);
    for (int i = tid; i < nwin; i += RD_SB_THREADS) win_out[i] = s_win[i];
    rd_window_search<S_, P_, PRE_>(s_win, nwin, nbw, tid, RD_SB_THREADS, &s_nm, s_match);
    __syncthreads();
    RD_SB_STAMP(4);
    const uint32_t nm = s_nm;
    rd_packet *recs = a.recs_host + (size_t)stream * (size_t)(B + 1);
    int32_t *fe = a.fe_host + (size_t)stream * (size_t)(B + 1);
    rd_stream_view v;
    v.base = ring + 32 + 2 * (size_t)B;
    v.valid_from = RD_SB_VALID_FROM(a.seen_before, B);
    v.n = B;
    {
        __builtin_amdgcn_fence(__ATOMIC_RELEASE, "workgroup");
        for (uint32_t i = (uint32_t)wave; i < nm; i += RD_SB_THREADS / 64) {
            const int pos = __builtin_amdgcn_readfirstlane(s_match[i]);
            uint32_t byte = 0;
            bool same_prev = true, same_next = true;
#define RD_BITS3(o) rd_lds_bits32(s_win, nwin, (o))
            RD_WAVE_BYTES(K_, S_, pos, lane, RD_BITS3, byte, same_prev, same_next);
#undef RD_BITS3
            const bool superseded = RD_SUPERSEDED(S_, pos, B, same_prev, same_next);
            if (superseded) {
                rd_store_void(nullptr, &recs[i], lane);
                if (a.parse && lane == 0) fe[i] = RD_FE_NONE;
                continue;
            }
            double rssi = 0.0, snr = 0.0;
            rd_rssi_u8(v, 0, a.cfg, (long)pos, lane, rssi, snr);
            rd_store_record(nullptr, &recs[i], lane, stream, (long)a.seen_before, (long)pos, a.cfg.nbytes, byte, rssi, snr);
            if (a.parse) {
                const int32_t e = rd_wave_parse(v, a.cfg, (long)pos, byte, lane);
                if (lane == 0) fe[i] = e;
            }
        }
    }
    __syncthreads();
    if (tid == 0) {
        a.cnt_host[stream] = nm;
        __builtin_amdgcn_fence(__ATOMIC_RELEASE, "");
        __hip_atomic_store(&a.flag_host[stream], a.seq, __ATOMIC_RELAXED, __HIP_MEMORY_SCOPE_SYSTEM);
    }
    RD_SB_STAMP(5);
}

int rd_launch_stream_block(const rd_sb_args &a_in, int n_streams, hipStream_t st) {
    const rd_devcfg &c = a_in.cfg;
    if (!rd_davis_shape(c) || c.L != 2 * c.B || c.B % 32 || c.B < 2048 || c.B > 16384)
        return 0;
    rd_sb_args a = a_in;
    a.stamps = nullptr;
#ifdef RD_DIAG
    a.stamps = rd_sb_stamp_buffer();
#endif
    const size_t lds = 32 + 2 * (size_t)c.B + (size_t)(2 * c.B / 32) * 4 + ((size_t)c.B + 1) * 4;
    hipLaunchKernelGGL((k_stream_block<14, 16, 0x91D3ull, 80>), dim3((unsigned)n_streams), dim3(RD_SB_THREADS), lds, st, a);
    return 1;
}
```

Before: 2.119 million MS/s.

## Run the fused tail on a shared side stream overlapping the next demod

Adds a per-device non-blocking side stream that runs the one-launch tail kernel, ordered by an event after demod, so a tail can overlap the next run's demod on the main stream. A SIDE variant of k_tail uses smaller LDS, a shallower prefetch depth, higher occupancy, a leaner exact-bit group function and lazy tap loads. When another handle shares the device and the previous run used the side tail, the demod grid gives up some workgroups so the tail can co-reside. This adds cross-handle synchronisation (settling before input rewrites) and may shrink the demod grid.

```diff
diff --git a/include/rtldavis_hip.h b/include/rtldavis_hip.h
--- a/include/rtldavis_hip.h
+++ b/include/rtldavis_hip.h
@@ -107,6 +107,7 @@
 #define RD_FORM_ORDERED_TAIL 1u
 #define RD_FORM_SECOND_PASS 8u
 #define RD_FORM_ONE_LAUNCH_TAIL 16u
+#define RD_FORM_SIDE_TAIL 32u
 int rd_batch_last_run_forms(rd_batch *b, uint32_t *forms);
 int rd_batch_get_counters(rd_batch *b, uint64_t *fixup_runs, uint64_t *matches);
 int rd_k1_schedule(rd_batch *b, uint32_t *tiles_per_chunk, uint32_t *waves);
diff --git a/rtldavis_amd/batch.py b/rtldavis_amd/batch.py
--- a/rtldavis_amd/batch.py
+++ b/rtldavis_amd/batch.py
@@ -92,7 +92,8 @@
     def last_run_forms(self) -> dict:
         f = C.c_uint32()
         _lib.check(_lib.lib().rd_batch_last_run_forms(self._b, C.byref(f)))
-        return {"ordered_tail": bool(f.value & 1), "second_pass": bool(f.value & 8), "one_launch_tail": bool(f.value & 16)}
+        return {"ordered_tail": bool(f.value & 1), "second_pass": bool(f.value & 8), "one_launch_tail": bool(f.value & 16),
+                "side_tail": bool(f.value & 32)}
 
     def counters(self) -> dict:
         f, m = C.c_uint64(), C.c_uint64()
diff --git a/rtldavis_amd/csrc/rd_batch.hip b/rtldavis_amd/csrc/rd_batch.hip
--- a/rtldavis_amd/csrc/rd_batch.hip
+++ b/rtldavis_amd/csrc/rd_batch.hip
@@ -35,6 +35,8 @@
     uint32_t *h_cnt_pin = nullptr;
     rd_packet *h_recs_pin = nullptr;
     hipStream_t copy_stream = nullptr;
+    hipStream_t tail_stream = nullptr;
+    bool side_joined = false;
     hipEvent_t done = nullptr;
     hipEvent_t kdone = nullptr;
     hipEvent_t kfirst = nullptr;
@@ -50,6 +52,7 @@
     hipEvent_t *ev = nullptr;
     rd_run_plan plan;
     bool ft_run = false;
+    bool side = false;
     bool dev_order = false;
     int dense = 0;
     bool second_pass = false;
@@ -70,6 +73,7 @@
     rd_batch_sizes sz;
     bool dev_ready = false;
     bool timing = false, timing_detail = false, parse = false, pipelined = false;
+    rd_side_env side_env = {false, 0};
     rd_batch_bufs m;
     rd_batch_run_state run;
     rd_batch_learned learned;
@@ -131,6 +135,29 @@
     return RD_OK;
 }
 
+struct rd_side_dev { hipStream_t stream = nullptr; int handles = 0; };
+static std::mutex g_side_mx;
+static std::map<int, rd_side_dev> g_side;
+
+static int side_join(rd_batch *b) {
+    std::lock_guard<std::mutex> g(g_side_mx);
+    rd_side_dev &d = g_side[b->m.device];
+    if (b->side_env.on && !d.stream) HIPCHK(hipStreamCreateWithFlags(&d.stream, hipStreamNonBlocking));
+    b->m.tail_stream = b->side_env.on ? d.stream : nullptr;
+    d.handles++;
+    b->m.side_joined = true;
+    return RD_OK;
+}
+static void side_leave(rd_batch *b) {
+    std::lock_guard<std::mutex> g(g_side_mx);
+    if (b->m.side_joined) g_side[b->m.device].handles--;
+    b->m.side_joined = false;
+}
+static bool side_others(int device) {
+    std::lock_guard<std::mutex> g(g_side_mx);
+    return g_side[device].handles > 1;
+}
+
 static int batch_alloc(rd_batch *b) {
     rd_batch_bufs &m = b->m;
     if (b->dev_ready) return rd_use_device(m.device);
@@ -156,6 +183,8 @@
     HIPCHK(hipEventCreateWithFlags(&m.kdone, hipEventDisableTiming));
     HIPCHK(hipEventCreateWithFlags(&m.kfirst, hipEventDisableTiming));
     HIPCHK(hipEventCreateWithFlags(&m.uploaded, hipEventDisableTiming));
+    b->side_env = rd_batch_side_env();
+    if ((rc = side_join(b))) return rc;
     HIPCHK(hipStreamCreateWithFlags(&m.copy_stream, hipStreamNonBlocking));
     b->dev_ready = true;
     return RD_OK;
@@ -252,6 +281,7 @@
         std::lock_guard<std::mutex> g(g_tail_mx);
         tail_drop(b);
     }
+    side_leave(b);
     if (b->dev_ready && rd_owns_device_state()) {
         if (b->m.device >= 0) hipSetDevice(b->m.device);
         if (b->run.ran && !b->run.fetched) hipDeviceSynchronize();
@@ -265,6 +295,7 @@
     if (!b || !dev_ptr) return rd_fail_msg(RD_ERR_ARG, "null argument");
     int rc = batch_alloc(b);
     if (rc) return rc;
+    if (b->run.ran && b->run.side && (rc = batch_settle(b, nullptr, "the run's side tail before its input is rewritten"))) return rc;
     *dev_ptr = b->m.d_iq;
     if (nbytes) *nbytes = b->sz.iq_bytes;
     return RD_OK;
@@ -311,7 +342,7 @@
 static int batch_tail(rd_batch *b, bool first, uint32_t *zero_next = nullptr) {
     rd_batch_bufs &m = b->m;
     rd_batch_run_state &r = b->run;
-    hipStream_t st = r.stream;
+    hipStream_t st = first && r.side ? m.tail_stream : r.stream;
     const rd_layout lay = batch_layout(b);
     const long B = b->dc.B, L = b->dc.L, p_lo = B - L, p_hi = (long)(b->n_blocks + 1) * B - L;
     const bool last_on_slice = !b->parse, defer = first && r.plan.defer;
@@ -325,7 +356,7 @@
         r.ft_seq = r.ft_seq % 4095u + 1u;
         const int ok = rd_launch_tail_fused(lay, b->dc, b->n_blocks, p_lo, p_hi, fb, b->sz.ft_limit ? b->sz.ft_limit : fb.bcap, r.ft_seq, 0,
                                             m.d_recs, m.rec_cap, batch_cnt(b), st, last_on_slice ? last : nullptr, zero_next,
-                                            (uint32_t)b->sz.cnt_stride);
+                                            (uint32_t)b->sz.cnt_stride, r.side);
         if (!ok) return rd_fail_msg(RD_ERR_STATE, "the one-launch tail refused a shape its buffers were allocated for");
         r.dev_order = true;
         r.dense = 1;
@@ -398,7 +429,8 @@
     if ((rc = batch_begin_run(b, st, &had_upload))) return rc;
     uint32_t *cnt = batch_cnt(b), *cnt_next = b->m.d_cnt + (size_t)(r.cnt_set ^ 1) * b->sz.cnt_stride;
     const rd_run_plan p = r.plan = rd_batch_plan_run({b->sz.fast_ok, b->sz.ft_ok, b->learned.tail_off, r.timing, r.detail, b->pipelined,
-                                                      b->parse, batch_stream_has_tail(b->m.device, st)});
+                                                      b->parse, batch_stream_has_tail(b->m.device, st), b->m.tail_stream != nullptr,
+                                                      r.ran && r.side, side_others(b->m.device), b->learned.bcap, b->side_env.reserve});
     uint32_t *fixl = p.buckets ? b->m.fixb : b->m.d_fix, *bcnt = p.buckets ? cnt + b->sz.ft_cnt_off : nullptr;
     const uint32_t fixc = p.buckets ? b->sz.fix_bcap : b->sz.fix_cap;
     const rd_layout lay = batch_layout(b);
@@ -406,7 +438,7 @@
     if (p.record_around) HIPCHK(hipEventRecord(r.ev[0], st));
     if (p.demod) {
         honoured = rd_launch_demod(lay, fixl, fixc, cnt, st, batch_event(b, p.ride_start), batch_event(b, p.ride_stop),
-                                   p.buckets ? RD_DEMOD_FIX_BUCKETS : 0u, r.last_launch, bcnt);
+                                   p.buckets ? RD_DEMOD_FIX_BUCKETS : 0u, r.last_launch, bcnt, p.reserve);
         if (honoured & RD_DEMOD_REFUSED) return batch_refused(b, had_upload);
     }
     if (p.record_around) HIPCHK(hipEventRecord(r.ev[1], st));
@@ -414,6 +446,8 @@
     if (p.carrier && (rc = batch_adopt(b->m.device, st, batch_event(b, p.carrier)))) return rc;
     r.second_pass = false;
     r.ft_run = p.demod && (honoured & RD_DEMOD_FIX_BUCKETS);
+    r.side = p.side_tail && r.ft_run;
+    if (r.side) HIPCHK(hipStreamWaitEvent(b->m.tail_stream, batch_event(b, p.ride_stop), 0));
     if (!r.ft_run)
         rd_launch_fixup(lay, fixl, fixc, cnt, p.demod ? 0 : 1, cnt_next, st, (uint32_t)b->sz.cnt_stride, b->learned.last_fix);
     if (r.timing && r.detail) HIPCHK(hipEventRecord(r.ev[2], st));
@@ -607,7 +641,8 @@
     if (!b || !forms) return rd_fail_msg(RD_ERR_ARG, "null argument");
     int rc = batch_finish(b);
     if (rc) return rc;
-    *forms = (b->run.dev_order ? RD_FORM_ORDERED_TAIL | RD_FORM_ONE_LAUNCH_TAIL : 0u) | (b->run.second_pass ? RD_FORM_SECOND_PASS : 0u);
+    *forms = (b->run.dev_order ? RD_FORM_ORDERED_TAIL | RD_FORM_ONE_LAUNCH_TAIL : 0u) | (b->run.second_pass ? RD_FORM_SECOND_PASS : 0u) |
+             (b->run.side ? RD_FORM_SIDE_TAIL : 0u);
     return RD_OK;
 }
 
diff --git a/rtldavis_amd/csrc/rd_batch_plan.cpp b/rtldavis_amd/csrc/rd_batch_plan.cpp
--- a/rtldavis_amd/csrc/rd_batch_plan.cpp
+++ b/rtldavis_amd/csrc/rd_batch_plan.cpp
@@ -71,7 +71,25 @@
     p.defer = m.pipelined && !m.parse && !(m.timing && m.timing_detail);
     p.end_again = m.timing ? RD_RUN_EV4 : RD_RUN_KDONE;
     p.end = p.defer ? RD_RUN_EV_NONE : p.end_again;
+    p.side_tail = m.side_on && p.buckets && !m.pipelined && !m.parse && rd_batch_tail_lds(m.bcap) <= RD_SIDE_LDS;
+    if (p.side_tail && p.ride_stop == RD_RUN_EV_NONE) p.ride_stop = RD_RUN_KFIRST;
+    p.reserve = p.side_tail && m.prev_side && m.others ? m.reserve : 0u;
     return p;
+}
+
+rd_side_env rd_batch_side_env(void) {
+    rd_side_env s = {true, RD_SIDE_RESERVE};
+    if (const char *e = getenv("RD_TAIL_STREAM")) s.on = atol(e) != 0;
+    if (const char *e = getenv("RD_TAIL_RESERVE")) {
+        const long k = atol(e);
+        s.reserve = k < 0 ? 0u : (uint32_t)std::min<long>(k, 1l << 20);
+    }
+    return s;
+}
+
+uint64_t rd_batch_reserved_grid(uint64_t wgs, uint64_t max_wgs, uint32_t k, uint64_t min_wgs) {
+    if (k == 0 || wgs != max_wgs || wgs <= k || wgs - k < min_wgs) return wgs;
+    return wgs - k;
 }
 
 rd_ladder_action rd_batch_ladder_step(const rd_ladder_in &in, rd_batch_learned &lr) {
diff --git a/rtldavis_amd/csrc/rd_batch_plan.h b/rtldavis_amd/csrc/rd_batch_plan.h
--- a/rtldavis_amd/csrc/rd_batch_plan.h
+++ b/rtldavis_amd/csrc/rd_batch_plan.h
@@ -53,12 +53,26 @@
     bool defer = false;
     rd_run_event end = RD_RUN_EV_NONE;
     rd_run_event end_again = RD_RUN_EV_NONE;
+    bool side_tail = false;
+    uint32_t reserve = 0;
 };
 struct rd_run_mode {
     bool fast_ok, ft_ok, tail_off, timing, timing_detail, pipelined, parse;
     bool parked;
+    bool side_on;
+    bool prev_side;
+    bool others;
+    uint32_t bcap;
+    uint32_t reserve;
 };
 rd_run_plan rd_batch_plan_run(const rd_run_mode &m);
+
+static inline size_t rd_batch_tail_lds(uint32_t bcap) { return (size_t)RD_FT_STREAMS * bcap * (8 + 1 + 2 + 4) * sizeof(uint32_t); }
+#define RD_SIDE_LDS (24u * 1024u)
+#define RD_SIDE_RESERVE 256u
+struct rd_side_env { bool on; uint32_t reserve; };
+rd_side_env rd_batch_side_env(void);
+uint64_t rd_batch_reserved_grid(uint64_t wgs, uint64_t max_wgs, uint32_t k, uint64_t min_wgs);
 
 struct rd_batch_learned {
     bool tail_off = false;
diff --git a/rtldavis_amd/csrc/rd_demod_mfma.hip b/rtldavis_amd/csrc/rd_demod_mfma.hip
--- a/rtldavis_amd/csrc/rd_demod_mfma.hip
+++ b/rtldavis_amd/csrc/rd_demod_mfma.hip
@@ -648,6 +648,7 @@
     hipEvent_t ev_start, ev_stop;
     uint32_t *bucket_cnt = nullptr;
     uint32_t *chunk_out = nullptr;
+    uint32_t reserve = 0;
     float *dbg_g;
 };
 
@@ -671,6 +672,7 @@
     uint64_t max_wgs = (uint64_t)P.n_cu * per_cu;
     if (P.test_wgs > 0 && (uint64_t)P.test_wgs < max_wgs) max_wgs = (uint64_t)P.test_wgs;
     if (wgs > max_wgs) wgs = max_wgs;
+    wgs = rd_batch_reserved_grid(wgs, max_wgs, a.reserve, RD_NQUEUE / RD_MF_WAVES);
     {
         const uint64_t nwaves = wgs * RD_MF_WAVES;
         const bool queues = !(P.stflags & 4096) && chunk >= 4;
@@ -703,9 +705,10 @@
 
 int rd_launch_demod_mfma(const rd_layout &lay, uint32_t *fix_list, uint32_t fix_cap, uint32_t *counters, hipStream_t st,
                           hipEvent_t ev_start, hipEvent_t ev_stop, float *dbg_g, uint32_t flags, uint32_t *chunk_out,
-                          uint32_t *bucket_cnt) {
+                          uint32_t *bucket_cnt, uint32_t reserve) {
     rd_mf_launch_args a;
     a.chunk_out = chunk_out;
+    a.reserve = reserve;
     a.bucket_cnt = (flags & RD_DEMOD_FIX_BUCKETS) && !dbg_g ? bucket_cnt : nullptr;
     a.lay = lay;
     a.tps = (lay.n_samples + RD_TILE_SAMPLES - 1) / RD_TILE_SAMPLES;
diff --git a/rtldavis_amd/csrc/rd_internal.h b/rtldavis_amd/csrc/rd_internal.h
--- a/rtldavis_amd/csrc/rd_internal.h
+++ b/rtldavis_amd/csrc/rd_internal.h
@@ -44,10 +44,11 @@
 #define RD_DEMOD_REFUSED 0x80000000u
 uint32_t rd_launch_demod(const rd_layout &lay, uint32_t *fix_list, uint32_t fix_cap, uint32_t *counters, hipStream_t st,
                          hipEvent_t ev_start = nullptr, hipEvent_t ev_stop = nullptr, uint32_t flags = 0,
-                         uint32_t *chunk_out = nullptr, uint32_t *bucket_cnt = nullptr);
+                         uint32_t *chunk_out = nullptr, uint32_t *bucket_cnt = nullptr, uint32_t reserve = 0);
 int rd_launch_demod_mfma(const rd_layout &lay, uint32_t *fix_list, uint32_t fix_cap, uint32_t *counters, hipStream_t st,
                           hipEvent_t ev_start = nullptr, hipEvent_t ev_stop = nullptr, float *dbg_g = nullptr,
-                          uint32_t flags = 0, uint32_t *chunk_out = nullptr, uint32_t *bucket_cnt = nullptr);
+                          uint32_t flags = 0, uint32_t *chunk_out = nullptr, uint32_t *bucket_cnt = nullptr,
+                          uint32_t reserve = 0);
 void rd_debug_last_launch(uint32_t out[2]);
 void rd_launch_fixup(const rd_layout &lay, const uint32_t *fix_list, uint32_t fix_cap, uint32_t *counters, int all,
                      uint32_t *zero_next, hipStream_t st, uint32_t zero_words = RD_CNT_TOTAL, uint64_t expect = 0);
@@ -56,7 +57,8 @@
                       hipStream_t st);
 int rd_launch_tail_fused(const rd_layout &lay, const rd_devcfg &cfg, int n_calls, long p_lo, long p_hi, const rd_ft_bufs &fb,
                          uint32_t bucket_limit, uint32_t seq, int skip_fix, rd_packet *recs, uint32_t rec_cap, uint32_t *counters,
-                         hipStream_t st, hipEvent_t ev_stop = nullptr, uint32_t *zero_next = nullptr, uint32_t zero_words = 0);
+                         hipStream_t st, hipEvent_t ev_stop = nullptr, uint32_t *zero_next = nullptr, uint32_t zero_words = 0,
+                         bool side = false);
 int rd_launch_slice(const rd_layout &lay, const uint32_t *bits, size_t bits_stride, long n_bits, const rd_devcfg &cfg,
                      const rd_match *matches, uint32_t match_cap, int batch_mode, int n_calls, int call,
                      rd_packet *recs, rd_packet *recs_host, uint32_t *counters, hipStream_t st,
diff --git a/rtldavis_amd/csrc/rd_tail.hip b/rtldavis_amd/csrc/rd_tail.hip
--- a/rtldavis_amd/csrc/rd_tail.hip
+++ b/rtldavis_amd/csrc/rd_tail.hip
@@ -54,8 +54,60 @@
     return rd_match_from<S_, P_, PRE_, 3>(m, r, o);
 }
 
-template <int S_, int P_, uint64_t PRE_, int K_>
-__global__ __launch_bounds__(RD_FT_WG, 4) void k_tail(rd_ft_args a) {
+#ifndef RD_FT_SIDE_DEPTH
+#define RD_FT_SIDE_DEPTH 3
+#endif
+__device__ __forceinline__ uint32_t rd_exact_group_dw_lean(const uint32_t *dw, const rd_stream_view &v, long t0, int count) {
+    const long zh64 = v.valid_from - (t0 - 10);
+    const int zh = zh64 <= 0 ? 0 : zh64 >= 17 ? 17 : (int)zh64;
+    int ya[17], yb[17];
+    auto sample = [&](int i) {
+        const uint32_t d = dw[i >> 1] >> (16 * (i & 1));
+        ya[i] = i < zh ? 0 : 5 * (int)(d & 0xFF) - 637;
+        yb[i] = i < zh ? 0 : 5 * (int)((d >> 8) & 0xFF) - 637;
+    };
+    auto fir_from = [&](int j0) {
+        rd_dd2 w[9];
+#pragma unroll
+        for (int m = 0; m < 9; m++) {
+            const int i = j0 + m, ph = (i + 2) & 3;
+            const double a = (double)ya[i], b = (double)yb[i];
+            w[m].x = ph == 0 ? a : ph == 1 ? -b : ph == 2 ? -a : b;
+            w[m].y = ph == 0 ? b : ph == 1 ? a : ph == 2 ? -b : -a;
+        }
+        return rd_fir_f64_exact(w);
+    };
+#pragma unroll
+    for (int i = 0; i < 9; i++) sample(i);
+    rd_dd2 prev = fir_from(0);
+    uint32_t word = 0, unsure = 0;
+#pragma unroll
+    for (int r = 0; r < RD_GROUP; r++) {
+        __builtin_amdgcn_sched_barrier(0);
+        sample(r + 9);
+        const rd_dd2 cur = fir_from(r + 1);
+        const double p1 = prev.y * cur.x, p2 = prev.x * cur.y, d = p1 - p2;
+        const double guard = 4.440892098500626e-16 * (__builtin_fabs(p1) + __builtin_fabs(p2));
+        if (r < count) {
+            if (d > guard) { }
+            else if (d < -guard) word |= 1u << r;
+            else unsure |= 1u << r;
+        }
+        prev = cur;
+    }
+    while (unsure) {
+        const int r = __builtin_ctz(unsure);
+        unsure &= unsure - 1;
+        rd_i2 y[10];
+#pragma unroll
+        for (int m = 0; m < 10; m++) y[m] = rd_sample_int(v, t0 + r - 10 + m);
+        word |= rd_exact_bit(rd_fir_int(&y[0]), rd_fir_int(&y[1])) << r;
+    }
+    return word;
+}
+
+template <int S_, int P_, uint64_t PRE_, int K_, bool SIDE_ = false>
+__global__ __launch_bounds__(RD_FT_WG, SIDE_ ? 7 : 4) void k_tail(rd_ft_args a) {
     constexpr int G = RD_FT_STREAMS;
     static_assert(PRE_ & 1, "positions below 0 are skipped because the preamble starts with a one");
     static_assert(RD_FT_WG == 64 * G, "one wave per stream in the classify strips");
@@ -65,7 +117,8 @@
     uint32_t *s_ord = s_dyn + (size_t)G * a.bcap * 9;
     __shared__ uint32_t s_cnt[G], s_kept[G];
     __shared__ uint32_t s_ready;
-    const int tid = threadIdx.x, lane = tid & 63, wave = __builtin_amdgcn_readfirstlane(tid >> 6);
+    const int tid = threadIdx.x, wave = __builtin_amdgcn_readfirstlane(tid >> 6);
+    int lane = tid & 63;
     const int grp = blockIdx.x, n_groups = gridDim.x;
     const int stream0 = grp * G;
     const int n_here = a.lay.n_streams - stream0 < G ? a.lay.n_streams - stream0 : G;
@@ -80,7 +133,7 @@
     uint32_t n_fix_raw = 0;
     if (!a.skip_fix) {
         const uint32_t *bk = a.fixb + (size_t)grp * a.fix_bcap;
-        const uint32_t e_first = (uint32_t)tid < a.fix_bcap ? bk[tid] : 0u;
+        const uint32_t e_first = !SIDE_ && (uint32_t)tid < a.fix_bcap ? bk[tid] : 0u;
         n_fix_raw = a.fixcnt[grp];
         const uint32_t n_fix = n_fix_raw < a.fix_bcap ? n_fix_raw : a.fix_bcap;
         uint32_t *s_items = s_t;
@@ -90,7 +143,7 @@
             if (tid == 0) s_nitems = 0;
             __syncthreads();
             const uint32_t i = i0 + (uint32_t)tid;
-            const uint32_t e = i < n_fix ? (i0 == 0 ? e_first : bk[i]) : 0u;
+            const uint32_t e = i < n_fix ? (!SIDE_ && i0 == 0 ? e_first : bk[i]) : 0u;
             const uint32_t k = (uint32_t)__popc(e & 0xFu);
             if (k) {
                 uint32_t at = atomicAdd(&s_nitems, k);
@@ -119,12 +172,18 @@
                 const int d_hi = z <= 0 ? 0 : z >= 20 ? 10 : (int)((z + 1) / 2);
 #pragma unroll
                 for (int d = 0; d < 10; d++) dw[d] = (d >= d_lo && d < d_hi) ? *(const uint32_t *)(p + 4 * d) : 0u;
-                ((uint8_t *)a.lay.bits)[(size_t)widx * 4 + g] = (uint8_t)rd_exact_group_dw(dw, t0, count, a.lay.valid_from);
+                ((uint8_t *)a.lay.bits)[(size_t)widx * 4 + g] =
+                    (uint8_t)(SIDE_ ? rd_exact_group_dw_lean(dw, rd_view_of(a.lay, s), t0, count) : rd_exact_group_dw(dw, t0, count, a.lay.valid_from));
             }
             if (i0 + RD_FT_WG < n_fix) __syncthreads();
         }
     }
     __syncthreads();
+    if constexpr (SIDE_) {
+        int t = tid;
+        asm volatile("" : "+v"(t));
+        lane = t & 63;
+    }
     if (wave == 0) RD_FT_STAMP(1);
 
     {
@@ -187,7 +246,7 @@
                 }
             }
         };
-        constexpr int DEPTH = RD_FT_DEPTH;
+        constexpr int DEPTH = SIDE_ ? RD_FT_SIDE_DEPTH : RD_FT_DEPTH;
         uint32_t rb[DEPTH][NW];
         const int dq = G / wgps, dr = G % wgps;
         int fg = wave / wgps, fr = wave % wgps, fu = wave;
@@ -425,11 +484,16 @@
     float *s_res = (float *)(s_dyn + (size_t)G * a.bcap * 11);
     if ((uint32_t)wave < total) {
         rd_k_h8 Ahi[3], Alo[3];
-#pragma unroll
-        for (int d = 0; d < 3; d++) {
-            Ahi[d] = *(const rd_k_h8 *)g_rssi_taps.v[0][d][lane];
-            Alo[d] = *(const rd_k_h8 *)g_rssi_taps.v[1][d][lane];
-        }
+        auto load_taps = [&]() {
+            const rd_mf_taps *tp = &g_rssi_taps;
+            if constexpr (SIDE_) asm volatile("" : "+s"(tp));
+#pragma unroll
+            for (int d = 0; d < 3; d++) {
+                Ahi[d] = *(const rd_k_h8 *)tp->v[0][d][lane];
+                Alo[d] = *(const rd_k_h8 *)tp->v[1][d][lane];
+            }
+        };
+        if constexpr (!SIDE_) load_taps();
         struct task { int stream, call, q; };
         auto task_at = [&](uint32_t r) {
             const uint32_t o = s_ord[r];
@@ -461,6 +525,7 @@
             double rssi = 0.0, snr = 0.0;
             if (j_now.ok) {
                 float noise, sig;
+                if constexpr (SIDE_) load_taps();
                 rd_rssi_block(j_now, d_now, Ahi, Alo, lane, noise, sig);
                 rd_rssi_finish(noise, sig, j_now.ns, j_now.pe, j_now.q, lane, rssi, snr);
             } else {
@@ -509,11 +574,11 @@
 }
 #endif
 
-size_t rd_tail_fused_lds(uint32_t bcap) { return (size_t)RD_FT_STREAMS * bcap * (8 + 1 + 2 + 4) * sizeof(uint32_t); }
+size_t rd_tail_fused_lds(uint32_t bcap) { return rd_batch_tail_lds(bcap); }
 
 int rd_launch_tail_fused(const rd_layout &lay, const rd_devcfg &cfg, int n_calls, long p_lo, long p_hi, const rd_ft_bufs &fb,
                          uint32_t bucket_limit, uint32_t seq, int skip_fix, rd_packet *recs, uint32_t rec_cap, uint32_t *counters,
-                         hipStream_t st, hipEvent_t ev_stop, uint32_t *zero_next, uint32_t zero_words) {
+                         hipStream_t st, hipEvent_t ev_stop, uint32_t *zero_next, uint32_t zero_words, bool side) {
     const long n_bits = lay.n_samples;
     if (!rd_davis_shape(cfg) || n_bits >= (1l << 30) || cfg.B >= (1 << 24) ||
         lay.n_streams <= 0 || p_lo > 0 || p_hi < 0 || p_hi >= (1l << 30) || !fb.gstate || !fb.fixb || fb.bcap == 0 || fb.bcap % 32 ||
@@ -537,8 +602,13 @@
         a.stamps = g_ft_stamps;
     }
 #endif
-    const size_t lds = std::max<size_t>(rd_tail_fused_lds(fb.bcap), 33 * 1024);
-    static bool attr_set = false;
+    const size_t lds = std::max<size_t>(rd_tail_fused_lds(fb.bcap), side ? RD_SIDE_LDS : 33 * 1024);
+    static bool attr_set = false, attr_set_side = false;
+    if (side) {
+        if (lds > 48 * 1024) rd_allow_lds((const void *)k_tail<14, 16, 0x91D3ull, 80, true>, 150 * 1024, attr_set_side);
+        rd_launch_ev(k_tail<14, 16, 0x91D3ull, 80, true>, dim3(groups), dim3(RD_FT_WG), lds, st, ev_stop, a);
+        return 1;
+    }
     if (lds > 48 * 1024) rd_allow_lds((const void *)k_tail<14, 16, 0x91D3ull, 80>, 150 * 1024, attr_set);
     rd_launch_ev(k_tail<14, 16, 0x91D3ull, 80>, dim3(groups), dim3(RD_FT_WG), lds, st, ev_stop, a);
     return 1;
diff --git a/rtldavis_amd/csrc/rd_tail_kernels.hip b/rtldavis_amd/csrc/rd_tail_kernels.hip
--- a/rtldavis_amd/csrc/rd_tail_kernels.hip
+++ b/rtldavis_amd/csrc/rd_tail_kernels.hip
@@ -1,9 +1,11 @@
 #include "rd_device.h"
 
 uint32_t rd_launch_demod(const rd_layout &lay, uint32_t *fix_list, uint32_t fix_cap, uint32_t *counters, hipStream_t st,
-                         hipEvent_t ev_start, hipEvent_t ev_stop, uint32_t flags, uint32_t *chunk_out, uint32_t *bucket_cnt) {
+                         hipEvent_t ev_start, hipEvent_t ev_stop, uint32_t flags, uint32_t *chunk_out, uint32_t *bucket_cnt,
+                         uint32_t reserve) {
     if (!bucket_cnt) flags &= ~RD_DEMOD_FIX_BUCKETS;
-    const int bucketed = rd_launch_demod_mfma(lay, fix_list, fix_cap, counters, st, ev_start, ev_stop, nullptr, flags, chunk_out, bucket_cnt);
+    const int bucketed = rd_launch_demod_mfma(lay, fix_list, fix_cap, counters, st, ev_start, ev_stop, nullptr, flags, chunk_out, bucket_cnt,
+                                              reserve);
     if (bucketed < 0) return RD_DEMOD_REFUSED;
     return bucketed ? RD_DEMOD_FIX_BUCKETS : 0u;
 }
```

Result: slower. 1.995 million MS/s (-5.9%).
